# qq456cvb/VoteNet

Hardware: AMD Instinct MI355X
Metric: SUN RGB-D 20k-pt scenes/sec (fwd+bwd) (higher is better)
Workload: dtype f32

## Files before the change

### votenet_amd/_lib.py

```python
import ctypes
import os
import re
import subprocess

import torch

_HERE = os.path.dirname(os.path.abspath(__file__))
_LIB_PATH = os.path.join(_HERE, "lib", "libvotenet_hip.so")
_lib = None
SIDE_LIBS = {
    "monitors": "votenet_monitors.h",
    "guard": "votenet_step_guard.h",
    "features": "votenet_point_features.h",
    "detect": "votenet_detections.h",
    "boxpts": "votenet_box_points.h",
    "aabb": "votenet_aabb_nms.h",
    "depth": "votenet_depth_scan.h",
    "votesup": "votenet_vote_supervision.h",
    "propsup": "votenet_proposal_supervision.h",
    "votesamp": "votenet_vote_sampling.h",
    "instbox": "votenet_instance_boxes.h",
    "instvote": "votenet_instance_votes.h",
    "unitvote": "votenet_unit_votes.h",
}
_side = {}


class VotenetError(RuntimeError):
    """A HIP runtime / launch / workspace error reported by libvotenet_hip.so."""


class InvalidArgumentError(ValueError):
    """Mirror of tf.errors.InvalidArgumentError raised by the reference's OP_REQUIRES checks."""


def lib_path():
    return _LIB_PATH


def build(force=False):
    if force:
        import glob
        objs = [o for d in ["obj"] + [os.path.join(name, "obj") for name in SIDE_LIBS] for o in glob.glob(os.path.join(_HERE, "csrc", d, "*.o"))]
        for f in [_LIB_PATH] + [side_path(name) for name in SIDE_LIBS] + objs:
            if os.path.exists(f):
                os.remove(f)
    out = subprocess.run(["bash", os.path.join(_HERE, "csrc", "build.sh")], capture_output=True, text=True)
    if out.returncode != 0:
        raise VotenetError("libvotenet_hip.so build failed:\n" + out.stdout + out.stderr)
    return _LIB_PATH


_SCALARS = {"int": ctypes.c_int, "long": ctypes.c_long, "float": ctypes.c_float, "double": ctypes.c_double, "unsigned": ctypes.c_uint,
            "unsigned long long": ctypes.c_ulonglong, "size_t": ctypes.c_size_t}
_POINTEES = set(_SCALARS) | {"void", "char", "unsigned char", "unsigned short", "long long"}


def _declarator(text, where):
    words = text.replace("*", " * ").split()
    if not words or not words[-1].isidentifier():
        raise ValueError("%s: cannot read the declaration '%s'" % (where, " ".join(text.split())))
    return " ".join(w for w in words[:-1] if w != "const" and w != "*"), words.count("*"), words[-1]


def _ctype(base, stars, structs, where, ret=False):
    if stars == 0 and base in _SCALARS:
        return _SCALARS[base]
    if stars == 0 and ret and base == "void":
        return None
    if stars == 1 and base in structs:
        return ctypes.POINTER(structs[base])
    if stars == 1 and ret and base == "char":
        return ctypes.c_char_p
    if stars == 1 and base in _POINTEES:
        return ctypes.c_void_p
    raise ValueError("%s: no ctypes type for the C type '%s'" % (where, base + " *" * stars))


def parse_header(text, structs):
    text = re.sub(r"/\*.*?\*/|//[^\n]*", " ", text, flags=re.S)
    text = re.sub(r"#ifdef __cplusplus.*?#endif", "", text, flags=re.S)
    text = re.sub(r"^[ \t]*#.*$", "", text, flags=re.M)

    def struct(m):
        name, fields = m.group(2), []
        for line in filter(str.strip, m.group(1).split(";")):
            decls = [_declarator(d, name) for d in line.split(",")]
            fields += [(n, _ctype(decls[0][0], stars, structs, name + "." + n)) for _, stars, n in decls]
        structs[name] = type("".join(w.capitalize() for w in name.split("_")[1:]), (ctypes.Structure,),
                             {"_fields_": fields, "__doc__": "struct %s of the C ABI." % name})
        return ""
    text = re.sub(r"typedef\s+struct\s+\w+\s*\{(.*?)\}\s*(\w+)\s*;", struct, text, flags=re.S)
    funcs = {}
    for stmt in text.split(";"):
        if not stmt.strip():
            continue
        m = re.fullmatch(r"(.*?)\((.*)\)\s*", stmt, flags=re.S)
        if not m:
            raise ValueError("not a function declaration: '%s'" % " ".join(stmt.split()))
        base, stars, name = _declarator(m.group(1), "function")
        params = [] if m.group(2).strip() == "void" else m.group(2).split(",")
        funcs[name] = (_ctype(base, stars, structs, name, ret=True),
                       [_ctype(*_declarator(p, name)[:2], structs, name) for p in params])
    return funcs


_STRUCTS = ("BnRaw", "CoefTail", "MlpInput", "RowSegment", "CopySegment")
_abi_read = None


def _abi():
    global _abi_read
    if _abi_read is None:
        structs, protos = {}, []
        for h in ("votenet_hip.h", "votenet_hip_debug.h"):
            with open(os.path.join(_HERE, os.pardir, "include", h)) as f:
                protos.append(parse_header(f.read(), structs))
        globals().update({cls.__name__: cls for cls in structs.values()})
        _abi_read = tuple(protos)
    return _abi_read


def __getattr__(name):
    if name in _STRUCTS:
        _abi()
        return globals()[name]
    raise AttributeError("module %r has no attribute %r" % (__name__, name))


class _Library(ctypes.CDLL):

    def __getattr__(self, name):
        fn = super().__getattr__(name)
        for protos in _abi():
            if name in protos:
                fn.restype, fn.argtypes = protos[name]
        if "debug" in name and name not in ("votenet_debug_enable", "votenet_debug_enabled", "votenet_debug_fps_split_timeouts"):
            self.votenet_debug_enable(1)
        return fn


def lib():
    global _lib
    if _lib is None:
        if not os.path.exists(_LIB_PATH):
            raise VotenetError(
                "libvotenet_hip.so not found at %s -- run `python -c 'import __graft_entry__ as g; g.build()'` "
                "(there is no CPU fallback)" % _LIB_PATH)
        L = _Library(_LIB_PATH)
        for name in _abi()[0]:
            getattr(L, name)
        _lib = L
    return _lib


def side_path(name):
    return os.path.join(os.path.dirname(_LIB_PATH), "libvotenet_%s.so" % name)


def side_loaded(name):
    return name in _side


def side_lib(name):
    if name not in _side:
        path = side_path(name)
        if not os.path.exists(path):
            raise VotenetError("libvotenet_%s.so not found at %s -- run `python -c 'import __graft_entry__ as g; g.build()'` "
                               "(there is no CPU fallback)" % (name, path))
        with open(os.path.join(_HERE, os.pardir, "include", SIDE_LIBS[name])) as f:
            protos = parse_header(f.read(), {})
        S = ctypes.CDLL(path)
        for fname, (restype, argtypes) in protos.items():
            fn = getattr(S, fname)
            fn.restype, fn.argtypes = restype, argtypes
        last_error, = [getattr(S, fname) for fname in protos if fname.endswith("_last_error")]
        _side[name] = (S, last_error)
    return _side[name][0]


def check(rc, side=None):
    if rc == 0:
        return
    if side is None:
        msg, who = lib().votenet_last_error().decode(), "hip"
    else:
        side_lib(side)
        msg, who = _side[side][1]().decode(), side
    if rc == 1:
        raise InvalidArgumentError(msg)
    raise VotenetError("libvotenet_%s error %d: %s" % (who, rc, msg))


_raw_stream = getattr(torch._C, "_cuda_getCurrentRawStream", None)
_cur_device = getattr(torch._C, "_cuda_getDevice", None)


def stream_ptr():
    if _raw_stream is not None and _cur_device is not None:
        return _raw_stream(_cur_device())
    return torch.cuda.current_stream().cuda_stream


class _NoGuard:
    def __enter__(self):
        return None

    def __exit__(self, *a):
        return False


_NOGUARD = _NoGuard()


def device_guard(device):
    idx = device.index
    if _cur_device is not None and (idx is None or idx == _cur_device()):
        return _NOGUARD
    return torch.cuda.device(device)


def ptr(t):
    return t.data_ptr() if t is not None else None


def dev_f32(t, name, rank=None, last=None):
    if not isinstance(t, torch.Tensor):
        raise InvalidArgumentError("%s must be a torch.Tensor" % name)
    if not t.is_cuda:
        raise VotenetError("%s must live on the GPU (no CPU fallback in votenet_amd)" % name)
    if t.dtype != torch.float32:
        raise InvalidArgumentError("%s must be float32" % name)
    if rank is not None and t.dim() != rank:
        raise InvalidArgumentError("%s expects rank %d, got shape %s" % (name, rank, tuple(t.shape)))
    if last is not None and t.shape[-1] != last:
        raise InvalidArgumentError("%s expects last dimension %d, got shape %s" % (name, last, tuple(t.shape)))
    return t.contiguous()


def pitched_rows(t):
    return t.dim() == 3 and t.stride(2) == 1 and t.stride(1) >= t.shape[2] and t.stride(0) == t.shape[1] * t.stride(1)


def dev_f32_rows(t, name):
    if isinstance(t, torch.Tensor) and t.is_cuda and t.dtype == torch.float32 and pitched_rows(t):
        return t
    return dev_f32(t, name, 3)


def dev_i32(t, name, rank=None):
    if not isinstance(t, torch.Tensor):
        raise InvalidArgumentError("%s must be a torch.Tensor" % name)
    if not t.is_cuda:
        raise VotenetError("%s must live on the GPU (no CPU fallback in votenet_amd)" % name)
    if t.dtype != torch.int32:
        raise InvalidArgumentError("%s must be int32" % name)
    if rank is not None and t.dim() != rank:
        raise InvalidArgumentError("%s expects rank %d, got shape %s" % (name, rank, tuple(t.shape)))
    return t.contiguous()
```

### votenet_amd/csrc/half.hip

```cpp
#include "mlp_types.h"

namespace votenet {

constexpr int PS = kPiece, NP = kBallPieces, TP = kTilePieces;

__device__ __forceinline__ int kept_pieces(int cnt)
{
    const int c = cnt < 1 ? 1 : cnt;
    const int k = (c + PS - 1) / PS;
    return k > NP ? NP : k;
}

__global__ __launch_bounds__(1024) void half_groups_kernel(int G, const int *__restrict__ pts_cnt, int *__restrict__ pos, int *__restrict__ hc,
                                                           float *__restrict__ wh, int *__restrict__ nh_out, int *nh_host)
{
    __shared__ int s_wave[16];
    __shared__ int s_carry;
    const int tid = threadIdx.x, lane = tid & 63, wv = tid >> 6;
    if (tid == 0) s_carry = 0;
    __syncthreads();
    for (int c0 = 0; c0 < G; c0 += 1024) {
        const int c = c0 + tid;
        const int kc = c < G ? kept_pieces(pts_cnt[c]) : 1;
        const int mine = kc - 1;
        int x = mine;
#pragma unroll
        for (int off = 1; off < 64; off <<= 1) {
            const int t = __shfl_up(x, off);
            if (lane >= off) x += t;
        }
        if (lane == 63) s_wave[wv] = x;
        __syncthreads();
        int base = s_carry;
        for (int w = 0; w < wv; w++) base += s_wave[w];
        int p = base + x - mine;
        if (c < G) {
            hc[c] = c * NP;
            for (int j = 1; j < NP; j++) {
                if (j < kc) {
                    hc[G + p] = c * NP + j;
                    pos[c * (NP - 1) + j - 1] = p++;
                } else {
                    pos[c * (NP - 1) + j - 1] = -1;
                }
            }
        }
        __syncthreads();
        if (tid == 1023) s_carry = base + x;
        __syncthreads();
    }
    if (tid == 0) {
        int n2 = s_carry;
        for (int c = 0; c < G && ((G + n2) % TP) != 0; c++)
            for (int j = 1; j < NP && ((G + n2) % TP) != 0; j++)
                if (pos[c * (NP - 1) + j - 1] < 0) {
                    pos[c * (NP - 1) + j - 1] = n2;
                    hc[G + n2] = c * NP + j;
                    n2++;
                }
        s_carry = n2;
        nh_out[0] = G + n2;
        if (nh_host != nullptr) {
            nh_host[0] = G + n2;
            __threadfence_system();
        }
    }
    __syncthreads();
    const int nh = G + s_carry;
    for (int q = tid; q < nh; q += 1024) {
        float w = 1.0f;
        if (q < G) {
            int kc = 1;
            for (int j = 1; j < NP; j++) kc += pos[q * (NP - 1) + j - 1] >= 0 ? 1 : 0;
            w = 1.0f + (float)(PS * (NP - kc));
        }
        wh[q] = w;
    }
}

__device__ __forceinline__ double half_shfl_xor_f64(double v, int m)
{
    int lo = __double2loint(v), hi = __double2hiint(v);
    lo = __shfl_xor(lo, m);
    hi = __shfl_xor(hi, m);
    return __hiloint2double(hi, lo);
}
__device__ __forceinline__ long long half_fixed(float v) { return (long long)((double)v * 4294967296.0); }

__device__ __forceinline__ void half_sort_runs(unsigned prow, bool live, int lane, int &run_start, int &run_len)
{
    const unsigned prev = __shfl_up(prow, 1);
    const bool prev_live = __shfl_up((int)live, 1) != 0;
    const bool starts = live && (lane == 0 || !prev_live || prev != prow);
    const unsigned long long sm = __ballot(starts), lm = __ballot(live);
    const unsigned long long below = sm & ((lane == 63) ? ~0ull : ((1ull << (lane + 1)) - 1ull));
    run_start = below ? 63 - __builtin_clzll(below) : 0;
    const unsigned long long after = (sm | ~lm) & ~((run_start == 63) ? ~0ull : ((1ull << (run_start + 1)) - 1ull));
    const int end = after ? __builtin_ctzll(after) : 64;
    run_len = end - run_start;
}
__global__ __launch_bounds__(256) void assemble_rows_half_kernel(const int *__restrict__ nh_dev, long max_rows, int n, int groups_per_scene, const float *__restrict__ xyz,
                                                                 const float *__restrict__ new_xyz, const int *__restrict__ idx,
                                                                 const int *__restrict__ pts_cnt, const int *__restrict__ hc,
                                                                 float4 *__restrict__ geo, long long *__restrict__ cntv,
                                                                 double *__restrict__ moments, int *__restrict__ count)
{
    __shared__ double red[4][9];
    double acc[9];
#pragma unroll
    for (int i = 0; i < 9; i++) acc[i] = 0.0;
    const long rows = (long)nh_dev[0] * PS;
    for (long r0 = (long)blockIdx.x * 256; r0 < max_rows; r0 += (long)gridDim.x * 256) {
        const long r = r0 + threadIdx.x;
        const bool live = r < rows;
        unsigned my_prow = 0;
        if (!live && r < max_rows) geo[r] = make_float4(0.f, 0.f, 0.f, __uint_as_float(0u));
        if (live) {
        const int q = (int)(r / PS), s = (int)(r % PS);
        const int code = hc[q];
        const int c = code / NP;
        const int k = (code % NP) * PS + s;
        const int id = idx[(size_t)c * 64 + k];
        const unsigned prow = ((unsigned)c / (unsigned)groups_per_scene) * (unsigned)n + (unsigned)id;
        const float dx = xyz[(size_t)prow * 3 + 0] - new_xyz[(size_t)c * 3 + 0];
        const float dy = xyz[(size_t)prow * 3 + 1] - new_xyz[(size_t)c * 3 + 1];
        const float dz = xyz[(size_t)prow * 3 + 2] - new_xyz[(size_t)c * 3 + 2];
        geo[r] = make_float4(dx, dy, dz, __uint_as_float(prow));
        my_prow = prow;
        int cnt = pts_cnt[c];
        if (cnt < 1) cnt = 1;
        if (k < cnt) {
            const long long mult = (k == 0) ? (long long)(64 - cnt + 1) : 1LL;
            if (cntv) {
                unsigned long long *cv = reinterpret_cast<unsigned long long *>(cntv + (size_t)prow * 4);
                atomicAdd(cv + 0, (unsigned long long)mult);
                atomicAdd(cv + 1, (unsigned long long)(mult * half_fixed(dx)));
                atomicAdd(cv + 2, (unsigned long long)(mult * half_fixed(dy)));
                atomicAdd(cv + 3, (unsigned long long)(mult * half_fixed(dz)));
            }
            const double m = (double)mult, x = dx, y = dy, z = dz;
            acc[0] += m * x; acc[1] += m * y; acc[2] += m * z;
            acc[3] += m * x * x; acc[4] += m * x * y; acc[5] += m * x * z; acc[6] += m * y * y; acc[7] += m * y * z; acc[8] += m * z * z;
        }
        }
        if (count) {
            int rs, rl;
            half_sort_runs(my_prow, live, threadIdx.x & 63, rs, rl);
            if (live && rs == (int)(threadIdx.x & 63)) atomicAdd(&count[my_prow], rl);
        }
    }
    if (!moments) return;
#pragma unroll
    for (int i = 0; i < 9; i++) {
        double v = acc[i];
#pragma unroll
        for (int m = 32; m >= 1; m >>= 1) v += half_shfl_xor_f64(v, m);
        if ((threadIdx.x & 63) == 0) red[threadIdx.x >> 6][i] = v;
    }
    __syncthreads();
    if (threadIdx.x < 9)
        unsafeAtomicAdd(&moments[threadIdx.x], (red[0][threadIdx.x] + red[1][threadIdx.x]) + (red[2][threadIdx.x] + red[3][threadIdx.x]));
}

__global__ __launch_bounds__(256) void narrow_rows_half_kernel(const int *__restrict__ nh_dev, int n, int groups_per_scene, int c,
                                                               const float *__restrict__ xyz, const float *__restrict__ new_xyz,
                                                               const float *__restrict__ feat, const int *__restrict__ idx,
                                                               const int *__restrict__ pts_cnt, const int *__restrict__ hc,
                                                               float *__restrict__ u8, double *__restrict__ moments)
{
    __shared__ double red[4][44];
    double acc[44];
#pragma unroll
    for (int i = 0; i < 44; i++) acc[i] = 0.0;
    const long rows = (long)nh_dev[0] * PS;
    for (long r = (long)blockIdx.x * 256 + threadIdx.x; r < rows; r += (long)gridDim.x * 256) {
        const int q = (int)(r / PS), s = (int)(r % PS);
        const int code = hc[q];
        const int ctr = code / NP;
        const int k = (code % NP) * PS + s;
        const int id = idx[(size_t)ctr * 64 + k];
        const size_t prow = (size_t)((unsigned)ctr / (unsigned)groups_per_scene) * n + id;
        float u[8];
        u[0] = xyz[prow * 3 + 0] - new_xyz[(size_t)ctr * 3 + 0];
        u[1] = xyz[prow * 3 + 1] - new_xyz[(size_t)ctr * 3 + 1];
        u[2] = xyz[prow * 3 + 2] - new_xyz[(size_t)ctr * 3 + 2];
#pragma unroll
        for (int d = 0; d < 5; d++) u[3 + d] = d < c ? feat[prow * c + d] : 0.0f;
        *reinterpret_cast<float4 *>(u8 + (size_t)r * 8) = make_float4(u[0], u[1], u[2], u[3]);
        *reinterpret_cast<float4 *>(u8 + (size_t)r * 8 + 4) = make_float4(u[4], u[5], u[6], u[7]);
        int cnt = pts_cnt[ctr];
        if (cnt < 1) cnt = 1;
        if (k < cnt) {
            const double mult = (k == 0) ? (double)(64 - cnt + 1) : 1.0;
            int t = 8;
#pragma unroll
            for (int d = 0; d < 8; d++) {
                acc[d] += mult * (double)u[d];
#pragma unroll
                for (int e = d; e < 8; e++) acc[t++] += mult * ((double)u[d] * (double)u[e]);
            }
        }
    }
    if (!moments) return;
#pragma unroll
    for (int i = 0; i < 44; i++) {
        double v = acc[i];
#pragma unroll
        for (int m = 32; m >= 1; m >>= 1) v += half_shfl_xor_f64(v, m);
        if ((threadIdx.x & 63) == 0) red[threadIdx.x >> 6][i] = v;
    }
    __syncthreads();
    if (threadIdx.x < 44) {
        const double v = (red[0][threadIdx.x] + red[1][threadIdx.x]) + (red[2][threadIdx.x] + red[3][threadIdx.x]);
        const int i = threadIdx.x;
        if (i < 8) {
            unsafeAtomicAdd(&moments[i], v);
        } else {
            int d = 0, t = 8;
            while (i >= t + (8 - d)) {
                t += 8 - d;
                d++;
            }
            const int e = d + (i - t);
            unsafeAtomicAdd(&moments[8 + d * 8 + e], v);
            if (e != d) unsafeAtomicAdd(&moments[8 + e * 8 + d], v);
        }
    }
}

__global__ void bn_pool_finalize_half_kernel(long total, int G, int c, const float *__restrict__ zbest, const int *__restrict__ abest,
                                             const int *__restrict__ pos, const float *__restrict__ scale, const float *__restrict__ shift,
                                             BnRaw raw, int relu, float *__restrict__ out, int *__restrict__ argmax, float *__restrict__ zsel)
{
    const long e0 = (long)blockIdx.x * blockDim.x + threadIdx.x;
    const int ch = (int)(e0 % c);
    float s = 0.0f, h = 0.0f;
    if (e0 < total) {
        if (raw.stats) bn_raw_channel(raw, c, ch, e0 < c, s, h);
        else {
            s = scale[ch];
            h = shift[ch];
        }
    }
    for (long e = e0; e < total; e += (long)gridDim.x * blockDim.x) {
        const long g = e / c;
        const float sg = s >= 0.0f ? 1.0f : -1.0f;
        int pj[NP - 1];
#pragma unroll
        for (int j = 1; j < NP; j++) pj[j - 1] = pos[g * (NP - 1) + j - 1];
        float zb[NP];
        int ab[NP];
        zb[0] = zbest[e];
        ab[0] = abest[e];
#pragma unroll
        for (int j = 1; j < NP; j++) {
            const size_t e2 = pj[j - 1] >= 0 ? (size_t)(G + pj[j - 1]) * c + ch : (size_t)e;
            zb[j] = zbest[e2];
            ab[j] = abest[e2];
        }
        float best = sg * zb[0];
        int ibest = ab[0];
#pragma unroll
        for (int j = 1; j < NP; j++) {
            const float b = sg * zb[j];
            if (pj[j - 1] >= 0 && b > best) {
                best = b;
                ibest = j * PS + ab[j];
            }
        }
        const float zr = sg * best;
        float v = zr * s + h;
        if (relu && !(v > 0.0f)) v = 0.0f;
        out[e] = v;
        if (argmax) argmax[e] = ibest;
        if (zsel) zsel[e] = zr;
    }
}

__global__ __launch_bounds__(256) void half_sort_count_kernel(const int *__restrict__ nh_dev, const float4 *__restrict__ geo,
                                                              int *__restrict__ count)
{
    const long rows = (long)nh_dev[0] * PS;
    const int lane = threadIdx.x & 63;
    for (long r0 = (long)blockIdx.x * 256; r0 < rows; r0 += (long)gridDim.x * 256) {
        const long r = r0 + threadIdx.x;
        const bool live = r < rows;
        const unsigned prow = live ? __float_as_uint(geo[r].w) : 0u;
        int rs, rl;
        half_sort_runs(prow, live, lane, rs, rl);
        if (live && rs == lane) atomicAdd(&count[prow], rl);
    }
}
__global__ __launch_bounds__(1024) void half_sort_scan_kernel(int npts, int *__restrict__ count)
{
    __shared__ int s_wave[16];
    const int tid = threadIdx.x, lane = tid & 63, wv = tid >> 6;
    const int per = (npts + 1023) / 1024;
    const int b0 = tid * per < npts ? tid * per : npts, e0 = b0 + per < npts ? b0 + per : npts;
    constexpr int KEEP = 16;
    int v[KEEP];
    int tot = 0;
    if (per <= KEEP) {
#pragma unroll
        for (int i = 0; i < KEEP; i++) v[i] = b0 + i < e0 ? count[b0 + i] : 0;
#pragma unroll
        for (int i = 0; i < KEEP; i++) tot += v[i];
    } else {
        for (int p = b0; p < e0; p++) tot += count[p];
    }
    int x = tot;
#pragma unroll
    for (int off = 1; off < 64; off <<= 1) {
        const int t = __shfl_up(x, off);
        if (lane >= off) x += t;
    }
    if (lane == 63) s_wave[wv] = x;
    __syncthreads();
    int run = x - tot;
    for (int w = 0; w < wv; w++) run += s_wave[w];
    if (per <= KEEP) {
#pragma unroll
        for (int i = 0; i < KEEP; i++) {
            if (b0 + i < e0) count[b0 + i] = run;
            run += v[i];
        }
        return;
    }
    for (int p = b0; p < e0; p++) {
        const int c = count[p];
        count[p] = run;
        run += c;
    }
}
__global__ __launch_bounds__(256) void half_sort_fill_kernel(const int *__restrict__ nh_dev, const float4 *__restrict__ geo,
                                                             int *__restrict__ cursor, int *__restrict__ order)
{
    const long rows = (long)nh_dev[0] * PS;
    const int lane = threadIdx.x & 63;
    for (long r0 = (long)blockIdx.x * 256; r0 < rows; r0 += (long)gridDim.x * 256) {
        const long r = r0 + threadIdx.x;
        const bool live = r < rows;
        const unsigned prow = live ? __float_as_uint(geo[r].w) : 0u;
        int rs, rl;
        half_sort_runs(prow, live, lane, rs, rl);
        int base = 0;
        if (live && rs == lane) base = atomicAdd(&cursor[prow], rl);
        base = __shfl(base, rs);
        if (live) order[base + (lane - rs)] = (int)r;
    }
}

template <int COUT>
__global__ __launch_bounds__(256) void group_linear_bwd_sorted_kernel(long rows, const int *__restrict__ order, const float4 *__restrict__ geo,
                                                                      const float *__restrict__ wh, const float *__restrict__ ptab,
                                                                      const float *__restrict__ wx, const float *__restrict__ da,
                                                                      const float *__restrict__ coef, int relu, float *__restrict__ spt,
                                                                      float *__restrict__ dw_xyz, const int *__restrict__ nh_dev)
{
    if (nh_dev != nullptr) {
        const long lim = (long)nh_dev[0] * PS;
        rows = lim < rows ? lim : rows;
    }
    constexpr int CPB = 256 / COUT;
    constexpr int CH = 64;
    __shared__ int s_row[CPB][CH];
    __shared__ float4 s_geo[CPB][CH];
    __shared__ float s_w[CPB][CH];
    __shared__ float red[256][3];
    const int tid = threadIdx.x;
    const int ch = tid % COUT, cl = tid / COUT;
    const float kA = coef[ch], kB = coef[COUT + ch], kC = coef[2 * COUT + ch], kS = coef[3 * COUT + ch], kH = coef[4 * COUT + ch];
    const float wx0 = wx[ch], wx1 = wx[COUT + ch], wx2 = wx[2 * COUT + ch];
    float a0 = 0.f, a1 = 0.f, a2 = 0.f;
    const long nchunk = (rows + CH - 1) / CH;
    for (long c0 = (long)blockIdx.x * CPB; c0 < nchunk; c0 += (long)gridDim.x * CPB) {
        lds_barrier();
        if (tid < CPB * CH) {
            const long e = c0 * CH + tid;
            int r = -1;
            float4 g4 = make_float4(0.f, 0.f, 0.f, 0.f);
            float w = 1.0f;
            if (e < rows) {
                r = order[e];
                g4 = geo[r];
                if (r % PS == 0) w = wh[r / PS];
            }
            s_row[tid / CH][tid % CH] = r;
            s_geo[tid / CH][tid % CH] = g4;
            s_w[tid / CH][tid % CH] = w;
        }
        lds_barrier();
        if (c0 + cl >= nchunk) continue;
        unsigned cur = 0xffffffffu;
        float acc = 0.0f;
        bool first = true;
#pragma unroll 1
        for (int e0 = 0; e0 < CH; e0 += 8) {
            float gg[8], zz[8];
#pragma unroll
            for (int u = 0; u < 8; u++) {
                const int r = s_row[cl][e0 + u];
                const int rr = r < 0 ? 0 : r;
                gg[u] = da[(size_t)rr * COUT + ch];
                zz[u] = ptab[(size_t)__float_as_uint(s_geo[cl][e0 + u].w) * COUT + ch];
            }
#pragma unroll
            for (int u = 0; u < 8; u++) {
                if (s_row[cl][e0 + u] < 0) continue;
                const float4 g4 = s_geo[cl][e0 + u];
                const unsigned prow = __float_as_uint(g4.w);
                if (prow != cur) {
                    if (cur != 0xffffffffu) {
                        if (first) unsafeAtomicAdd(&spt[(size_t)cur * COUT + ch], acc);
                        else spt[(size_t)cur * COUT + ch] = acc;
                        first = false;
                    }
                    cur = prow;
                    acc = 0.0f;
                }
                const float z = assembled_z(zz[u], g4, wx0, wx1, wx2);
                float gq = gg[u];
                if (relu && !(z * kS + kH > 0.0f)) gq = 0.0f;
                const float d = kA * gq + s_w[cl][e0 + u] * (kB + kC * z);
                a0 += g4.x * d;
                a1 += g4.y * d;
                a2 += g4.z * d;
                acc += d;
            }
        }
        if (cur != 0xffffffffu) unsafeAtomicAdd(&spt[(size_t)cur * COUT + ch], acc);
    }
    red[tid][0] = a0;
    red[tid][1] = a1;
    red[tid][2] = a2;
    __syncthreads();
    if (tid < COUT) {
#pragma unroll
        for (int d = 0; d < 3; d++) {
            float t = 0.0f;
            for (int q = 0; q < CPB; q++) t += red[q * COUT + tid][d];
            unsafeAtomicAdd(&dw_xyz[(size_t)d * COUT + tid], t);
        }
    }
}

constexpr int kMaskedSlots = 32;
template <int COUT>
__global__ __launch_bounds__(256) void group_linear_bwd_masked_kernel(long rows, const int *__restrict__ order, const float4 *__restrict__ geo,
                                                                      const float *__restrict__ ptab, const float *__restrict__ wx,
                                                                      const float *__restrict__ da, const float *__restrict__ scale,
                                                                      const float *__restrict__ shift, const float *__restrict__ mean,
                                                                      const float *__restrict__ var, float eps, int relu,
                                                                      float *__restrict__ sg, float *__restrict__ ug, double *__restrict__ sums,
                                                                      double *__restrict__ part ,
                                                                      const int *__restrict__ nh_dev, CoefTail tail)
{
    if (nh_dev != nullptr) {
        const long lim = (long)nh_dev[0] * PS;
        rows = lim < rows ? lim : rows;
    }
    constexpr int CPB = 256 / COUT;
    constexpr int CH = 64;
    constexpr int GB = 8;
    __shared__ int s_row[CPB][CH];
    __shared__ float4 s_geo[CPB][CH];
    __shared__ float red[256][5];
    const int tid = threadIdx.x;
    const int ch = tid % COUT, cl = tid / COUT;
    const float kS = scale[ch], kH = shift[ch], kM = mean[ch], kR = 1.0f / sqrtf(var[ch] + eps);
    const float wx0 = wx[ch], wx1 = wx[COUT + ch], wx2 = wx[2 * COUT + ch];
    float a0 = 0.f, a1 = 0.f, a2 = 0.f, s1 = 0.f, s2 = 0.f;
    const long nchunk = (rows + CH - 1) / CH;
    for (long c0 = (long)blockIdx.x * CPB; c0 < nchunk; c0 += (long)gridDim.x * CPB) {
        lds_barrier();
        if (tid < CPB * CH) {
            const long e = c0 * CH + tid;
            int r = -1;
            float4 g4 = make_float4(0.f, 0.f, 0.f, 0.f);
            if (e < rows) {
                r = order[e];
                g4 = geo[r];
            }
            s_row[tid / CH][tid % CH] = r;
            s_geo[tid / CH][tid % CH] = g4;
        }
        lds_barrier();
        if (c0 + cl >= nchunk) continue;
        unsigned cur = 0xffffffffu;
        float acc = 0.0f;
        bool first = true;
#pragma unroll 1
        for (int e0 = 0; e0 < CH; e0 += GB) {
            float gg[GB], zz[GB];
#pragma unroll
            for (int u = 0; u < GB; u++) {
                const int r = s_row[cl][e0 + u];
                const int rr = r < 0 ? 0 : r;
                gg[u] = da[(size_t)rr * COUT + ch];
                zz[u] = ptab[(size_t)__float_as_uint(s_geo[cl][e0 + u].w) * COUT + ch];
            }
#pragma unroll
            for (int u = 0; u < GB; u++) {
                if (s_row[cl][e0 + u] < 0) continue;
                const float4 g4 = s_geo[cl][e0 + u];
                const unsigned prow = __float_as_uint(g4.w);
                if (prow != cur) {
                    if (cur != 0xffffffffu) {
                        if (first) unsafeAtomicAdd(&sg[(size_t)cur * COUT + ch], acc);
                        else sg[(size_t)cur * COUT + ch] = acc;
                        first = false;
                    }
                    cur = prow;
                    acc = 0.0f;
                }
                const float z = assembled_z(zz[u], g4, wx0, wx1, wx2);
                float gq = gg[u];
                if (relu && !(z * kS + kH > 0.0f)) gq = 0.0f;
                a0 += g4.x * gq;
                a1 += g4.y * gq;
                a2 += g4.z * gq;
                s1 += gq;
                s2 += gq * ((z - kM) * kR);
                acc += gq;
            }
        }
        if (cur != 0xffffffffu) unsafeAtomicAdd(&sg[(size_t)cur * COUT + ch], acc);
    }
    red[tid][0] = a0;
    red[tid][1] = a1;
    red[tid][2] = a2;
    red[tid][3] = s1;
    red[tid][4] = s2;
    __syncthreads();
    if (tid < COUT) {
        float t[5];
#pragma unroll
        for (int d = 0; d < 5; d++) {
            t[d] = 0.0f;
            for (int q = 0; q < CPB; q++) t[d] += red[q * COUT + tid][d];
        }
        double *ps = part + (size_t)(blockIdx.x % kMaskedSlots) * 5 * COUT;
#pragma unroll
        for (int d = 0; d < 5; d++) unsafeAtomicAdd(&ps[(size_t)d * COUT + tid], (double)t[d]);
    }
    __shared__ unsigned s_last;
    asm volatile("s_waitcnt vmcnt(0)" ::: "memory");
    __syncthreads();
    if (threadIdx.x == 0) s_last = (__hip_atomic_fetch_add(tail.ticket, 1u, __ATOMIC_RELAXED, __HIP_MEMORY_SCOPE_AGENT) == gridDim.x - 1) ? 1u : 0u;
    __syncthreads();
    if (!s_last) return;
    const double invn = 1.0 / (double)tail.rows;
    for (int col = threadIdx.x; col < COUT; col += blockDim.x) {
        double q[5] = {0.0, 0.0, 0.0, 0.0, 0.0};
        for (int sl = 0; sl < kMaskedSlots; sl++)
#pragma unroll
            for (int d = 0; d < 5; d++)
                q[d] += __hip_atomic_load(&part[((size_t)sl * 5 + d) * COUT + col], __ATOMIC_RELAXED, __HIP_MEMORY_SCOPE_AGENT);
#pragma unroll
        for (int d = 0; d < 3; d++) ug[(size_t)d * COUT + col] = (float)q[d];
        sums[col] = q[3];
        sums[COUT + col] = q[4];
        const float inv = 1.0f / sqrtf(var[col] + eps);
        const float m1 = (float)(q[3] * invn), m2 = (float)(q[4] * invn);
        const float cA = tail.gamma[col] * inv;
        const float cC = -cA * inv * m2;
        tail.coef[col] = cA;
        tail.coef[COUT + col] = -cA * m1 - cC * mean[col];
        tail.coef[2 * COUT + col] = cC;
        tail.coef[3 * COUT + col] = scale[col];
        tail.coef[4 * COUT + col] = shift[col];
        if (tail.dgamma) tail.dgamma[col] += (float)q[4];
        if (tail.dbeta) tail.dbeta[col] += (float)q[3];
    }
    if (threadIdx.x == 0) *tail.ticket = 0u;
}

template <int COUT>
__global__ __launch_bounds__(256) void assembled_point_grad_kernel(long npts, const float *__restrict__ ptab, const long long *__restrict__ cntv,
                                                                   const float *__restrict__ wx, const float *__restrict__ coef,
                                                                   float *__restrict__ s, float *__restrict__ vp )
{
    constexpr int PPB = 256 / COUT;
    constexpr int U = 4;
    __shared__ float red[256][3];
    const int tid = threadIdx.x, ch = tid % COUT, pl = tid / COUT;
    const float kA = coef[ch], kB = coef[COUT + ch], kC = coef[2 * COUT + ch];
    const float wx0 = wx[ch], wx1 = wx[COUT + ch], wx2 = wx[2 * COUT + ch];
    float v0 = 0.f, v1 = 0.f, v2 = 0.f;
    const long stride = (long)gridDim.x * PPB;
    for (long p0 = (long)blockIdx.x * PPB + pl; p0 < npts; p0 += U * stride) {
        long long c4[U][4];
        float pv[U], sv[U];
#pragma unroll
        for (int u = 0; u < U; u++) {
            const long p = p0 + u * stride < npts ? p0 + u * stride : p0;
            const long long *cv = cntv + (size_t)p * 4;
            c4[u][0] = cv[0];
            c4[u][1] = cv[1];
            c4[u][2] = cv[2];
            c4[u][3] = cv[3];
            pv[u] = ptab[(size_t)p * COUT + ch];
            sv[u] = s[(size_t)p * COUT + ch];
        }
#pragma unroll
        for (int u = 0; u < U; u++) {
            const long p = p0 + u * stride;
            if (p >= npts || c4[u][0] == 0) continue;
            const float fx = (float)((double)c4[u][1] * (1.0 / 4294967296.0)), fy = (float)((double)c4[u][2] * (1.0 / 4294967296.0)),
                        fz = (float)((double)c4[u][3] * (1.0 / 4294967296.0));
            const float fc = (float)c4[u][0];
            const float zsum = fc * pv[u] + (fx * wx0 + fy * wx1 + fz * wx2);
            s[(size_t)p * COUT + ch] = kA * sv[u] + fc * kB + kC * zsum;
            v0 += fx * pv[u];
            v1 += fy * pv[u];
            v2 += fz * pv[u];
        }
    }
    red[tid][0] = v0;
    red[tid][1] = v1;
    red[tid][2] = v2;
    __syncthreads();
    if (tid < COUT) {
#pragma unroll
        for (int d = 0; d < 3; d++) {
            float t = 0.0f;
            for (int q = 0; q < PPB; q++) t += red[q * COUT + tid][d];
            unsafeAtomicAdd(&vp[((size_t)(blockIdx.x % kMaskedSlots) * 3 + d) * COUT + tid], t);
        }
    }
}

__global__ __launch_bounds__(256) void assembled_wx_finish_kernel(int cout, const float *__restrict__ coef, const float *__restrict__ ug,
                                                                  const float *__restrict__ vp, int nparts, const double *__restrict__ mom,
                                                                  const float *__restrict__ wx, float *__restrict__ dw_xyz)
{
// ... 241 lines not shown
```

### votenet_amd/csrc/loss.hip

```cpp
#include "common.h"
#include "nearest_box.h"

namespace votenet {

#ifndef LOSS_ABL
#define LOSS_ABL 0
#endif
constexpr int LOSS_T = 1024;
constexpr int LOSS_MAXC = 32;
constexpr int LOSS_NACC = 12;

struct LossArgs {
    int b, n, p, bb, nh, ns, nc;
    const float *seeds, *votes, *pxyz, *pout;
    const float *gxyz, *glwh, *groty;
    const int *sem, *hlab, *slab;
    const float *hres, *sres;
    float pos_thr, neg_thr;
    float *losses, *d_votes, *d_pxyz, *d_pout;
    long pout_pitch;
};

__device__ __forceinline__ float huber(float e, float &grad)
{
    const float a = fabsf(e);
    grad = a <= 1.0f ? e : (e > 0.0f ? 1.0f : -1.0f);
    return a <= 1.0f ? 0.5f * e * e : a - 0.5f;
}

__device__ __forceinline__ float softmax_ce(const float *lg, int c, int label, float *probs)
{
    float m = lg[0];
    for (int i = 1; i < c; i++) m = fmaxf(m, lg[i]);
    float s = 0.0f;
    for (int i = 0; i < c; i++) {
        probs[i] = expf(lg[i] - m);
        s += probs[i];
    }
    if ((unsigned)label >= (unsigned)c) {
        const float nan = __uint_as_float(0x7FC00000u);
        for (int i = 0; i < c; i++) probs[i] = nan;
        return nan;
    }
    const float inv = 1.0f / s;
    for (int i = 0; i < c; i++) probs[i] = probs[i] * inv - (i == label ? 1.0f : 0.0f);
    return logf(s) + m - lg[label];
}


__global__ __launch_bounds__(256) void votenet_loss_count_kernel(LossArgs A, int *counts)
{
    __shared__ float s_box[LOSS_MAXBOX][8];
    const int b = blockIdx.x, tid = threadIdx.x, BB = A.bb, P = A.p;
    for (int j = tid; j < BB; j += 256)
        for (int k = 0; k < 3; k++) s_box[j][k] = A.gxyz[(b * BB + j) * 3 + k];
    __syncthreads();
    int np_local = 0, nn_local = 0;
    for (int pq = tid; pq < P; pq += 256) {
        const int q = b * P + pq;
        int g;
        const float best = nearest_box(s_box, BB, A.pxyz[q * 3 + 0], A.pxyz[q * 3 + 1], A.pxyz[q * 3 + 2], g);
        np_local += best < A.pos_thr;
        nn_local += best > A.neg_thr;
    }
    for (int off = 32; off > 0; off >>= 1) {
        np_local += __shfl_down(np_local, off);
        nn_local += __shfl_down(nn_local, off);
    }
    if ((tid & 63) == 0) {
        if (np_local) atomicAdd(&counts[0], np_local);
        if (nn_local) atomicAdd(&counts[1], nn_local);
    }
}

__global__ __launch_bounds__(LOSS_T) void votenet_loss_kernel(LossArgs A, int *counts, float *partial )
{
    __shared__ float s_box[LOSS_MAXBOX][8];
    __shared__ float s_red[LOSS_T / 64][LOSS_NACC];
    __shared__ float s_dual[LOSS_MAXBOX][3];
    __shared__ int s_dualp[LOSS_MAXBOX];
    __shared__ int s_last;
    const int tid = threadIdx.x, b = blockIdx.x;
    const int B = A.b, N = A.n, P = A.p, BB = A.bb, NH = A.nh, NS = A.ns, NC = A.nc;
    const int W = 5 + 2 * NH + 4 * NS + NC;
    for (int j = tid; j < BB; j += LOSS_T) {
        const int e = b * BB + j;
        s_box[j][0] = A.gxyz[e * 3 + 0];
        s_box[j][1] = A.gxyz[e * 3 + 1];
        s_box[j][2] = A.gxyz[e * 3 + 2];
        s_box[j][3] = A.glwh[e * 3 + 0] * 0.5f;
        s_box[j][4] = A.glwh[e * 3 + 1] * 0.5f;
        s_box[j][5] = A.glwh[e * 3 + 2] * 0.5f;
        s_box[j][6] = cosf(-A.groty[e]);
        s_box[j][7] = sinf(-A.groty[e]);
    }
    __syncthreads();
    const int n_pos = counts[0], n_neg = counts[1];
    const float inv_np = 1.0f / (float)n_pos, inv_nn = 1.0f / (float)n_neg;
    float acc[LOSS_NACC];
#pragma unroll
    for (int i = 0; i < LOSS_NACC; i++) acc[i] = 0.0f;
    const int wave = tid >> 6, nwave = LOSS_T / 64;
    const int nbusy = (P + 63) / 64 < nwave ? (P + 63) / 64 : nwave, nfree = nwave - nbusy;
    const bool early = nfree > 0;
    const float inv_bn = 1.0f / (float)(B * N);
    auto seed_terms = [&](int first, int step) {
        for (int i = first; i < ((LOSS_ABL & 2) ? 0 : N); i += step) {
            const int e = b * N + i;
            const float sx = A.seeds[e * 3 + 0], sy = A.seeds[e * 3 + 1], sz = A.seeds[e * 3 + 2];
            float best = 0.0f;
            int g = 0;
            bool surface = false;
            for (int j = 0; j < BB; j++) {
                const float dx = fabsf(sx - s_box[j][0]), dy = fabsf(sy - s_box[j][1]), dz = fabsf(sz - s_box[j][2]);
                const float c = s_box[j][6], s = s_box[j][7];
                const float rx = c * dx + s * dz, ry = dy, rz = -s * dx + c * dz;
                surface = surface || (rx < s_box[j][3] && ry < s_box[j][4] && rz < s_box[j][5]);
                const float d = sqrtf(rx * rx + ry * ry + rz * rz);
                if (j == 0 || d < best) {
                    best = d;
                    g = j;
                }
            }
            if (surface) {
                for (int k = 0; k < 3; k++) {
                    const float df = A.votes[e * 3 + k] - s_box[g][k];
                    acc[0] += fabsf(df);
                    A.d_votes[e * 3 + k] = (df > 0.0f ? 1.0f : (df < 0.0f ? -1.0f : 0.0f)) * inv_bn;
                }
            }
        }
    };
    float pr[LOSS_MAXC];
    for (int pq = tid; pq < ((LOSS_ABL & 1) ? 0 : P); pq += LOSS_T) {
        const int q = b * P + pq;
        const float px = A.pxyz[q * 3 + 0], py = A.pxyz[q * 3 + 1], pz = A.pxyz[q * 3 + 2];
        int g;
        const float best = nearest_box(s_box, BB, px, py, pz, g);
        const float *o = A.pout + (size_t)q * A.pout_pitch;
        float *go = A.d_pout + (size_t)q * W;
        const bool pos = best < A.pos_thr, neg = best > A.neg_thr;
        if (pos || neg) {
            const float l = softmax_ce(o, 2, pos ? 1 : 0, pr);
            const float w = 0.5f * (pos ? inv_np : inv_nn);
            acc[pos ? 1 : 2] += l;
            go[0] = pr[0] * w;
            go[1] = pr[1] * w;
        }
        if (pos) {
            const int gi = b * BB + g;
            const float cg[3] = {s_box[g][0] - px, s_box[g][1] - py, s_box[g][2] - pz};
            for (int k = 0; k < 3; k++) {
                float gr;
                acc[3] += huber(o[2 + k] - cg[k], gr);
                go[2 + k] += gr * inv_np;
                A.d_pxyz[q * 3 + k] += gr * inv_np;
            }
            const int hl = A.hlab[gi];
            const bool hok = (unsigned)hl < (unsigned)NH;
            acc[5] += softmax_ce(o + 5, NH, hl, pr);
            for (int i = 0; i < NH; i++) go[5 + i] = pr[i] * (0.1f * inv_np);
            {
                float gr;
                acc[6] += huber((hok ? o[5 + NH + hl] : 0.0f) - A.hres[gi], gr);
                if (hok) go[5 + NH + hl] = gr * inv_np;
            }
            const int sl = A.slab[gi], so = 5 + 2 * NH;
            const bool sok = (unsigned)sl < (unsigned)NS;
            acc[7] += softmax_ce(o + so, NS, sl, pr);
            for (int i = 0; i < NS; i++) go[so + i] = pr[i] * (0.1f * inv_np);
            for (int k = 0; k < 3; k++) {
                float gr;
                acc[8] += huber((sok ? o[so + NS + sl * 3 + k] : 0.0f) - A.sres[gi * 3 + k], gr);
                if (sok) go[so + NS + sl * 3 + k] = gr * inv_np;
            }
            const int co = W - NC;
            acc[9] += softmax_ce(o + co, NC, A.sem[gi], pr);
            for (int i = 0; i < NC; i++) go[co + i] = pr[i] * (0.1f * inv_np);
        }
    }
    const float inv_bbb = 1.0f / (float)(B * BB);
    const int dw = early ? wave - nbusy : wave, dstep = early ? nfree : nwave;
    for (int j = dw < 0 ? BB : dw; j < ((LOSS_ABL & 4) ? 0 : BB); j += dstep) {
        const int lane = tid & 63;
        const float gx = s_box[j][0], gy = s_box[j][1], gz = s_box[j][2];
        float best = INFINITY;
        int bp = 0x7FFFFFFF;
        for (int p = lane; p < P; p += 64) {
            const float dx = A.pxyz[(b * P + p) * 3 + 0] - gx, dy = A.pxyz[(b * P + p) * 3 + 1] - gy,
                        dz = A.pxyz[(b * P + p) * 3 + 2] - gz;
            const float d = sqrtf(dx * dx + dy * dy + dz * dz);
            if (d < best) {
                best = d;
                bp = p;
            }
        }
        for (int off = 32; off > 0; off >>= 1) {
            const float ob = __shfl_xor(best, off);
            const int op = __shfl_xor(bp, off);
            if (ob < best || (ob == best && op < bp)) {
                best = ob;
                bp = op;
            }
        }
        if ((unsigned)bp >= (unsigned)P) bp = 0;
        if (lane < 3) {
            const int k = lane, q = b * P + bp;
            const float cgk = (k == 0 ? gx : (k == 1 ? gy : gz)) - A.pxyz[q * 3 + k];
            float gr;
            acc[4] += huber(A.pout[(size_t)q * A.pout_pitch + 2 + k] - cgk, gr);
            s_dual[j][k] = gr * inv_bbb;
            if (k == 0) s_dualp[j] = bp;
        }
    }
    if (early && wave >= nbusy) seed_terms(tid - nbusy * 64, nfree * 64);
    __syncthreads();
    for (int pq = tid; pq < P; pq += LOSS_T) {
        const int q = b * P + pq;
        for (int j = 0; j < BB; j++)
            if (s_dualp[j] == pq) {
#pragma unroll
                for (int k = 0; k < 3; k++) {
                    A.d_pout[(size_t)q * W + 2 + k] += s_dual[j][k];
                    A.d_pxyz[q * 3 + k] += s_dual[j][k];
                }
            }
    }
    if (!early) seed_terms(tid, LOSS_T);
#pragma unroll
    for (int i = 0; i < LOSS_NACC; i++) {
        float v = acc[i];
        for (int off = 32; off > 0; off >>= 1) v += __shfl_down(v, off);
        if ((tid & 63) == 0) s_red[tid >> 6][i] = v;
    }
    __syncthreads();
    if (tid < LOSS_NACC) {
        float v = 0.0f;
        for (int w = 0; w < LOSS_T / 64; w++) v += s_red[w][tid];
        partial[b * LOSS_NACC + tid] = v;
    }
    __threadfence();
    __syncthreads();
    if (tid == 0) s_last = (atomicAdd(&counts[2], 1) == B - 1);
    __syncthreads();
    if (!s_last) return;
    __threadfence();
    if (tid < LOSS_NACC) {
        float v = 0.0f;
        for (int sc = 0; sc < B; sc++) v += __builtin_nontemporal_load(&partial[sc * LOSS_NACC + tid]);
        s_red[0][tid] = v;
    }
    __syncthreads();
    if (tid == 0) {
        float t[LOSS_NACC];
        for (int i = 0; i < LOSS_NACC; i++) t[i] = s_red[0][i];
        const float vote = t[0] * inv_bn;
        const float obj = t[1] * inv_np + t[2] * inv_nn;
        const float center = t[3] * inv_np + t[4] * inv_bbb;
        const float hcls = t[5] * inv_np, hres = t[6] * inv_np, scls = t[7] * inv_np, sres = t[8] * inv_np, sem = t[9] * inv_np;
        const float box = center + 0.1f * hcls + hres + 0.1f * scls + sres;
        float *L = A.losses;
        L[0] = vote + 0.5f * obj + box + 0.1f * sem;
        L[1] = vote;
        L[2] = obj;
        L[3] = center;
        L[4] = hcls;
        L[5] = hres;
        L[6] = scls;
        L[7] = sres;
        L[8] = sem;
        L[9] = box;
        L[10] = (float)n_pos;
        L[11] = (float)n_neg;
    }
}

}

using namespace votenet;

extern "C" size_t votenet_loss_workspace_floats(int b) { return 4 + (size_t)(b > 0 ? b : 0) * LOSS_NACC; }

extern "C" int votenet_loss_pitched(int b, int n_seeds, int n_prop, int n_box, int nh, int ns, int nc, const float *seeds_xyz,
                            const float *votes_xyz, const float *proposals_xyz, const float *proposals_output, long output_pitch,
                            const float *bboxes_xyz,
                            const float *bboxes_lwh, const float *bboxes_roty, const int *semantic_labels, const int *heading_labels,
                            const float *heading_residuals, const int *size_labels, const float *size_residuals, float pos_thr,
                            float neg_thr, float *losses, float *d_votes_xyz, float *d_proposals_xyz, float *d_proposals_output,
                            float *workspace, void *stream)
{
    VN_REQUIRE(b > 0 && n_seeds > 0 && n_prop > 0 && n_box > 0, "votenet_loss expects b, n_seeds, n_prop, n_box > 0");
    VN_REQUIRE(n_box <= LOSS_MAXBOX, "votenet_loss expects at most 256 boxes per scene");
    VN_REQUIRE(nh > 0 && ns > 0 && nc > 0 && nh <= LOSS_MAXC && ns <= LOSS_MAXC && nc <= LOSS_MAXC, "votenet_loss expects 0 < nh, ns, nc <= 32");
    VN_REQUIRE(pos_thr < neg_thr, "votenet_loss expects pos_thr < neg_thr (config.py)");
    VN_REQUIRE(seeds_xyz && votes_xyz && proposals_xyz && proposals_output && bboxes_xyz && bboxes_lwh && bboxes_roty &&
                   semantic_labels && heading_labels && heading_residuals && size_labels && size_residuals && losses &&
                   d_votes_xyz && d_proposals_xyz && d_proposals_output && workspace,
               "votenet_loss: null buffer");
    VN_REQUIRE(output_pitch >= 5 + 2 * nh + 4 * ns + nc, "votenet_loss: the pitch of proposals_output is smaller than its width");
    LossArgs a = {b, n_seeds, n_prop, n_box, nh, ns, nc, seeds_xyz, votes_xyz, proposals_xyz, proposals_output, bboxes_xyz, bboxes_lwh,
                  bboxes_roty, semantic_labels, heading_labels, size_labels, heading_residuals, size_residuals, pos_thr, neg_thr, losses,
                  d_votes_xyz, d_proposals_xyz, d_proposals_output, output_pitch};
    int *counts = reinterpret_cast<int *>(workspace);
    hipStream_t st = as_stream(stream);
    hipLaunchKernelGGL(votenet_loss_count_kernel, dim3(b), dim3(256), 0, st, a, counts);
    hipLaunchKernelGGL(votenet_loss_kernel, dim3(b), dim3(LOSS_T), 0, st, a, counts, workspace + 4);
    return check_launch("votenet_loss");
}

extern "C" int votenet_loss(int b, int n_seeds, int n_prop, int n_box, int nh, int ns, int nc, const float *seeds_xyz,
                            const float *votes_xyz, const float *proposals_xyz, const float *proposals_output, const float *bboxes_xyz,
                            const float *bboxes_lwh, const float *bboxes_roty, const int *semantic_labels, const int *heading_labels,
                            const float *heading_residuals, const int *size_labels, const float *size_residuals, float pos_thr,
                            float neg_thr, float *losses, float *d_votes_xyz, float *d_proposals_xyz, float *d_proposals_output,
                            float *workspace, void *stream)
{
    return votenet_loss_pitched(b, n_seeds, n_prop, n_box, nh, ns, nc, seeds_xyz, votes_xyz, proposals_xyz, proposals_output,
                                5 + 2 * nh + 4 * ns + nc, bboxes_xyz, bboxes_lwh, bboxes_roty, semantic_labels, heading_labels,
                                heading_residuals, size_labels, size_residuals, pos_thr, neg_thr, losses, d_votes_xyz, d_proposals_xyz,
                                d_proposals_output, workspace, stream);
}

namespace votenet {

__global__ void decode_boxes_kernel(int total, int nh, int ns, int nc, const float *__restrict__ pxyz, const float *__restrict__ pout,
                                    const float *__restrict__ mean_size, float *__restrict__ boxes, float *__restrict__ scores)
{
    const int q = blockIdx.x * blockDim.x + threadIdx.x;
    if (q >= total) return;
    const int W = 5 + 2 * nh + 4 * ns + nc;
    const float *o = pout + (size_t)q * W;
    int sc = 0;
    for (int i = 1; i < ns; i++)
        if (o[5 + 2 * nh + i] > o[5 + 2 * nh + sc]) sc = i;
    int hc = 0;
    for (int i = 1; i < nh; i++)
        if (o[5 + i] > o[5 + hc]) hc = i;
    float size[3];
    for (int k = 0; k < 3; k++) size[k] = mean_size[sc * 3 + k] * fmaxf(1.0f + o[5 + 2 * nh + ns + sc * 3 + k], 1e-6f);
    const float cx = pxyz[q * 3 + 0] + o[2], cy = pxyz[q * 3 + 1] + o[3], cz = pxyz[q * 3 + 2] + o[4];
    const float PI_F = 3.14159265358979323846f;
    const float t = ((float)hc * 2.0f + o[5 + nh + hc]) * (PI_F / (float)nh);
    float ang = fmodf(t, 2.0f * PI_F);
    if (ang < 0.0f) ang += 2.0f * PI_F;
    const float c = cosf(ang), s = sinf(ang);
    const float l = size[0], w = size[1], h = size[2];
    const float sx[8] = {1, 1, -1, -1, 1, 1, -1, -1}, sy[8] = {1, 1, 1, 1, -1, -1, -1, -1}, sz[8] = {1, -1, -1, 1, 1, -1, -1, 1};
    float *bx = boxes + (size_t)q * 24;
    for (int m = 0; m < 8; m++) {
        const float x0 = sx[m] * l * 0.5f, y0 = sy[m] * h * 0.5f, z0 = sz[m] * w * 0.5f;
        bx[m * 3 + 0] = c * x0 + s * z0 + cx;
        bx[m * 3 + 1] = y0 + cy;
        bx[m * 3 + 2] = -s * x0 + c * z0 + cz;
    }
    float best = o[W - nc];
    for (int i = 1; i < nc; i++) best = fmaxf(best, o[W - nc + i]);
    scores[q] = best;
}

}

extern "C" int votenet_decode_boxes(int b, int n_prop, int nh, int ns, int nc, const float *proposals_xyz, const float *proposals_output,
                                    const float *class_mean_size, float *bboxes, float *scores, void *stream)
{
    VN_REQUIRE(b >= 0 && n_prop >= 0 && nh > 0 && ns > 0 && nc > 0, "decode_boxes: bad shape");
    const int total = b * n_prop;
    if (total == 0) return VOTENET_OK;
    VN_REQUIRE(proposals_xyz && proposals_output && class_mean_size && bboxes && scores, "decode_boxes: null buffer");
    hipLaunchKernelGGL(votenet::decode_boxes_kernel, dim3((total + 255) / 256), dim3(256), 0, as_stream(stream), total, nh, ns, nc,
                       proposals_xyz, proposals_output, class_mean_size, bboxes, scores);
    return check_launch("decode_boxes");
}
```

### votenet_amd/loss.py

```python
import torch

from . import _lib as L
from .synth import NC, NH, NS

POSITIVE_THRES, NEGATIVE_THRES = 0.3, 0.6
NAMES = ("total_cost", "vote_reg_loss", "obj_cls_loss", "center_loss", "heading_cls_loss", "heading_residual_loss",
         "size_cls_loss", "size_residual_loss", "sem_cls_loss", "box_loss", "n_pos", "n_neg")
GT_KEYS = ("bboxes_xyz", "bboxes_lwh", "bboxes_roty", "semantic_labels", "heading_labels", "heading_residuals", "size_labels",
           "size_residuals")


def gt_to_device(gt, device):
    return {k: torch.from_numpy(gt[k]).contiguous().to(device) for k in GT_KEYS}


def loss_buffers(out, losses=None):
    from . import mlp as M
    votes, pxyz, pout = out["votes_xyz"], out["proposals_xyz"], out["proposals_output"]
    nws = int(L.lib().votenet_loss_workspace_floats(votes.shape[0]))
    if losses is None:
        losses = torch.empty(12, dtype=torch.float32, device=votes.device)
    return losses, M._zeros_f32((votes.numel() + pxyz.numel() + pout.numel() + nws,), votes.device)


def cotangent_views(votes, pxyz, pout, flat):
    nv, npx, npo = votes.numel(), pxyz.numel(), pout.numel()
    cot = dict(votes_xyz=flat[:nv].view_as(votes), proposals_xyz=flat[nv:nv + npx].view_as(pxyz),
               proposals_output=flat[nv + npx:nv + npx + npo].view_as(pout))
    return cot, flat[nv + npx + npo:]


def check_losses(losses, dev, who):
    if not (isinstance(losses, torch.Tensor) and losses.is_cuda and losses.dtype == torch.float32 and losses.numel() == 12
            and losses.is_contiguous() and losses.device == dev):
        raise L.InvalidArgumentError("%s: losses must be the 12 floats of votenet_loss on the device" % who)


def votenet_loss(out, gt, nh=NH, ns=NS, nc=NC, buffers=None):
    seeds = L.dev_f32(out["seeds_xyz"], "loss seeds_xyz", 3, 3)
    votes = L.dev_f32(out["votes_xyz"], "loss votes_xyz", 3, 3)
    pxyz = L.dev_f32(out["proposals_xyz"], "loss proposals_xyz", 3, 3)
    pout = L.dev_f32_rows(out["proposals_output"], "loss proposals_output")
    b, n = seeds.shape[:2]
    p = pxyz.shape[1]
    bb = gt["bboxes_xyz"].shape[1]
    if pout.shape[2] != 5 + 2 * nh + 4 * ns + nc:
        raise L.InvalidArgumentError("loss: proposals_output has %d channels, expected %d" % (pout.shape[2], 5 + 2 * nh + 4 * ns + nc))
    dev = seeds.device
    total = votes.numel() + pxyz.numel() + pout.numel() + int(L.lib().votenet_loss_workspace_floats(b))
    from . import mlp as M
    if buffers is not None:
        losses, flat = buffers
        if flat.numel() != total or losses.numel() != 12:
            raise L.InvalidArgumentError("loss: the buffers were made for other shapes (loss_buffers(out))")
    else:
        losses = torch.empty(12, dtype=torch.float32, device=dev)
        flat = M._zeros_f32((total,), dev)
    cot, ws = cotangent_views(votes, pxyz, pout, flat)
    with L.device_guard(dev):
        L.check(L.lib().votenet_loss_pitched(b, n, p, bb, nh, ns, nc, L.ptr(seeds), L.ptr(votes), L.ptr(pxyz), L.ptr(pout), pout.stride(1),
                                     L.ptr(gt["bboxes_xyz"]), L.ptr(gt["bboxes_lwh"]), L.ptr(gt["bboxes_roty"]),
                                     L.ptr(gt["semantic_labels"]), L.ptr(gt["heading_labels"]), L.ptr(gt["heading_residuals"]),
                                     L.ptr(gt["size_labels"]), L.ptr(gt["size_residuals"]), POSITIVE_THRES, NEGATIVE_THRES,
                                     L.ptr(losses), L.ptr(cot["votes_xyz"]), L.ptr(cot["proposals_xyz"]), L.ptr(cot["proposals_output"]),
                                     L.ptr(ws), L.stream_ptr()))
    return losses, cot


ACCURACY_COUNTS = ("n_obj_correct", "n_sem_correct", "n_pos", "n_neg")
RING_COLS = 5


def votenet_accuracies(out, gt, nh=NH, ns=NS, nc=NC, losses=None, ring=None, ring_row=0, buffers=None):
    pxyz = L.dev_f32(out["proposals_xyz"], "accuracies proposals_xyz", 3, 3)
    pout = L.dev_f32_rows(out["proposals_output"], "accuracies proposals_output")
    b, p = pxyz.shape[:2]
    if pout.shape[2] != 5 + 2 * nh + 4 * ns + nc or tuple(pout.shape[:2]) != (b, p):
        raise L.InvalidArgumentError("accuracies: proposals_output has shape %s, expected (%d, %d, %d)"
                                     % (tuple(pout.shape), b, p, 5 + 2 * nh + 4 * ns + nc))
    gxyz, sem = L.dev_f32(gt["bboxes_xyz"], "accuracies bboxes_xyz", 3, 3), L.dev_i32(gt["semantic_labels"], "accuracies semantic_labels", 2)
    if gxyz.shape[0] != b or tuple(sem.shape) != tuple(gxyz.shape[:2]):
        raise L.InvalidArgumentError("accuracies: ground truth of %s boxes / %s labels for %d scenes" % (tuple(gxyz.shape), tuple(sem.shape), b))
    dev = pxyz.device
    if buffers is not None:
        acc, counts, work = buffers
    else:
        acc = torch.empty(2, dtype=torch.float32, device=dev)
        counts = torch.empty(4, dtype=torch.int32, device=dev)
        work = torch.zeros(8, dtype=torch.int32, device=dev)
    if acc.numel() != 2 or counts.numel() != 4 or work.numel() < 8:
        raise L.InvalidArgumentError("accuracies: buffers of the wrong size")
    rows = 0
    if ring is not None:
        ring = L.dev_f32(ring, "accuracies ring", 2, RING_COLS)
        rows = ring.shape[0]
        if not 0 <= ring_row < rows:
            raise L.InvalidArgumentError("accuracies: row %d outside a ring of %d rows" % (ring_row, rows))
    if losses is not None and (losses.numel() != 12 or losses.dtype != torch.float32 or not losses.is_cuda):
        raise L.InvalidArgumentError("accuracies: losses must be the 12 floats of votenet_loss on the device")
    with L.device_guard(dev):
        L.check(L.side_lib("monitors").votenet_accuracies(b, p, gxyz.shape[1], nh, ns, nc, L.ptr(pxyz), L.ptr(pout), pout.stride(1), L.ptr(gxyz), L.ptr(sem),
                                           POSITIVE_THRES, NEGATIVE_THRES, L.ptr(losses), L.ptr(ring), rows, ring_row, L.ptr(acc),
                                           L.ptr(counts), L.ptr(work), L.stream_ptr()), side="monitors")
    return acc, counts


def decode_boxes(proposals_xyz, proposals_output, nh=NH, ns=NS, nc=NC):
    from .synth import MEAN_SIZES
    pxyz = L.dev_f32(proposals_xyz, "decode_boxes proposals_xyz", 3, 3)
    pout = L.dev_f32(proposals_output, "decode_boxes proposals_output", 3)
    b, p = pxyz.shape[:2]
    if pout.shape[2] != 5 + 2 * nh + 4 * ns + nc:
        raise L.InvalidArgumentError("decode_boxes: proposals_output has %d channels" % pout.shape[2])
    mean = torch.tensor(MEAN_SIZES, dtype=torch.float32, device=pxyz.device).contiguous()
    boxes = torch.empty((b, p, 8, 3), dtype=torch.float32, device=pxyz.device)
    scores = torch.empty((b, p), dtype=torch.float32, device=pxyz.device)
    with L.device_guard(pxyz.device):
        L.check(L.lib().votenet_decode_boxes(b, p, nh, ns, nc, L.ptr(pxyz), L.ptr(pout), L.ptr(mean), L.ptr(boxes), L.ptr(scores),
                                             L.stream_ptr()))
    return boxes, scores
```

### votenet_amd/model.py

```python

import math
from typing import NamedTuple

import torch

from . import checkpoint
from . import dp
from . import mlp as M
from . import pointnet2 as P

NH, NS, NC = 12, 10, 10
PREFETCH_AFTER = 2
SIDE_PRIORITY = 0
WGRAD_PRIORITY = 0
PROPOSAL_NUM = 256
PROPOSAL_OUT = 5 + 2 * NH + 4 * NS + NC
LEARNING_RATE = 1e-3


GEOMETRY_GRAPHS = True
GEOMETRY_MAX_EVICTIONS = 8
GEOMETRY_RING = 3


# ... 442 lines not shown
            tape.append(dict(op="vote", recs=recs, b=b, n=n))
        return v_xyz, v_p

    def propose(self, votes_xyz, votes_points, seeds_xyz, tape=None, prop_fps=None):
        geom = None
        if self.proposal_sampling == "vote_fps":
            from . import vote_sampling as VSAMP
            pr = self.proposal
            geom = pr.geometry(votes_xyz, grouped=VSAMP.cluster_votes(votes_xyz, pr.npoint, pr.radius, pr.nsample))
        elif prop_fps is not None:
            geom = self.proposal.geometry(votes_xyz, fps_idx=prop_fps, ahead=False)
        p_xyz, p_out, _ = self.proposal.forward(votes_xyz, votes_points, sample_xyz=seeds_xyz, tape=tape, geom=geom)
        return p_xyz, p_out

    def forward(self, x, tape=None, next_x=None, feats=None, next_feats=None):
        self._sa1_points(x, feats)
        self.store.refresh_split()
        M.arena_begin(self.device)
        try:
            lv, g = self.backbone_levels(x, tape, next_x=next_x, feats=feats, next_feats=next_feats)
            self._stamp_tape(tape)
            out = self._head_forward(lv, g.get("fp1"), g.get("fp2"), g.get("prop_fps"), tape,
                                     copy_seeds=self._geometry.current is not None)
        finally:
            M.arena_end()
        return out

    def _stamp_tape(self, tape):
        gg = self._geometry.current
        if gg is not None and tape:
            tape[0]["geometry_stamp"] = (gg, gg.generation)

    def _head_forward(self, lv, fp1_geom, fp2_geom, prop_fps, tape, copy_seeds=False):
        l3_p2 = self.fp1.forward(lv["l3_xyz"], lv["l4_xyz"], lv["l3_p"], lv["l4_p"], tape=tape, geom=fp1_geom)
        seeds_p = self.fp2.forward(lv["l2_xyz"], lv["l3_xyz"], lv["l2_p"], l3_p2, tape=tape, geom=fp2_geom)
        seeds_xyz = lv["l2_xyz"]
        seeds_out = torch.empty_like(seeds_xyz) if copy_seeds else None
        v_xyz, v_p = self.vote(seeds_xyz, seeds_p, tape, seeds_copy=seeds_out)
        p_xyz, p_out = self.propose(v_xyz, v_p, seeds_xyz, tape, prop_fps)
        return dict(seeds_xyz=seeds_out if seeds_out is not None else seeds_xyz, seeds_points=seeds_p, votes_xyz=v_xyz, votes_points=v_p,
                    proposals_xyz=p_xyz, proposals_output=p_out)

    def decode_boxes(self, proposals_xyz, proposals_output):
        from . import loss as VL
        return VL.decode_boxes(proposals_xyz, proposals_output)

    BN_MOMENTUM = 0.9

    def _bn_layers(self):
        mods = [self.sa1, self.sa2, self.sa3, self.sa4, self.fp1, self.fp2, self.proposal]
        layers = [L for m in mods for L in m.mlp + (getattr(m, "mlp2", None) or [])] + list(self.voting)
        return [L for L in layers if L.bn]

    def _ema_state(self):
        if getattr(self, "_ema", None) is None:
            self._ema = {}
            st = self.store
            self._ema_flat = torch.zeros_like(st.bn_flat) if st.bn_flat is not None else None
            base = st.bn_flat.data_ptr() if st.bn_flat is not None else 0
            for L in self._bn_layers():
                blk = st._bn_views.get(L.name)
                if blk is not None and self._ema_flat is not None:
                    o = (blk.data_ptr() - base) // 4
                    t = self._ema_flat[o:o + 4 * L.cout].view(4, L.cout)
                else:
                    t = torch.zeros((4, L.cout), dtype=torch.float32, device=self.device)
                t[3].fill_(1.0)
                self._ema[L.name] = t
            self._ema_fac = {}
            self._ema_fac_flat = None
            self._ema_fac_by_rows = {}
            self._ema_version = 0
        return self._ema

    @staticmethod
    def _bn_records(tape):
        for t in tape:
            for r in t.get("recs", []) + t.get("recs2", []):
                if r.get("bn_out") is not None:
                    yield r

    def update_moving_averages(self, tape):
        ema = self._ema_state()
        recs = list(self._bn_records(tape))
        for r in recs:
            P.check_bn_block(r)
        st = self.store
        blocks = st._bn_views
        if self._ema_flat is not None and self._ema_flat.is_cuda and len(recs) == len(blocks) and \
                all(r["bn_out"] is blocks.get(r["layer"].name) for r in recs):
            key = tuple(r["rows"] for r in recs)
            if self._ema_fac_flat is None or self._ema_fac_flat[0] != key:
                f = self._ema_fac_by_rows.get(key)
                if f is None:
                    f = torch.full_like(st.bn_flat, 1.0 - self.BN_MOMENTUM)
                    base = st.bn_flat.data_ptr()
                    for r in recs:
                        c, rows = r["layer"].cout, r["rows"]
                        o = (blocks[r["layer"].name].data_ptr() - base) // 4
                        f[o + 3 * c:o + 4 * c] *= rows / max(rows - 1.0, 1.0)
                    self._ema_fac_by_rows[key] = f
                self._ema_fac_flat = (key, f)
            from . import _lib as L_
            with L_.device_guard(self.device):
                L_.check(L_.lib().votenet_ema_update(st.bn_flat.numel(), self.BN_MOMENTUM, L_.ptr(self._ema_flat), L_.ptr(st.bn_flat),
                                                     L_.ptr(self._ema_fac_flat[1]), L_.stream_ptr()))
            self._ema_version += 1
            return
        dst, src, fac = [], [], []
        for r in recs:
            name, rows = r["layer"].name, r["rows"]
            key = (name, rows)
            if key not in self._ema_fac:
                f = torch.full((4, r["layer"].cout), 1.0 - self.BN_MOMENTUM, dtype=torch.float32, device=self.device)
                f[3].mul_(rows / max(rows - 1.0, 1.0))
                self._ema_fac[key] = f
            dst.append(ema[name])
            src.append(r["bn_out"])
            fac.append(self._ema_fac[key])
        if dst:
            torch._foreach_mul_(dst, self.BN_MOMENTUM)
            torch._foreach_addcmul_(dst, src, fac)
            self._ema_version += 1

    def inference_bn(self):
        ema = self._ema_state()
        key = (self._ema_version, self.store.generation, self.store.flat._version)
        if getattr(self, "_frozen_key", None) != key:
            self._frozen = {}
            for L in self._bn_layers():
                e = ema[L.name]
                sc = L.p("gamma") * torch.rsqrt(e[3] + M.BN_EPS)
                self._frozen[L.name] = M.FrozenBN(torch.stack([sc, L.p("beta") - e[2] * sc]).contiguous())
            self._frozen_key = key
        return self._frozen

    def predict(self, x, iou_threshold=0.25, next_x=None, sync=True, batch_statistics=False, feats=None, next_feats=None,
                protocol="reference", min_points=0, nms_overlap="rotated", nms_measure="iou"):
        from . import aabb_nms, detections, tf_nms3d
        params = detections.protocol_params(protocol, iou_threshold)
        aabb_nms.check_overlap(protocol, nms_overlap, nms_measure, "predict")
        if isinstance(min_points, bool) or not isinstance(min_points, int) or min_points < 0:
            raise M.L.InvalidArgumentError("predict: min_points must be an int >= 0, got %r" % (min_points,))
        self._sa1_points(x, feats, "predict")
        if not batch_statistics and self._ema_state() is not None and self._ema_version == 0 and not getattr(self, "_warned_ema", False):
            import warnings
            warnings.warn("VoteNetHotPath.predict: no training step has updated the BatchNorm moving averages yet (mean 0, variance 1): "
                          "pass batch_statistics=True for a freshly initialised model", stacklevel=2)
            self._warned_ema = True
        with P.frozen_bn(None if batch_statistics else self.inference_bn()):
            out = self.forward(x, next_x=next_x, **self._feats_kw(feats, next_feats))
        boxes, score = self.decode_boxes(out["proposals_xyz"], out["proposals_output"])
        objectness = lambda: out["proposals_output"][..., :2].contiguous()
        gate = {}
        if min_points > 0:
            from . import box_points
            gate = dict(point_counts=box_points.box_point_counts(boxes, x))
            gated = box_points.gate_objectness(objectness(), gate["point_counts"], min_points)
            objectness = lambda: gated
        if params is not None:
            cls = out["proposals_output"][..., -NC:].contiguous()
            if nms_overlap == "rotated":
                det = detections.class_nms3d(boxes, objectness(), cls, **params)
            else:
                det = aabb_nms.class_nms_aabb(boxes, objectness(), cls, overlap=nms_overlap, measure=nms_measure, **params)
            return dict(bboxes=boxes, scores=score, class_scores=cls, **gate, **det, **out)
        keep = tf_nms3d.NMS3D(boxes, score, objectness(), iou_threshold, padded=not sync)
        extra = dict(gate) if sync else dict(nms_count=keep[1], **gate)
        return dict(bboxes=boxes, scores=score, nms_idx=keep if sync else keep[0], class_scores=out["proposals_output"][..., -NC:].contiguous(),
                    **extra, **out)

    def make_cotangents(self, b, seed=0):
        g = torch.Generator(device="cpu").manual_seed(1234 + seed)
        n_seed = self.sa2.npoint
        return dict(proposals_output=(torch.randn(b, PROPOSAL_NUM, PROPOSAL_OUT, generator=g) / (b * PROPOSAL_NUM)).to(self.device),
                    votes_xyz=(torch.randn(b, n_seed, 3, generator=g) / (b * n_seed)).to(self.device))

    def backward(self, tape, cot):
        self.check_tape(tape)
        M.arena_begin(self.device)
        try:
            with P.WGRAD.on(self._wgrad_side()):
                self._backward(tape, cot)
                P.wgrad_join()
        finally:
            M.arena_end()

    @staticmethod
    def check_tape(tape):
        stamp = tape[0].get("geometry_stamp") if tape else None
        if stamp is not None and stamp[0].generation != stamp[1]:
            raise M.L.VotenetError("backward(): the geometry buffers this tape was recorded on have been overwritten by %d later prefetch(es) "
                                   "(model.GeometryGraph; a tape on prefetched geometry is valid until GEOMETRY_RING - 1 = %d further "
                                   "batches have been prefetched)" % (stamp[0].generation - stamp[1], GEOMETRY_RING - 1))

    def _backward(self, tape, cot):
        d_l2p, d_l3p, d_l4p = self._head_backward(tape[4:8], cot)
        self._levels_backward(tape[:4], d_l2p, d_l3p, d_l4p)

    def _head_backward(self, tail, cot, cut=None):
        fp1, fp2, vote, prop = tail
        cut = cut if cut is not None else (lambda: None)
        d_vp, d_vx = self.proposal.backward(prop, cot["proposals_output"], need_feat_grad=True, need_xyz_grad=True)
        P.wgrad_flush()
        cut()
        if cot.get("proposals_xyz") is not None:
            d_vx = P.tf_sampling.gather_point_grad_raw(d_vx.shape[1], prop["fps_idx"], cot["proposals_xyz"], into=d_vx.contiguous())
        b, n = vote["b"], vote["n"]
        rows = b * n
        last = self.voting[-1]
        padw = last.cout_pad if last.cout_pad else 259
        d_votes_p = torch.empty((rows, padw), dtype=torch.float32, device=d_vp.device)
        cv = cot.get("votes_xyz")
        segs = [(d_votes_p[:, :3], d_vx.reshape(rows, 3), cv.reshape(rows, 3) if cv is not None else None),
                (d_votes_p[:, 3:259], d_vp.reshape(rows, 256), None)]
        if padw > 259:
            segs.append((d_votes_p[:, 259:], None, None))
        if vote.get("unit") is not None:
            from . import unit_votes as UV
            UV.unit_votes_backward(d_vx, cv, d_vp, vote["unit"]["y"], vote["unit"]["norm"], d_votes_p)
        else:
            M.row_segments(rows, segs)
        d_votes = d_votes_p[:, :259]
        d_in = P.mlp_chain_backward(vote["recs"], d_votes, "plain", need_input_grad=True, g_padded=d_votes_p if padw > 259 else None)
        P.wgrad_flush()
        cut()
        d_seeds_p = torch.empty((b, n, 256), dtype=torch.float32, device=d_vp.device)
        M.row_segments(rows, [(d_seeds_p.view(rows, 256), d_votes[:, 3:], d_in[:, 3:259])])
        d_l2p, d_l3p2 = self.fp2.backward(fp2, d_seeds_p)
        P.wgrad_flush()
        cut()
        d_l3p, d_l4p = self.fp1.backward(fp1, d_l3p2)
        P.wgrad_flush()
        return d_l2p, d_l3p, d_l4p

    def _levels_backward(self, levels, d_l2p, d_l3p, d_l4p):
        sa1, sa2, sa3, sa4 = levels
        self._grams_early(dict(sa1=sa1, sa2=sa2, sa3=sa3, sa4=sa4))
        g3, _ = self.sa4.backward(sa4, d_l4p)
        P.wgrad_flush()
        d_l3p = P.add_rows(d_l3p, g3)
        g2, _ = self.sa3.backward(sa3, d_l3p)
        P.wgrad_flush()
        d_l2p = P.add_rows(d_l2p, g2)
        if getattr(self, "_gsync", None) is not None:
            self._gsync.start_tail([P.WGRAD.stream])
        with P.WGRAD.on(None if getattr(self, "inline_wgrad_tail", INLINE_WGRAD_TAIL) else P.WGRAD.stream):
            g1, _ = self.sa2.backward(sa2, d_l2p)
            P.wgrad_flush()
            with P.WGRAD.fine():
                self.sa1.backward(sa1, g1, need_feat_grad=False)

    def _stretch_eligible(self, x, cot, gt):
        return bool(STRETCH_GRAPH and gt is not None and cot is None and x.is_cuda and not M.DETERMINISTIC and PREFETCH_AFTER < 5
                    and M.PROFILE_EVENTS is None and P._FROZEN.table is None and not getattr(self, "_stretch_off", False)
                    and not torch.cuda.is_current_stream_capturing())

    @staticmethod
    def _stretch_inputs(lv, g):
        ins = dict(lv)
        for name in ("fp1", "fp2"):
            idx = g[name].idx
            ins[name + "_idx"], ins[name + "_w"] = idx, g[name].weight
            inv = getattr(idx, "_inv", None)
            if inv is not None:
                ins[name + "_inv0"], ins[name + "_inv1"] = inv
        ins["prop_fps"] = g["prop_fps"]
        return ins

    def _stretch_body(self, I, tape_levels, wgrad_stream, gt=None, cut=None, loss_hook=None, copy_seeds=False):
        from . import loss as VL

        def geom(name):
            idx = I[name + "_idx"]
            if name + "_inv0" in I:
                idx._inv = (I[name + "_inv0"], I[name + "_inv1"])
            return P.FPGeometry(idx, I[name + "_w"])
        tail = []
        lv = {k: I[k] for k in ("l2_xyz", "l2_p", "l3_xyz", "l3_p", "l4_xyz", "l4_p")}
        out = self._head_forward(lv, geom("fp1"), geom("fp2"), I["prop_fps"], tail, copy_seeds=copy_seeds)
        self.update_moving_averages(list(tape_levels) + tail)
        losses, cot = loss_hook(out) if loss_hook is not None else VL.votenet_loss(out, gt)
        if loss_hook is None:
            self._after_loss(out, gt, losses, cot)
        with P.WGRAD.on(wgrad_stream):
            grads = self._head_backward(tail, cot, cut=cut)
            if cut is None:
                P.wgrad_join()
        self._stretch_tail = tail
        return out, losses, grads

    def _train_step_stretch(self, x, gt, tape, next_x, feats=None, next_feats=None):
        self.store.refresh_split()
        lv, g = self.backbone_levels(x, tape, next_x=next_x, feats=feats, next_feats=next_feats)
        self._stamp_tape(tape)
        self._keep_seed_levels(tape)
        self._grams_ahead(tape)
        if not all(k in g for k in ("fp1", "fp2", "prop_fps")):
            g = dict(g)
            g.setdefault("fp1", P.FPModule.geometry(lv["l3_xyz"], lv["l4_xyz"]))
            g.setdefault("fp2", P.FPModule.geometry(lv["l2_xyz"], lv["l3_xyz"]))
            g.setdefault("prop_fps", P.tf_sampling.farthest_point_sample(self.proposal.npoint, lv["l2_xyz"]))
        ins = self._stretch_inputs(lv, g)
        key = tuple((k, tuple(v.shape), v.dtype) for k, v in ins.items()) + (P.HALF_GROUPS, P.ASSEMBLE_FIRST, P.ASSEMBLE_INLINE, P.POOL_GRAM_BACKWARD, P.ASSEMBLED_DECOMPOSED,
                                                                             self.overlap_wgrad, STRETCH_SEGMENTS, M.SPLIT_K, M.COEF_TAIL, P.WGRAD_BATCH, P.POOL_IN_EPILOGUE,
                                                                             self.store.split, bool(getattr(self, "inline_wgrad_tail", INLINE_WGRAD_TAIL)), M.FORWARD_H2, M.ADHOC_H2,
                                                                             self.proposal_sampling or "seed_fps", self.vote_features or "sum", M.CONFIG_EPOCH)
        graphs = self.__dict__.setdefault("_stretch_graphs", {})
        sg = graphs.get(key)
        self._gsync.begin()
        if sg is None:
            dkey = key[:-1]
            demand = self.__dict__.setdefault("_stretch_demand", {}).get(dkey)
            geometry_events = P.tf_sampling.PROFILE_EVENTS is not None or P.tf_grouping.PROFILE_EVENTS is not None
            if demand is None or geometry_events:
                a = M._StatsArena
                off0, want0 = a.off, a.want32
                self.check_tape(tape)
                out, self.last_losses, grads = self._stretch_body(ins, tape, self._wgrad_side(), gt=gt,
                                                                  copy_seeds=self._geometry.current is not None)
                self._stretch_demand[dkey] = (a.off - off0, a.want32 - want0)
                self._backward_levels_pass(tape, grads)
                return out
            while len(graphs) >= STRETCH_MAX_GRAPHS:
                graphs.pop(min(graphs, key=lambda k: graphs[k].last_used))
            sg = graphs[key] = StretchGraph(self, ins, tape, demand)
        self._stretch_clock = getattr(self, "_stretch_clock", 0) + 1
        sg.last_used = self._stretch_clock
        self.store._fresh_wait()
        out, self.last_losses, grads = sg.replay(ins, gt, self._wgrad_side(),
                                                 after_loss=self._after_loss)
        self._ema_version += 1
        self._backward_levels_pass(tape, grads)
        return out

    def _grams_early(self, levels):
        if not GRAM_EARLY or M.DETERMINISTIC or P.WGRAD.stream is None:
            return
        todo = [levels[n]["recs"][-1] for n in GRAM_EARLY if n in levels]
        todo = [r for r in todo if r.get("gram_form") and r.get("in_affine") is not None and "gram_ahead" not in r]
        if not todo:
            return

        def run():
            for r in todo:
                r["gram_ahead"] = M.gram(r["x"], r["in_affine"][:2], r["in_relu"], half=r.get("half"))
        P.on_wgrad_stream(run, *[r["x"] for r in todo])
        P.wgrad_flush()

    def _grams_ahead(self, tape):
        if not GRAMS_AHEAD or M.DETERMINISTIC or not self.overlap_wgrad or not torch.cuda.is_available():
            return
        todo = [t["recs"][-1] for t in tape[:4] if t.get("op") == "sa" and t["recs"][-1].get("gram_form") and t["recs"][-1].get("in_affine") is not None]
        if not todo:
            return

        def run():
            for r in todo:
                r["gram_ahead"] = M.gram(r["x"], r["in_affine"][:2], r["in_relu"], half=r.get("half"))
        with P.WGRAD.on(self._wgrad_side()):
            P.on_wgrad_stream(run, *[r["x"] for r in todo])

    def _backward_levels_pass(self, tape, grads):
        self.check_tape(tape)
        M.arena_begin(self.device)
        try:
            with P.WGRAD.on(self._wgrad_side()):
                self._levels_backward(tape[:4], *grads)
                P.wgrad_join()
        finally:
            M.arena_end()

    def drop_graphs(self):
        self.__dict__.pop("_stretch_graphs", None)
        self.__dict__.pop("_stretch_demand", None)
        self._geometry.drop()

    monitors = None
    last_accuracies = None

    def enable_monitors(self, window=100, tensors_every=0):
        from . import monitors
        self.monitors = monitors.Monitors(self, window, tensors_every)
        self.last_accuracies = None
        return self.monitors

    def disable_monitors(self):
        self.monitors = None
        self.last_accuracies = None

    vote_supervision = None

    def enable_vote_supervision(self, mode="paper"):
        from . import vote_supervision as VS
        if mode not in VS.MODES:
            raise M.L.InvalidArgumentError("enable_vote_supervision: mode must be one of %s, got %r" % (", ".join(VS.MODES), mode))
        if mode == "paper" and self.instance_votes == "instance":
            raise M.L.InvalidArgumentError("enable_vote_supervision: \"paper\" and enable_instance_votes() both write the vote term: "
                                           "disable_instance_votes() first")
        self.vote_supervision = mode

    def disable_vote_supervision(self):
        self.vote_supervision = None

    instance_votes = None

    def enable_instance_votes(self, mode="instance"):
        from . import instance_votes as IV
        if mode not in IV.MODES:
            raise M.L.InvalidArgumentError("enable_instance_votes: mode must be one of %s, got %r" % (", ".join(IV.MODES), mode))
        if mode == "instance" and self.vote_supervision == "paper":
            raise M.L.InvalidArgumentError("enable_instance_votes: enable_vote_supervision(\"paper\") is in force and both write the vote "
                                           "term: disable_vote_supervision() first")
        self.instance_votes = mode

    def disable_instance_votes(self):
        self.instance_votes = None
        self.__dict__.pop("_seed_levels", None)

    def _check_point_box(self, x, gt):
        pb = gt.get("point_box") if hasattr(gt, "get") else None
        want = tuple(x.shape[:2])
        if not (torch.is_tensor(pb) and pb.dtype == torch.int32 and pb.device == x.device and tuple(pb.shape) == want and pb.is_contiguous()):
            raise M.L.InvalidArgumentError(
                "train_step: enable_instance_votes() is in force: gt[\"point_box\"] must be a contiguous int32 tensor of shape %s on %s "
                "(input_pipeline.build_batch_from_labels(..., point_box=True)), got %s"
                % (want, x.device, (tuple(pb.shape), pb.dtype, pb.device) if torch.is_tensor(pb) else type(pb).__name__))

    def _keep_seed_levels(self, tape):
        if self.instance_votes != "instance":
            return
        sa = [t for t in tape[:2] if t.get("op") == "sa" and t.get("fps_idx") is not None]
        if len(sa) != 2:
            raise M.L.VotenetError("enable_instance_votes: the tape does not start with sa1's and sa2's records")
        gg = self._geometry.current
        self._seed_levels = (sa[0]["fps_idx"], sa[1]["fps_idx"], gg, gg.generation if gg is not None else 0)

    proposal_supervision = None

    def enable_proposal_supervision(self, mode="paper"):
        from . import proposal_supervision as PS
        if mode not in PS.MODES:
            raise M.L.InvalidArgumentError("enable_proposal_supervision: mode must be one of %s, got %r" % (", ".join(PS.MODES), mode))
        self.proposal_supervision = mode

    def disable_proposal_supervision(self):
        self.proposal_supervision = None

    def _after_loss(self, out, gt, losses, cot):
        if self.vote_supervision == "paper":
            from . import vote_supervision as VS
            work, supervised = self._loss_tail_buffers(VS, out["votes_xyz"].shape[0], 1)
            VS.paper_vote_loss(out, gt, losses, d_votes=cot["votes_xyz"], supervised=supervised, work=work)
        if self.instance_votes == "instance":
            from . import instance_votes as IV
            idx1, idx2, gg, generation = self._seed_levels
            if gg is not None and gg.generation != generation:
                raise M.L.VotenetError("instance votes: the geometry buffers that hold this step's fps_idx have been overwritten by a later prefetch")
            work, counts = self._loss_tail_buffers(IV, out["votes_xyz"].shape[0], 2)
            IV.instance_vote_loss(out, gt, losses, (idx1, idx2), d_votes=cot["votes_xyz"], counts=counts, work=work)
        if self.proposal_supervision == "paper":
            from . import proposal_supervision as PS
            work, counts = self._loss_tail_buffers(PS, out["proposals_xyz"].shape[0], 3)
            PS.paper_proposal_loss(out, gt, losses, d_xyz=cot["proposals_xyz"], d_out=cot["proposals_output"], counts=counts, work=work)
        if self.monitors is not None:
            self.last_accuracies = self.monitors.after_loss(out, gt, losses)

    def _loss_tail_buffers(self, mod, b, ncounts):
        work = self.__dict__.setdefault("_loss_tail_work", {})
        if (mod, b) not in work:
            work[mod, b] = (mod.workspace(b, self.device), torch.empty(ncounts, dtype=torch.int32, device=self.device))
        return work[mod, b]

    proposal_sampling = None

    def enable_proposal_sampling(self, mode="vote_fps"):
        from . import vote_sampling as VSAMP
        if mode not in VSAMP.MODES:
            raise M.L.InvalidArgumentError("enable_proposal_sampling: mode must be one of %s, got %r" % (", ".join(VSAMP.MODES), mode))
        if mode == "vote_fps":
            n, pr = self.sa2.npoint, self.proposal
            if pr.knn or pr.group_all or not VSAMP.supported(n, pr.npoint, pr.nsample):
                raise M.L.InvalidArgumentError(
                    "enable_proposal_sampling: vote_fps takes 1 to %d votes, 1 to %d clusters and 1 to %d votes per ball-query cluster; "
                    "this network has %d seeds and a proposal module of npoint %r, nsample %r, knn %r, group_all %r"
                    % (VSAMP.MAX_N, VSAMP.MAX_M, VSAMP.MAX_NSAMPLE, n, pr.npoint, pr.nsample, pr.knn, pr.group_all))
        self.proposal_sampling = mode

    def disable_proposal_sampling(self):
        self.proposal_sampling = None

    vote_features = None

    def enable_vote_features(self, mode="unit"):
        from . import unit_votes as UV
        if mode not in UV.MODES:
            raise M.L.InvalidArgumentError("enable_vote_features: mode must be one of %s, got %r" % (", ".join(UV.MODES), mode))
        self.vote_features = mode

    def disable_vote_features(self):
        self.vote_features = None

    step_guard = None

    def enable_step_guard(self):
        from . import step_guard
        self.step_guard = step_guard.StepGuard(self)
        return self.step_guard

    def disable_step_guard(self):
        self.step_guard = None

    def init_optimizer(self, lr=LEARNING_RATE):
        s = self.store
        base = s.flat.data_ptr()
        seg = []
        for name, shape, _ in s._specs:
            a = (s.views[name].data_ptr() - base) // 4
            seg += [a, a + math.prod(shape)]
        self._seg = torch.tensor(seg, dtype=torch.int64, device=self.device)
        self._sumsq = torch.zeros(M.SUMSQ_SLICES * (len(seg) // 2), dtype=torch.float32, device=self.device)
        self._m = torch.zeros_like(s.flat)
        self._v = torch.zeros_like(s.flat)
        self._step = 0
        self._lr = lr

    def set_lr(self, lr):
        lr = float(lr)
        if not (math.isfinite(lr) and lr >= 0.0):
            raise ValueError("set_lr: the learning rate must be finite and >= 0, got %r" % lr)
        if not hasattr(self, "_seg"):
            self.init_optimizer(lr)
        self._lr = lr

    def state_dict(self, optimizer=True):
        return checkpoint.state_dict(self, optimizer)

    def load_state_dict(self, sd, strict=True):
        checkpoint.load_state_dict(self, sd, strict)

    def save(self, path, optimizer=True):
        checkpoint.save(self, path, optimizer)

    def load(self, path, strict=True):
        checkpoint.load(self, path, strict)

    def train_step(self, x, cot=None, world=1, gt=None, next_x=None, feats=None, next_feats=None):
        self._sa1_points(x, feats, "train_step")
        if self.instance_votes == "instance" and gt is not None:
            self._check_point_box(x, gt)
        if not hasattr(self, "_seg"):
            self.init_optimizer()
        self.store.grad.zero_()
        self.store.refresh_transposes(self._side_stream())
        tape = []
        M.arena_begin(self.device, whole_step=True)
        try:
            if getattr(self, "_gsync", None) is None:
                self._gsync = dp.GradSync(self.store, self.store.offset_of("sa3/"))
            if self._stretch_eligible(x, cot, gt):
                out = self._train_step_stretch(x, gt, tape, next_x, **self._feats_kw(feats, next_feats))
            else:
                out = self.forward(x, tape, next_x=next_x, **self._feats_kw(feats, next_feats))
                self._grams_ahead(tape)
                self.update_moving_averages(tape)
                if gt is not None:
                    from . import loss as VL
                    self._keep_seed_levels(tape)
                    self.last_losses, cot = VL.votenet_loss(out, gt)
                    self._after_loss(out, gt, self.last_losses, cot)
                self._gsync.begin()
                if PREFETCH_AFTER >= 5:
                    for nx, nf in self._pair_next(next_x, next_feats):
                        self.prefetch_geometry(nx, nf)
                self.backward(tape, cot)
        finally:
            M.arena_end()
        self.store.invalidate_transposes()
        gscale = self._gsync.finish()
        self._step += 1
        if self.step_guard is not None:
            self.step_guard.apply(self, gscale)
        else:
            M.clip_adam(self._seg, self._sumsq, self.store.flat, self.store.grad, self._m, self._v, self._lr, self._step,
                        grad_scale=gscale)
        if self.monitors is not None:
            self.monitors.after_optimizer(self, gscale, 0.5)
        return out
```

### votenet_amd/pointnet2.py

```python
import math
import threading
from typing import NamedTuple

import torch

from . import mlp as M
from . import tf_grouping, tf_interpolate, tf_sampling


PAD_RAGGED = True
NARROW_FIRST = True
PAD_RAGGED_IN = True
ASSEMBLE_FIRST = True
ASSEMBLE_INLINE = True
HALF_GROUPS = True
FUSE_BN_REDUCE = True


class ParamStore:

    def __init__(self, device):
        self.device = device
        self._specs = []
        self.flat = None
        self.grad = None
        self.views = {}
        self.gviews = {}
        self._tspecs = []
        self._tviews = {}
        self._tflat = self._ttable = None
        self.t_event = None
        self.split = False
        self._split_flat = self._split_t = None
        self.generation = 0
        self._split_gen = -1
        self._split_rows = []
        self._bn_specs = []
        self.bn_flat = None
        self._bn_views = {}
        self._bn_pass = {}
        self._bn_passes = 0

    def want_transpose(self, name, lo=0, hi=None):
        self._tspecs.append((name, lo, hi, "T", 0))

    def want_padded(self, name, pad_to):
        self._tspecs.append((name, 0, None, "P", pad_to))
        self._tspecs.append((name, 0, None, "PT", pad_to))

    def want_padded_rows(self, name, pad_to):
        self._tspecs.append((name, 0, None, "R", pad_to))
        self._tspecs.append((name, 0, None, "RT", pad_to))

    def enable_split(self, on=True):
        self.split = bool(on)
        if not on:
            for im in (self._split_flat, self._split_t, getattr(self, "_split_tf", None)):
                if im is not None:
                    im.close()
            self._split_flat = self._split_t = self._split_tf = None

    def refresh_split(self):
        if not self.split or self.flat is None or not self.flat.is_cuda:
            return
        if self._split_flat is None:
            mats = [v for v in self.views.values() if v.dim() == 2]
            mats += [self.views[name][lo:hi] for name, lo, hi in self._split_rows]
            self._split_flat = M.SplitImages(mats, pieces=2 if (M.FORWARD_H2 and not M.SPLIT_K) else 3)
        self._split_flat.refresh()
        self._split_gen = self.generation

    def rebuild_split(self):
        for name in ("_split_flat", "_split_t", "_split_tf"):
            im = getattr(self, name, None)
            if im is not None:
                im.close()
            setattr(self, name, None)
        self._split_gen = -1
        self.t_event = None
        M.CONFIG_EPOCH += 1

    def ensure_split(self):
        if self.split and self._split_gen != self.generation:
            self.refresh_split()

    def refresh_transposes(self, stream=None):
        if not self._tspecs:
            return
        if self._tflat is None:
            base = self.flat.data_ptr()
            table, total, shapes = [], 0, {}
            for name, lo, hi, kind, pad in self._tspecs:
                v = self.views[name]
                v2 = v if v.dim() == 2 else v.view(1, -1)
                if kind == "PT" and v.dim() != 2:
                    continue
                hi_ = v2.shape[0] if hi is None else hi
                rows, cols = hi_ - lo, v2.shape[1]
                src = (v.data_ptr() - base) // 4 + lo * cols
                if kind == "T":
                    table += [src, total, rows, cols, rows, 1]
                    shp = (cols, rows)
                elif kind == "R":
                    table += [src, total, rows, cols, cols, 0]
                    shp = (pad, cols)
                elif kind == "RT":
                    table += [src, total, rows, cols, pad, 1]
                    shp = (cols, pad)
                elif kind == "P":
                    table += [src, total, rows, cols, pad, 0]
                    shp = (rows, pad) if v.dim() == 2 else (pad,)
                else:
                    table += [src, total, rows, cols, rows, 1]
                    shp = (pad, rows)
                shapes[(name, lo, hi, kind)] = (total, shp)
                n_el = 1
                for d in shp:
                    n_el *= d
                total += (n_el + 3) // 4 * 4
            self._tflat = torch.zeros(total, dtype=torch.float32, device=self.device)
            self._ttable = torch.tensor(table, dtype=torch.int64, device=self.device)
            self._nseg = len(table) // 6
            for key, (off, shp) in shapes.items():
                n_el = 1
                for d in shp:
                    n_el *= d
                self._tviews[key] = self._tflat[off:off + n_el].view(shp)
        from . import _lib as L_
        cur = torch.cuda.current_stream()
        st = stream if stream is not None else cur
        if st is not cur:
            st.wait_stream(cur)
        with M.L.device_guard(self.device), torch.cuda.stream(st):
            L_.check(L_.lib().votenet_transpose_segments(self._nseg, L_.ptr(self._ttable), L_.ptr(self.flat),
                                                         L_.ptr(self._tflat), L_.stream_ptr()))
            if self.split:
                if self._split_t is None:
                    fwd = [v for k, v in self._tviews.items() if v.dim() == 2 and k[3] in ("R", "P")]
                    bwd = [v for k, v in self._tviews.items() if v.dim() == 2 and k[3] not in ("R", "P")]
                    h2 = M.FORWARD_H2 and not M.SPLIT_K
                    self._split_t = M.SplitImages(bwd + ([] if h2 else fwd))
                    self._split_tf = M.SplitImages(fwd, pieces=2) if h2 else None
                self._split_t.refresh()
                if self._split_tf is not None:
                    self._split_tf.refresh()
            self.t_event = torch.cuda.Event()
            self.t_event.record(st)
        self._t_waited = False

    def params_changed(self):
        self.generation += 1
        self.t_event = None

    def invalidate_transposes(self):
        self.params_changed()

    def _fresh(self, key):
        if self.t_event is None and self._tspecs and self.flat is not None and self.flat.is_cuda:
            self.refresh_transposes()
        v = self._tviews.get(key) if self.t_event is not None else None
        if v is None:
            return None
        if not self._t_waited:
            torch.cuda.current_stream().wait_event(self.t_event)
            self._t_waited = True
        return v

    def _fresh_wait(self):
        if self.t_event is None and self._tspecs and self.flat is not None and self.flat.is_cuda:
            self.refresh_transposes()
        if self.t_event is not None and not self._t_waited:
            torch.cuda.current_stream().wait_event(self.t_event)
            self._t_waited = True

    def transposed(self, name, lo=0, hi=None):
        v = self._fresh((name, lo, hi, "T"))
        return v if v is not None else self.views[name][lo:hi].t().contiguous()

    def padded(self, name, pad_to, transpose=False):
        v = self._fresh((name, 0, None, "PT" if transpose else "P"))
        if v is not None:
            return v
        w = self.views[name]
        p = torch.nn.functional.pad(w, (0, pad_to - w.shape[-1]))
        return p.t().contiguous() if transpose else p

    def padded_rows(self, name, pad_to, transpose=False):
        v = self._fresh((name, 0, None, "RT" if transpose else "R"))
        if v is not None:
            return v
        w = self.views[name]
        p = torch.nn.functional.pad(w, (0, 0, 0, pad_to - w.shape[0]))
        return p.t().contiguous() if transpose else p

    def declare(self, name, shape, init):
        self._specs.append((name, tuple(shape), init))

    def bn_block_written(self, name):
        self._bn_passes += 1
        self._bn_pass[name] = self._bn_passes
        return self._bn_passes

    def materialize(self, seed=0):
        offs, total = [], 0
        for _, shape, _ in self._specs:
            offs.append(total)
            total += (math.prod(shape) + 3) // 4 * 4
        self.flat = torch.zeros(total, dtype=torch.float32, device=self.device)
        self.grad = torch.zeros(total, dtype=torch.float32, device=self.device)
        nbn = sum(4 * c for _, c in self._bn_specs)
        self.bn_flat = torch.zeros(max(nbn, 1), dtype=torch.float32, device=self.device)
        o = 0
        for name, c in self._bn_specs:
            self._bn_views[name] = self.bn_flat[o:o + 4 * c].view(4, c)
            o += 4 * c
        gen = torch.Generator(device="cpu").manual_seed(seed)
        for (name, shape, init), off in zip(self._specs, offs):
            n = math.prod(shape)
            v = self.flat[off:off + n].view(shape)
            if init == "he":
                v.copy_((torch.randn(shape, generator=gen) * math.sqrt(2.0 / shape[0])).to(self.device))
            elif init == "ones":
                v.fill_(1.0)
            self.views[name] = v
            self.gviews[name] = self.grad[off:off + n].view(shape)
        return self

    def offset_of(self, prefix):
        for name, _, _ in self._specs:
            if name.startswith(prefix):
                return self.views[name].storage_offset()
        raise KeyError(prefix)

    def __getitem__(self, name):
        return self.views[name]

    def g(self, name):
        return self.gviews[name]

    def numel(self):
        return sum(math.prod(s) for _, s, _ in self._specs)


class Layer:

    def __init__(self, store, name, cin, cout, bn=True, relu=True):
        self.store, self.name, self.cin, self.cout, self.bn, self.relu = store, name, cin, cout, bn, relu
        store.declare(name + "/W", (cin, cout), "he")
        store.want_transpose(name + "/W")
        store.declare(name + "/b", (cout,), "zeros")
        if bn:
            store.declare(name + "/gamma", (cout,), "ones")
            store.declare(name + "/beta", (cout,), "zeros")
            store._bn_specs.append((name, cout))
        self.cout_pad = 0
        if PAD_RAGGED and not bn and cout % 64 != 0 and cin % 32 == 0:
            self.cout_pad = (cout + 63) // 64 * 64
            store.want_padded(name + "/W", self.cout_pad)
            store.want_padded(name + "/b", self.cout_pad)
        self.cin_pad = 0
        if PAD_RAGGED and bn and cin % 32 != 0 and cin > 64 and cout % 64 == 0:
            self.cin_pad = (cin + 63) // 64 * 64
            store.want_padded_rows(name + "/W", self.cin_pad)

    def p(self, k):
        st = self.store
        if st.split and st._split_gen != st.generation:
            st.refresh_split()
        return st[self.name + "/" + k]

    def wT(self, lo=0, hi=None):
        return self.store.transposed(self.name + "/W", lo, hi)

    def gp(self, k):
        return self.store.g(self.name + "/" + k)


def make_mlp(store, scope, cin, widths, prefix="conv", last_plain=False):
    layers = []
    for i, co in enumerate(widths):
        plain = last_plain and i == len(widths) - 1
        layers.append(Layer(store, "%s/%s%d" % (scope, prefix, i), cin, co, bn=not plain, relu=not plain))
        cin = co
    return layers


PRE_LINEAR = True
POOL_IN_EPILOGUE = True
POOL_GRAM_BACKWARD = True
ASSEMBLED_DECOMPOSED = True
class _FrozenBN(threading.local):
    table = None


_FROZEN = _FrozenBN()


class frozen_bn:
    def __init__(self, table):
        self.table = table

    def __enter__(self):
        self.prev, _FROZEN.table = _FROZEN.table, self.table
        return self.table

    def __exit__(self, *a):
        _FROZEN.table = self.prev
        return False


def _with_inverse(idx):
    yield idx
    yield from getattr(idx, "_inv", None) or ()


class NarrowRows(NamedTuple):
    u8: torch.Tensor
    mom: torch.Tensor
    half: object = None
# ... 250 lines not shown
            self._keep.append(thunks)
        else:
            for t in tensors:
                t.record_stream(self.stream)
        torch.cuda.set_stream(self.stream)
        try:
            for f in thunks:
                f()
        finally:
            torch.cuda.set_stream(main)
        self._pending = True

    def run(self, fn, *tensors):
        tensors = [t for t in tensors if isinstance(t, torch.Tensor)]
        if self._defer is not None:
            self._defer.append((fn, tensors))
        elif self.stream is None:
            fn()
        elif WGRAD_BATCH and not self._fine:
            self._deferred.append((fn, tensors))
        else:
            self.hand_over([fn], tensors)

    def flush(self):
        if self._deferred:
            if self.stream is None:
                for f, _ in self._deferred:
                    f()
            else:
                self.hand_over([f for f, _ in self._deferred], [t for _, ts in self._deferred for t in ts])
            self._deferred.clear()

    def join(self):
        self.flush()
        if self.stream is not None and self._pending:
            ev = self._event()
            ev.record(self.stream)
            torch.cuda.current_stream().wait_event(ev)
            self._pending = False


WGRAD = WgradLane()
on_wgrad_stream, wgrad_flush, wgrad_join = WGRAD.run, WGRAD.flush, WGRAD.join


def check_bn_block(rec):
    n = rec.get("bn_pass")
    if n is not None and rec["layer"].store._bn_pass.get(rec["layer"].name) != n:
        raise M.L.VotenetError("BatchNorm statistics of layer %s: the record belongs to forward pass %d, the layer's persistent block was "
                               "rewritten by a later training-mode pass (run backward / update_moving_averages before the next forward of "
                               "the same net)" % (rec["layer"].name, n))


def bn_of(rec):
    return rec["scale"], rec["shift"], rec["mean"], rec["var"]


def below_of(rec, with_z=False):
    if with_z:
        return rec["z"], rec["scale"], rec["shift"], rec["mean"], rec["var"], rec["layer"].relu
    return rec["scale"], rec["shift"], rec["mean"], rec["var"], rec["layer"].relu


def tail_of(rec):
    Lr = rec["layer"]
    return (rec["rows"], Lr.p("gamma"), Lr.gp("gamma"), Lr.gp("beta"))


def _bwd_pooled_gram(r, below, gout, argmax, zsel, k, want_da):
    L = r["layer"]
    x, aff, W, b, half = r["x"], r["in_affine"], L.p("W"), L.p("b"), r.get("half")
    coef = M.bn_backward_reduce_pool(gout, zsel, *bn_of(r), L.relu, tail=tail_of(r))
    mm = M.pool_dgrad_prepare(W, b, coef, x.shape[0]) if want_da else None

    def wgrad():
        G = r.pop("gram_ahead", None)
        if G is None:
            G = M.gram(x, aff[:2], r["in_relu"], half=half)
        M.pool_wgrad(x, r["in_scale"], r["in_shift"], r["in_relu"], G, W, b, coef, L.relu, gout, argmax, zsel, k, L.gp("W"), half=half)
    on_wgrad_stream(wgrad, x, aff, coef, gout, argmax, zsel)
    if not want_da:
        return None, None, False
    if below is not None and below["layer"].bn and below["z"] is x:
        da_below, coef_below = M.pool_dgrad(x, r["in_scale"], r["in_shift"], r["in_relu"], W, b, L.wT(), coef, L.relu, gout, argmax, zsel, k,
                                            below=below_of(below), mm=mm, below_tail=tail_of(below), half=half)
        return da_below, coef_below, False
    return M.pool_dgrad(x, r["in_scale"], r["in_shift"], r["in_relu"], W, b, L.wT(), coef, L.relu, gout, argmax, zsel, k, mm=mm,
                        half=half), None, False


def _bwd_above_assembled(r, r0, da, coef, pool, want_da):
    L, z = r["layer"], r["z"]
    geo, Pt, wx, half = r0["geo"], r0["P"], r0["wx"], r0["half"]
    on_wgrad_stream(lambda: M.assembled_wgrad_bn(geo, Pt, wx, r["in_scale"], r["in_shift"], r["in_relu"], z, coef, L.relu, da, L.gp("W"),
                                                 half=half), geo, Pt, z, coef, da)
    if ASSEMBLED_DECOMPOSED and half is not None and r0["layer"].bn and r0.get("cntv") is not None:
        da0 = M.dgrad_bn_half(z, coef, L.relu, L.wT(), da, half)
        return FirstLayerGrad(da=da0, relu=r0["layer"].relu, bn=bn_of(r0), tail=tail_of(r0)), None, True
    da0, coef0 = M.assembled_dgrad_bn_reduce(z, coef, L.relu, L.wT(), da, geo, Pt, wx, below_of(r0), below_tail=tail_of(r0), half=half)
    return da0, coef0, False


def _bwd_above_narrow(r, r0, da, coef, pool, want_da):
    L, z = r["layer"], r["z"]
    L0, u8, mom, half = r0["layer"], r0["u8"], r0["mom"], r0["half"]
    w0, b0 = L0.p("W"), L0.p("b")
    on_wgrad_stream(lambda: M.narrow_wgrad_bn(u8, w0, b0, r["in_scale"], r["in_shift"], r["in_relu"], z, coef, L.relu, da, L.gp("W"),
                                              half=half), u8, z, coef, da)
    coef0, ug = M.narrow_dgrad_bn_reduce(z, coef, L.relu, L.wT(), da, u8, w0, b0, below_of(r0), tail=tail_of(r0), half=half,
                                         mask=r.get("mask0") if M.NARROW_MASK else None)
    M.narrow_wgrad_first(mom, ug, coef0, w0, b0, L0.gp("W"))
    return None, None, True


def _bwd_padded_input(r, below, da, coef, pool, want_da):
    L, z = r["layer"], r["z"]

    def wgrad():
        G = M._zeros_f32((L.cin_pad, L.cout), z.device)
        M.wgrad_dense_bn(r["x"], z, coef, L.relu, G, da=da)
        gw = L.gp("W")
        M.row_segments(L.cin, [(gw, gw, G[:L.cin])])
    on_wgrad_stream(wgrad, r["x"], z, coef, da)
    if not want_da:
        return None, None, False
    return M.dgrad_bn(z, coef, L.relu, L.store.padded_rows(L.name + "/W", L.cin_pad, transpose=True), da=da)[:, :L.cin], None, False


def _bwd_fused_dense(r, below, da, coef, pool, want_da):
    L, z = r["layer"], r["z"]
    src = dict(gout=da, argmax=pool[0], k=pool[1]) if pool else dict(da=da)
    on_wgrad_stream(lambda: M.wgrad_dense_bn(r["x"], z, coef, L.relu, L.gp("W"), in_scale=r["in_scale"], in_shift=r["in_shift"],
                                             in_relu=r["in_relu"], **src), r["x"], z, coef, da, pool[0] if pool else None)
    if not want_da:
        return None, None, False
    if FUSE_BN_REDUCE and not pool and below is not None and below["layer"].bn and below["z"] is r["x"]:
        da_below, coef_below = M.dgrad_bn(z, coef, L.relu, L.wT(), da=da, below=below_of(below, with_z=True), below_tail=tail_of(below))
        return da_below, coef_below, False
    return M.dgrad_bn(z, coef, L.relu, L.wT(), **src), None, False


def _bwd_first_fused(r, below, da, coef, pool, want_da):
    return FirstLayerGrad(da=da, coef=coef, relu=r["layer"].relu), None, True


def _bwd_unfused(r, below, da, coef, pool, want_da):
    dz = M.bn_backward_apply(r["z"], coef, r["layer"].relu, da, argmax=pool[0] if pool else None, k=pool[1] if pool else 0)
    return _bwd_written_out(r, below, dz, want_da)


def _bwd_written_out(r, below, dz, want_da):
    L = r["layer"]
    if below is None and r["kind"] == "gather":
        return FirstLayerGrad(dz=dz), None, True
    on_wgrad_stream(lambda: M.wgrad_dense(r["x"], dz, L.gp("W"), r["in_scale"], r["in_shift"], r["in_relu"]), dz, r.get("x"))
    return (M.linear_dense(dz, L.wT(), want_stats=False)[0] if want_da else None), None, False


def _bwd_plain(r, below, dz, want_da, g_padded):
    L = r["layer"]
    on_wgrad_stream(lambda: M.bias_grad(dz, L.gp("b")), dz)
    if not r.get("padded"):
        return _bwd_written_out(r, below, dz, want_da)
    if g_padded is not None and g_padded.shape[1] == L.cout_pad:
        dzp = g_padded
    else:
        dzp = torch.empty((dz.shape[0], L.cout_pad), dtype=torch.float32, device=dz.device)
        M.row_segments(dz.shape[0], [(dzp[:, :L.cout], dz, None), (dzp[:, L.cout:], None, None)])

    def wgrad():
        G = M._zeros_f32((L.cin, L.cout_pad), dzp.device)
        M.wgrad_dense(r["x"], dzp, G, r["in_scale"], r["in_shift"], r["in_relu"])
        gw = L.gp("W")
        M.row_segments(L.cin, [(gw, gw, G[:, :L.cout])])
    on_wgrad_stream(wgrad, dzp, r.get("x"))
    if not want_da:
        return None, None, False
    return M.linear_dense(dzp, L.store.padded(L.name + "/W", L.cout_pad, transpose=True), want_stats=False)[0], None, False


def mlp_chain_backward(recs, g, mode, argmax=None, k=0, need_input_grad=True, zsel=None, g_padded=None):
    for r in recs:
        check_bn_block(r)
    last = len(recs) - 1
    da = g
    coef_from_above = None
    for i in range(last, -1, -1):
        r, below = recs[i], recs[i - 1] if i > 0 else None
        L = r["layer"]
        pooled = mode == "pool" and i == last
        want_da = i > 0 or need_input_grad
        if pooled and r.get("gram_form") and zsel is not None:
            step = _bwd_pooled_gram(r, below, da, argmax, zsel, k, want_da)
        elif not L.bn:
            step = _bwd_plain(r, below, da, want_da, g_padded if i == last else None)
        else:
            coef = coef_from_above
            if coef is None:
                coef = M.bn_backward_reduce(r["z"], *bn_of(r), L.relu, da, argmax=argmax if pooled else None, k=k if pooled else 0,
                                            tail=tail_of(r))
            if r.get("assembled"):
                arm = _bwd_above_assembled
            elif r.get("narrow"):
                arm = _bwd_above_narrow
            elif r.get("cin_padded") and not pooled and M.dgrad_bn_supported(r["rows"], L.cout, L.cin_pad):
                arm = _bwd_padded_input
            elif r["kind"] == "dense" and (not want_da or M.dgrad_bn_supported(r["rows"], L.cout, r["x"].shape[1])):
                arm = _bwd_fused_dense
            elif i == 0 and r["kind"] == "assembled":
                arm = _bwd_first_fused
            elif i == 0 and r["kind"] == "gather" and PRE_LINEAR and not pooled and r["feat"] is not None and \
                    M.group_linear_backward_supported(L.cout, r["idx"].shape[2]):
                arm = _bwd_first_fused
            else:
                arm = _bwd_unfused
            step = arm(r, below, da, coef, (argmax, k) if pooled else None, want_da)
        da, coef_from_above, done = step
        if done:
            break
    return da


def add_rows(a, b):
    c = a.shape[-1]
    rows = a.numel() // c
    out = torch.empty(a.shape, dtype=torch.float32, device=a.device)

    def two_d(t):
        if t.is_contiguous():
            return t.view(rows, c)
        if M.L.pitched_rows(t):
            return t.as_strided((rows, c), (t.stride(1), 1), t.storage_offset())
        return t.contiguous().view(rows, c)
    M.row_segments(rows, [(out.view(rows, c), two_d(a), two_d(b))])
    return out


def _group_indices(radius, nsample, xyz, new_xyz, knn):
    if knn:
        _, idx = tf_grouping.knn_point(nsample, xyz, new_xyz)
        return M.attach_inverse(idx, xyz.shape[1]), torch.full(idx.shape[:2], nsample, dtype=torch.int32, device=idx.device)
    idx, cnt = tf_grouping.query_ball_point(radius, nsample, xyz, new_xyz)
    return M.attach_inverse(idx, xyz.shape[1]), cnt


def sample_and_group(npoint, radius, nsample, xyz, sample_xyz=None, knn=False):
    fps_idx = tf_sampling.farthest_point_sample(npoint, sample_xyz if sample_xyz is not None else xyz)
    new_xyz = tf_sampling.gather_point(xyz, fps_idx)
    idx, pts_cnt = _group_indices(radius, nsample, xyz, new_xyz, knn)
    return fps_idx, new_xyz, idx, pts_cnt


POOLINGS = ("max", "avg", "weighted_avg", "max_and_avg")


class SAModule:

    def __init__(self, store, scope, npoint, radius, nsample, cin, mlp, mlp2=None, knn=False, prefix="conv", leaf=False, pooling="max",
                 group_all=False):
        if pooling not in POOLINGS:
            raise ValueError("SAModule: pooling must be one of %s, got %r" % (", ".join(POOLINGS), pooling))
        self.pooling, self.group_all = pooling, bool(group_all)
        self.plain_pool = self.group_all or pooling != "max"
        if self.group_all:
            npoint, radius, nsample, knn = 1, None, None, False
        self.npoint, self.radius, self.nsample, self.knn = npoint, radius, nsample, knn
        self.leaf, self.cin = leaf, cin
        self.mlp = make_mlp(store, scope, 3 + cin, mlp, prefix)
        store.want_transpose(self.mlp[0].name + "/W", 3, None)
        store._split_rows.append((self.mlp[0].name + "/W", 3, None))
        store.want_transpose(self.mlp[0].name + "/W", 0, 3)
        pooled = 2 * mlp[-1] if pooling == "max_and_avg" else mlp[-1]
        self.mlp2 = make_mlp(store, scope, pooled, mlp2, "conv_post_", last_plain=True) if mlp2 else None

    def narrow(self, rows):
        m = self.mlp
        return bool(NARROW_FIRST and not self.plain_pool and self.leaf and len(m) >= 3 and m[0].bn and m[1].bn and m[0].relu and
                    M.narrow_supported(rows, 3 + self.cin, m[0].cout, m[1].cout))

    def assembled(self, b, n):
        m = self.mlp
        if self.plain_pool:
            return False
        rows = b * self.npoint * self.nsample
        return bool(ASSEMBLE_FIRST and PRE_LINEAR and not M.DETERMINISTIC and self.cin > 0 and not self.narrow(rows) and len(m) >= 3
                    and m[0].bn and m[1].bn and m[0].relu and M.assembled_supported(rows, m[0].cout, m[1].cout)
                    and M.group_linear_backward_supported(m[0].cout, self.nsample) and b * n * m[0].cout * 4 < 2 ** 32)

    def half_groups(self, b, n):
        m = self.mlp
        if not (HALF_GROUPS and not self.plain_pool and not M.DETERMINISTIC and not self.knn and self.nsample == 64 and len(m) == 3 and m[2].bn and POOL_IN_EPILOGUE
                and POOL_GRAM_BACKWARD and (b * self.npoint) % 8 == 0 and M.pool_backward_supported(m[1].cout, m[2].cout, 64)):
            return False
        return bool(self.narrow(b * self.npoint * 64) or (m[1].cout == 128 and self.assembled(b, n)))

    def geometry(self, xyz, sample_xyz=None, fps_idx=None, points=None, ahead=True, grouped=None):
        if grouped is not None:
            fps_idx, new_xyz, idx, pts_cnt = grouped
            idx = M.attach_inverse(idx, xyz.shape[1])
            ahead = False
        elif fps_idx is None:
            fps_idx, new_xyz, idx, pts_cnt = sample_and_group(self.npoint, self.radius, self.nsample, xyz, sample_xyz, self.knn)
        else:
            new_xyz = tf_sampling.gather_point(xyz, fps_idx)
            idx, pts_cnt = _group_indices(self.radius, self.nsample, xyz, new_xyz, self.knn)
        first = None
        if (points is not None or self.cin == 0) and self.narrow(xyz.shape[0] * self.npoint * self.nsample):
            if ahead and self.half_groups(xyz.shape[0], xyz.shape[1]):
                half = M.half_groups(pts_cnt)
                first = NarrowRows(*M.narrow_rows_half(xyz, new_xyz, points, idx, pts_cnt, half), half)
            else:
                first = NarrowRows(*M.narrow_rows(xyz, new_xyz, points, idx))
        elif (ahead or ASSEMBLE_INLINE) and self.half_groups(xyz.shape[0], xyz.shape[1]):
            half = M.half_groups(pts_cnt, device_count=not ahead)
            first = AssembledRows(*M.assemble_rows_half(xyz, new_xyz, idx, pts_cnt, half), half)
            M.half_sort_rows(half, xyz.shape[0] * xyz.shape[1])
        elif self.assembled(xyz.shape[0], xyz.shape[1]) and (ahead or ASSEMBLE_INLINE):
            first = AssembledRows(*M.assemble_rows(xyz, new_xyz, idx, pts_cnt=pts_cnt, in_pass=not ahead))
        return SAGeometry(fps_idx, new_xyz, idx, pts_cnt, first)

    def forward(self, xyz, points, sample_xyz=None, tape=None, geom=None):
        if self.plain_pool:
            return self._forward_plain_pool(xyz, points, sample_xyz, tape, geom)
        b = xyz.shape[0]
        geom = geom if geom is not None else self.geometry(xyz, sample_xyz, points=points)
        fps_idx, new_xyz, idx, pts_cnt, ahead = geom.fps_idx, geom.new_xyz, geom.idx, geom.pts_cnt, geom.first
        recs = []
        rows = b * self.npoint * self.nsample
        if self.narrow(rows):
            r = ahead if isinstance(ahead, NarrowRows) else NarrowRows(*M.narrow_rows(xyz, new_xyz, points, idx))
            half = r.half.resolve() if r.half is not None else None
            first = NarrowInput(half.u8 if half is not None else r.u8, r.mom, half)
        elif points is not None and self.assembled(b, xyz.shape[1]) and (isinstance(ahead, AssembledRows) or ASSEMBLE_INLINE):
            r = ahead if isinstance(ahead, AssembledRows) else AssembledRows(*M.assemble_rows(xyz, new_xyz, idx, pts_cnt=pts_cnt, in_pass=True))
            half = r.half.resolve() if r.half is not None else None
            first = AssembledInput(xyz, new_xyz, points, idx, half.geo if half is not None else r.geo, r.cntv, r.mom, half)
        else:
            first = GatherInput(xyz, new_xyz, points, idx)
        z, pend = mlp_chain_forward(self.mlp, rows, first, recs, pool_k=self.nsample, keep_z=tape is not None)
        if recs[-1]["pool"] is not None:
            res = M.bn_pool_finalize(recs[-1]["pool"], None, None, True, want_argmax=tape is not None, bn=pend,
                                     want_zsel=tape is not None and bool(recs[-1].get("gram_form")), half=recs[-1].get("half"))
            pooled, argmax, zsel = res if len(res) == 3 else (res[0], res[1], None)
        else:
            zsel = None
            sc, sh = pend.finalize()
            pooled, argmax = M.bn_relu_max(z, self.nsample, sc, sh, True, want_argmax=tape is not None)
        recs2 = []
        out = pooled
        if self.mlp2:
            z2, _ = mlp_chain_forward(self.mlp2, b * self.npoint, DenseInput(pooled), recs2)
            out = z2
        if tape is not None:
            tape.append(dict(op="sa", module=self, recs=recs, recs2=recs2, argmax=argmax, zsel=zsel, fps_idx=fps_idx, idx=idx, pts_cnt=pts_cnt,
                             xyz=xyz, points=points, new_xyz=new_xyz, b=b))
        return new_xyz, out.reshape(b, self.npoint, -1), idx


    def backward(self, rec, g_out, need_feat_grad=True, need_xyz_grad=False):
        if self.plain_pool:
            return self._backward_plain_pool(rec, g_out, need_feat_grad, need_xyz_grad)
        b = rec["b"]
        g = g_out.reshape(b * self.npoint, -1).contiguous()
        if self.mlp2:
            g = mlp_chain_backward(rec["recs2"], g, "plain", need_input_grad=True)
        need_feat = need_feat_grad and rec["points"] is not None
        h = mlp_chain_backward(rec["recs"], g, "pool", argmax=rec["argmax"], k=self.nsample, need_input_grad=need_feat,
                               zsel=rec.get("zsel"))
        if rec["recs"][0]["kind"] == "narrow":
            if need_feat or need_xyz_grad:
                raise ValueError("SAModule(leaf=True): the narrow first layer keeps no per-row gradient; build the module with leaf=False")
            return None, None
        return self._first_layer_backward(rec, h, need_feat, need_xyz_grad)

    def _forward_plain_pool(self, xyz, points, sample_xyz, tape, geom):
        b, n = xyz.shape[:2]
        if self.group_all:
            fps_idx = pts_cnt = None
            new_xyz = torch.zeros((b, 1, 3), dtype=torch.float32, device=xyz.device)
            idx = torch.arange(n, dtype=torch.int32, device=xyz.device).view(1, 1, n).expand(b, 1, n).contiguous()
            m, k = 1, n
            x = xyz.reshape(b * n, 3)
            if points is not None:
                c = points.shape[2]
                x = torch.empty((b * n, 3 + c), dtype=torch.float32, device=xyz.device)
                M.row_segments(b * n, [(x[:, :3], xyz.reshape(b * n, 3), None), (x[:, 3:], points.reshape(b * n, c), None)])
            first = DenseInput(x)
        else:
            geom = geom if geom is not None else self.geometry(xyz, sample_xyz)
            fps_idx, new_xyz, idx, pts_cnt = geom.fps_idx, geom.new_xyz, geom.idx, geom.pts_cnt
            m, k = self.npoint, self.nsample
            first = GatherInput(xyz, new_xyz, points, idx)
        rows = b * m * k
        recs = []
        z, pend = mlp_chain_forward(self.mlp, rows, first, recs)
        sc, sh = pend.finalize()
        w = None
        if self.pooling == "weighted_avg":
            w = M.sa_pool_weights(xyz, None, None) if self.group_all else M.sa_pool_weights(xyz, new_xyz, idx)
        pooled, argmax = M.bn_relu_pool(z, k, sc, sh, self.mlp[-1].relu, self.pooling, w=w, want_argmax=tape is not None)
        recs2 = []
        out = pooled
        if self.mlp2:
            out, _ = mlp_chain_forward(self.mlp2, b * m, DenseInput(pooled), recs2)
        if tape is not None:
            tape.append(dict(op="sa", module=self, recs=recs, recs2=recs2, argmax=argmax, zsel=None, fps_idx=fps_idx, idx=idx,
                             pts_cnt=pts_cnt, xyz=xyz, points=points, new_xyz=new_xyz, b=b, m=m, k=k, weights=w))
        return new_xyz, out.reshape(b, m, -1), idx

    def _backward_plain_pool(self, rec, g_out, need_feat_grad, need_xyz_grad):
        b, m, k = rec["b"], rec["m"], rec["k"]
        g = g_out.reshape(b * m, -1).contiguous()
        if self.mlp2:
            g = mlp_chain_backward(rec["recs2"], g, "plain", need_input_grad=True)
        last = rec["recs"][-1]
        c = last["layer"].cout
        need_feat = need_feat_grad and rec["points"] is not None
        dy = M.sa_pool_grad(g, k, c, self.pooling, w=rec["weights"], argmax=rec["argmax"])
        dv = None
        if need_xyz_grad and self.pooling == "weighted_avg":
            new_xyz, idx = (None, None) if self.group_all else (rec["new_xyz"], rec["idx"])
            dv = M.sa_pool_weights_grad(rec["xyz"], new_xyz, idx, last["z"], last["scale"], last["shift"], last["layer"].relu, g,
                                        rec["weights"])
        xyz = rec["xyz"]
        n = xyz.shape[1]
        if not self.group_all:
            h = mlp_chain_backward(rec["recs"], dy, "act", need_input_grad=need_feat)
            return self._first_layer_backward(rec, h, need_feat, need_xyz_grad, d_rows_xyz_extra=dv)
        dx = mlp_chain_backward(rec["recs"], dy, "act", need_input_grad=need_feat or need_xyz_grad)
        d_feat = d_xyz = None
        if need_feat:
            c_in = rec["points"].shape[2]
            d_feat = torch.empty((b * n, c_in), dtype=torch.float32, device=xyz.device)
            M.row_segments(b * n, [(d_feat, dx[:, 3:3 + c_in], None)])
            d_feat = d_feat.view(b, n, c_in)
        if need_xyz_grad:
            d_xyz = torch.empty((b * n, 3), dtype=torch.float32, device=xyz.device)
            M.row_segments(b * n, [(d_xyz, dx[:, :3], dv)])
            d_xyz = d_xyz.view(b, n, 3)
        return d_feat, d_xyz

    def _first_layer_backward(self, rec, h, need_feat, need_xyz_grad, d_rows_xyz_extra=None):
        r0 = rec["recs"][0]
        L0 = r0["layer"]
        W, gW = L0.p("W"), L0.gp("W")
        xyz, new_xyz, feat, idx, pts_cnt = r0["xyz"], r0["new_xyz"], r0["feat"], r0["idx"], rec["pts_cnt"]
        b, n = xyz.shape[:2]
        cout = W.shape[1]
        d_feat = d_xyz = None
        if h.dz is not None:
            S, dz = _first_written_out(rec, h.dz, gW), h.dz
        elif r0["kind"] == "assembled" and r0.get("half") is not None:
            S, dz, d_xyz = _first_piece_layout(rec, h, W, gW, need_xyz_grad)
        elif r0["kind"] == "assembled":
            S, dz = M.group_linear_backward_assembled(xyz, new_xyz, idx, pts_cnt, r0["P"], r0["wx"], h.da, h.coef, h.relu, gW[:3],
                                                      want_dz=need_xyz_grad)
        else:
            S, dz = M.group_linear_backward(xyz, new_xyz, idx, pts_cnt, r0["z"], h.da, h.coef, h.relu, gW[:3], want_dz=need_xyz_grad)
        if feat is not None:
            c = feat.shape[2]
            if PRE_LINEAR:
                S2, feat2 = S.view(b * n, cout), feat.reshape(b * n, c)
                on_wgrad_stream(lambda: M.wgrad_dense(feat2, S2, gW[3:]), S2, feat2)
                if need_feat:
                    d2, _ = M.linear_dense(S2, L0.wT(3, None), want_stats=False)
                    d_feat = d2.view(b, n, c)
            else:
                on_wgrad_stream(lambda: M.wgrad_gather(xyz, new_xyz, feat, idx, dz, gW), dz, feat)
                if need_feat:
                    d_rows_feat, _ = M.linear_dense(dz, L0.wT(3, None), want_stats=False)
                    d_feat, _, _ = M.group_concat_grad(d_rows_feat, None, idx, pts_cnt, n, c)
        if need_xyz_grad and d_xyz is None:
            d_rows_xyz = M.rows_dot3(dz, W[:3])
            if d_rows_xyz_extra is not None:
                d_rows_xyz = add_rows(d_rows_xyz, d_rows_xyz_extra)
            _, d_xyz, d_new = M.group_concat_grad(None, d_rows_xyz, idx, pts_cnt, n, 0)
            d_xyz = tf_sampling.gather_point_grad_raw(n, rec["fps_idx"], d_new, into=d_xyz)
        return d_feat, d_xyz


def _first_written_out(rec, dz, gW):
    r0 = rec["recs"][0]
    xyz, new_xyz, feat, idx = r0["xyz"], r0["new_xyz"], r0["feat"], r0["idx"]
    if feat is None or PRE_LINEAR:
        on_wgrad_stream(lambda: M.wgrad_gather(xyz, new_xyz, None, idx, dz, gW), dz)
    if feat is not None and PRE_LINEAR:
        return M.group_concat_grad(dz, None, idx, rec["pts_cnt"], xyz.shape[1], gW.shape[1])[0]
    return None


def _first_piece_layout(rec, h, W, gW, need_xyz_grad):
    r0 = rec["recs"][0]
    half = r0["half"]
    b, n = r0["xyz"].shape[:2]
    if h.coef is None:
        S, coef = M.group_linear_backward_decomposed(half, b, n, r0["P"], r0["wx"], h.da, h.bn, h.relu, h.tail, r0["cntv"], r0["mom"],
                                                     gW[:3], defer=on_wgrad_stream)
    else:
        S, coef = M.group_linear_backward_half(half, b, n, r0["P"], r0["wx"], h.da, h.coef, h.relu, gW[:3]), h.coef
    if not need_xyz_grad:
        return S, None, None
    d_xyz = M.rows_dot3(S.view(b * n, W.shape[1]), W[:3]).view(b, n, 3)
    d_new = M.rows_dot3(M.half_centre_sums(half, r0["P"], r0["wx"], h.da, coef, h.relu), W[:3]).view(b, -1, 3)
    return S, None, tf_sampling.gather_point_grad_raw(n, rec["fps_idx"], d_new, into=d_xyz)


class SAModuleMSG:

    def __init__(self, store, scope, npoint, radius_list, nsample_list, cin, mlp_list):
        self.npoint, self.cin = npoint, cin
        self.scales = [SAModule(store, scope, npoint, r, k, cin, mlp, prefix="conv%d_" % i)
                       for i, (r, k, mlp) in enumerate(zip(radius_list, nsample_list, mlp_list))]
        self.widths = [mlp[-1] for mlp in mlp_list]

    @staticmethod
    def reference_rows(w):
        return torch.cat([w[3:], w[:3]], 0)

    @staticmethod
    def from_reference_rows(w):
        return torch.cat([w[-3:], w[:-3]], 0)

    def forward(self, xyz, points, tape=None):
        fps_idx = tf_sampling.farthest_point_sample(self.npoint, xyz)
        subs, outs, new_xyz = [], [], None
        for sc in self.scales:
            sub = [] if tape is not None else None
            new_xyz, o, _ = sc.forward(xyz, points, tape=sub, geom=sc.geometry(xyz, fps_idx=fps_idx))
            outs.append(o)
            subs.append(sub[0] if sub else None)
        if tape is not None:
            tape.append(dict(op="sa_msg", module=self, subs=subs))
        return new_xyz, torch.cat(outs, -1)

    def backward(self, rec, g_out, need_feat_grad=True):
        d_feat, o = None, 0
        for sc, sub, w in zip(self.scales, rec["subs"], self.widths):
            d, _ = sc.backward(sub, g_out[..., o:o + w].contiguous(), need_feat_grad=need_feat_grad)
            o += w
            if d is not None:
                d_feat = d if d_feat is None else d_feat + d
        return d_feat


class FPModule:

    def __init__(self, store, scope, cin1, cin2, mlp):
        self.mlp = make_mlp(store, scope, cin1 + cin2, mlp, "conv_")

    @staticmethod
    def geometry(xyz1, xyz2):
        dist, idx = tf_interpolate.three_nn(xyz1, xyz2)
        return FPGeometry(M.attach_inverse(idx, xyz2.shape[1], always=tf_interpolate.GATHER_GRAD), tf_interpolate.three_nn_weights(dist))

    def forward(self, xyz1, xyz2, points1, points2, tape=None, geom=None):
        b, n1 = xyz1.shape[:2]
        geom = geom if geom is not None else self.geometry(xyz1, xyz2)
        idx, weight = geom.idx, geom.weight
        if points1 is not None:
            x = tf_interpolate.three_interpolate_concat(points2, idx, weight, points1)
        else:
            x = tf_interpolate.three_interpolate(points2, idx, weight)
        rows = b * n1
        recs = []
        z, pend = mlp_chain_forward(self.mlp, rows, DenseInput(x.view(rows, -1)), recs)
        y = M.bn_relu(z, None, None, True, bn=pend)
        if tape is not None:
            tape.append(dict(op="fp", module=self, recs=recs, idx=idx, weight=weight, m=xyz2.shape[1],
                             c2=points2.shape[2], c1=0 if points1 is None else points1.shape[2], b=b, n1=n1))
        return y.view(b, n1, -1)

    def backward(self, rec, dy):
        b, n1, c1, c2 = rec["b"], rec["n1"], rec["c1"], rec["c2"]
        d_x = mlp_chain_backward(rec["recs"], dy.reshape(b * n1, -1).contiguous(), "act", need_input_grad=True)
        d_x3 = d_x.view(b, n1, c2 + c1)
        d_p1 = d_x3[:, :, c2:] if c1 else None
        d_p2 = tf_interpolate.three_interpolate_grad_raw(rec["m"], rec["idx"], rec["weight"], d_x3[:, :, :c2])
        return d_p1, d_p2
```

Measured before the change: 2297.

## Fuse vote gather, ball query, half-groups and row assembly; add fused loss kernel

Adds a side library that runs, for the vote-grouping SA layer, the gather of sampled centers, the ball query, the half-group layout, row assembly and sort counting as one launch sequence. This replaces separate gather_point, group_indices, half_groups, assemble and sort kernels. It also adds a fused loss kernel that replaces the pitched loss launch. Shared device bodies move into a header so both paths reuse them. The cost targeted is launch overhead and intermediate global-memory round trips, at the price of more code and extra zeroed workspace.

```diff
diff --git a/include/votenet_vote_group.h b/include/votenet_vote_group.h
--- /dev/null
+++ b/include/votenet_vote_group.h
@@ -0,0 +1,30 @@
+#ifndef VOTENET_VOTE_GROUP_H
+#define VOTENET_VOTE_GROUP_H
+
+#include <stddef.h>
+
+#ifdef __cplusplus
+extern "C" {
+#endif
+
+const char *votenet_votegroup_last_error(void);
+
+int votenet_vote_group_supported(int b, int n, int m);
+
+int votenet_vote_group(int b, int n, int m, float radius, const float *xyz, const int *fps_idx, float *new_xyz, int *idx, int *pts_cnt,
+                       int *pos, int *hc, float *wh, int *nh, float *geo, long long *cntv, double *moments, int *work, int *order,
+                       void *stream);
+
+int votenet_loss_fused(int b, int n_seeds, int n_prop, int n_box, int nh, int ns, int nc, const float *seeds_xyz,
+                       const float *votes_xyz, const float *proposals_xyz, const float *proposals_output, long output_pitch,
+                       const float *bboxes_xyz, const float *bboxes_lwh, const float *bboxes_roty,
+                       const int *semantic_labels, const int *heading_labels, const float *heading_residuals,
+                       const int *size_labels, const float *size_residuals, float pos_thr, float neg_thr, float *losses,
+                       float *d_votes_xyz, float *d_proposals_xyz, float *d_proposals_output, float *workspace, void *stream);
+size_t votenet_loss_fused_workspace_floats(int b);
+
+#ifdef __cplusplus
+}
+#endif
+
+#endif
diff --git a/votenet_amd/_lib.py b/votenet_amd/_lib.py
--- a/votenet_amd/_lib.py
+++ b/votenet_amd/_lib.py
@@ -22,6 +22,7 @@
     "instbox": "votenet_instance_boxes.h",
     "instvote": "votenet_instance_votes.h",
     "unitvote": "votenet_unit_votes.h",
+    "votegroup": "votenet_vote_group.h",
 }
 _side = {}
 
diff --git a/votenet_amd/csrc/half.hip b/votenet_amd/csrc/half.hip
--- a/votenet_amd/csrc/half.hip
+++ b/votenet_amd/csrc/half.hip
@@ -1,165 +1,20 @@
-#include "mlp_types.h"
+#include "half_pieces.h"
 
 namespace votenet {
-
-constexpr int PS = kPiece, NP = kBallPieces, TP = kTilePieces;
-
-__device__ __forceinline__ int kept_pieces(int cnt)
-{
-    const int c = cnt < 1 ? 1 : cnt;
-    const int k = (c + PS - 1) / PS;
-    return k > NP ? NP : k;
-}
 
 __global__ __launch_bounds__(1024) void half_groups_kernel(int G, const int *__restrict__ pts_cnt, int *__restrict__ pos, int *__restrict__ hc,
                                                            float *__restrict__ wh, int *__restrict__ nh_out, int *nh_host)
 {
-    __shared__ int s_wave[16];
-    __shared__ int s_carry;
-    const int tid = threadIdx.x, lane = tid & 63, wv = tid >> 6;
-    if (tid == 0) s_carry = 0;
-    __syncthreads();
-    for (int c0 = 0; c0 < G; c0 += 1024) {
-        const int c = c0 + tid;
-        const int kc = c < G ? kept_pieces(pts_cnt[c]) : 1;
-        const int mine = kc - 1;
-        int x = mine;
-#pragma unroll
-        for (int off = 1; off < 64; off <<= 1) {
-            const int t = __shfl_up(x, off);
-            if (lane >= off) x += t;
-        }
-        if (lane == 63) s_wave[wv] = x;
-        __syncthreads();
-        int base = s_carry;
-        for (int w = 0; w < wv; w++) base += s_wave[w];
-        int p = base + x - mine;
-        if (c < G) {
-            hc[c] = c * NP;
-            for (int j = 1; j < NP; j++) {
-                if (j < kc) {
-                    hc[G + p] = c * NP + j;
-                    pos[c * (NP - 1) + j - 1] = p++;
-                } else {
-                    pos[c * (NP - 1) + j - 1] = -1;
-                }
-            }
-        }
-        __syncthreads();
-        if (tid == 1023) s_carry = base + x;
-        __syncthreads();
-    }
-    if (tid == 0) {
-        int n2 = s_carry;
-        for (int c = 0; c < G && ((G + n2) % TP) != 0; c++)
-            for (int j = 1; j < NP && ((G + n2) % TP) != 0; j++)
-                if (pos[c * (NP - 1) + j - 1] < 0) {
-                    pos[c * (NP - 1) + j - 1] = n2;
-                    hc[G + n2] = c * NP + j;
-                    n2++;
-                }
-        s_carry = n2;
-        nh_out[0] = G + n2;
-        if (nh_host != nullptr) {
-            nh_host[0] = G + n2;
-            __threadfence_system();
-        }
-    }
-    __syncthreads();
-    const int nh = G + s_carry;
-    for (int q = tid; q < nh; q += 1024) {
-        float w = 1.0f;
-        if (q < G) {
-            int kc = 1;
-            for (int j = 1; j < NP; j++) kc += pos[q * (NP - 1) + j - 1] >= 0 ? 1 : 0;
-            w = 1.0f + (float)(PS * (NP - kc));
-        }
-        wh[q] = w;
-    }
-}
-
-__device__ __forceinline__ double half_shfl_xor_f64(double v, int m)
-{
-    int lo = __double2loint(v), hi = __double2hiint(v);
-    lo = __shfl_xor(lo, m);
-    hi = __shfl_xor(hi, m);
-    return __hiloint2double(hi, lo);
-}
-__device__ __forceinline__ long long half_fixed(float v) { return (long long)((double)v * 4294967296.0); }
-
-__device__ __forceinline__ void half_sort_runs(unsigned prow, bool live, int lane, int &run_start, int &run_len)
-{
-    const unsigned prev = __shfl_up(prow, 1);
-    const bool prev_live = __shfl_up((int)live, 1) != 0;
-    const bool starts = live && (lane == 0 || !prev_live || prev != prow);
-    const unsigned long long sm = __ballot(starts), lm = __ballot(live);
-    const unsigned long long below = sm & ((lane == 63) ? ~0ull : ((1ull << (lane + 1)) - 1ull));
-    run_start = below ? 63 - __builtin_clzll(below) : 0;
-    const unsigned long long after = (sm | ~lm) & ~((run_start == 63) ? ~0ull : ((1ull << (run_start + 1)) - 1ull));
-    const int end = after ? __builtin_ctzll(after) : 64;
-    run_len = end - run_start;
-}
+    half_groups_body(G, pts_cnt, pos, hc, wh, nh_out, nh_host);
+}
+
 __global__ __launch_bounds__(256) void assemble_rows_half_kernel(const int *__restrict__ nh_dev, long max_rows, int n, int groups_per_scene, const float *__restrict__ xyz,
                                                                  const float *__restrict__ new_xyz, const int *__restrict__ idx,
                                                                  const int *__restrict__ pts_cnt, const int *__restrict__ hc,
                                                                  float4 *__restrict__ geo, long long *__restrict__ cntv,
                                                                  double *__restrict__ moments, int *__restrict__ count)
 {
-    __shared__ double red[4][9];
-    double acc[9];
-#pragma unroll
-    for (int i = 0; i < 9; i++) acc[i] = 0.0;
-    const long rows = (long)nh_dev[0] * PS;
-    for (long r0 = (long)blockIdx.x * 256; r0 < max_rows; r0 += (long)gridDim.x * 256) {
-        const long r = r0 + threadIdx.x;
-        const bool live = r < rows;
-        unsigned my_prow = 0;
-        if (!live && r < max_rows) geo[r] = make_float4(0.f, 0.f, 0.f, __uint_as_float(0u));
-        if (live) {
-        const int q = (int)(r / PS), s = (int)(r % PS);
-        const int code = hc[q];
-        const int c = code / NP;
-        const int k = (code % NP) * PS + s;
-        const int id = idx[(size_t)c * 64 + k];
-        const unsigned prow = ((unsigned)c / (unsigned)groups_per_scene) * (unsigned)n + (unsigned)id;
-        const float dx = xyz[(size_t)prow * 3 + 0] - new_xyz[(size_t)c * 3 + 0];
-        const float dy = xyz[(size_t)prow * 3 + 1] - new_xyz[(size_t)c * 3 + 1];
-        const float dz = xyz[(size_t)prow * 3 + 2] - new_xyz[(size_t)c * 3 + 2];
-        geo[r] = make_float4(dx, dy, dz, __uint_as_float(prow));
-        my_prow = prow;
-        int cnt = pts_cnt[c];
-        if (cnt < 1) cnt = 1;
-        if (k < cnt) {
-            const long long mult = (k == 0) ? (long long)(64 - cnt + 1) : 1LL;
-            if (cntv) {
-                unsigned long long *cv = reinterpret_cast<unsigned long long *>(cntv + (size_t)prow * 4);
-                atomicAdd(cv + 0, (unsigned long long)mult);
-                atomicAdd(cv + 1, (unsigned long long)(mult * half_fixed(dx)));
-                atomicAdd(cv + 2, (unsigned long long)(mult * half_fixed(dy)));
-                atomicAdd(cv + 3, (unsigned long long)(mult * half_fixed(dz)));
-            }
-            const double m = (double)mult, x = dx, y = dy, z = dz;
-            acc[0] += m * x; acc[1] += m * y; acc[2] += m * z;
-            acc[3] += m * x * x; acc[4] += m * x * y; acc[5] += m * x * z; acc[6] += m * y * y; acc[7] += m * y * z; acc[8] += m * z * z;
-        }
-        }
-        if (count) {
-            int rs, rl;
-            half_sort_runs(my_prow, live, threadIdx.x & 63, rs, rl);
-            if (live && rs == (int)(threadIdx.x & 63)) atomicAdd(&count[my_prow], rl);
-        }
-    }
-    if (!moments) return;
-#pragma unroll
-    for (int i = 0; i < 9; i++) {
-        double v = acc[i];
-#pragma unroll
-        for (int m = 32; m >= 1; m >>= 1) v += half_shfl_xor_f64(v, m);
-        if ((threadIdx.x & 63) == 0) red[threadIdx.x >> 6][i] = v;
-    }
-    __syncthreads();
-    if (threadIdx.x < 9)
-        unsafeAtomicAdd(&moments[threadIdx.x], (red[0][threadIdx.x] + red[1][threadIdx.x]) + (red[2][threadIdx.x] + red[3][threadIdx.x]));
+    assemble_rows_half_body<false>(nh_dev, max_rows, n, groups_per_scene, xyz, new_xyz, idx, pts_cnt, hc, geo, cntv, moments, count, nullptr);
 }
 
 __global__ __launch_bounds__(256) void narrow_rows_half_kernel(const int *__restrict__ nh_dev, int n, int groups_per_scene, int c,
@@ -293,44 +148,7 @@
 }
 __global__ __launch_bounds__(1024) void half_sort_scan_kernel(int npts, int *__restrict__ count)
 {
-    __shared__ int s_wave[16];
-    const int tid = threadIdx.x, lane = tid & 63, wv = tid >> 6;
-    const int per = (npts + 1023) / 1024;
-    const int b0 = tid * per < npts ? tid * per : npts, e0 = b0 + per < npts ? b0 + per : npts;
-    constexpr int KEEP = 16;
-    int v[KEEP];
-    int tot = 0;
-    if (per <= KEEP) {
-#pragma unroll
-        for (int i = 0; i < KEEP; i++) v[i] = b0 + i < e0 ? count[b0 + i] : 0;
-#pragma unroll
-        for (int i = 0; i < KEEP; i++) tot += v[i];
-    } else {
-        for (int p = b0; p < e0; p++) tot += count[p];
-    }
-    int x = tot;
-#pragma unroll
-    for (int off = 1; off < 64; off <<= 1) {
-        const int t = __shfl_up(x, off);
-        if (lane >= off) x += t;
-    }
-    if (lane == 63) s_wave[wv] = x;
-    __syncthreads();
-    int run = x - tot;
-    for (int w = 0; w < wv; w++) run += s_wave[w];
-    if (per <= KEEP) {
-#pragma unroll
-        for (int i = 0; i < KEEP; i++) {
-            if (b0 + i < e0) count[b0 + i] = run;
-            run += v[i];
-        }
-        return;
-    }
-    for (int p = b0; p < e0; p++) {
-        const int c = count[p];
-        count[p] = run;
-        run += c;
-    }
+    half_sort_scan_body(npts, count);
 }
 __global__ __launch_bounds__(256) void half_sort_fill_kernel(const int *__restrict__ nh_dev, const float4 *__restrict__ geo,
                                                              int *__restrict__ cursor, int *__restrict__ order)
diff --git a/votenet_amd/csrc/half_pieces.h b/votenet_amd/csrc/half_pieces.h
--- /dev/null
+++ b/votenet_amd/csrc/half_pieces.h
@@ -0,0 +1,219 @@
+#pragma once
+#include "mlp_types.h"
+
+namespace votenet {
+
+constexpr int PS = kPiece, NP = kBallPieces, TP = kTilePieces;
+
+__device__ __forceinline__ int kept_pieces(int cnt)
+{
+    const int c = cnt < 1 ? 1 : cnt;
+    const int k = (c + PS - 1) / PS;
+    return k > NP ? NP : k;
+}
+
+__device__ __forceinline__ void half_groups_body(int G, const int *__restrict__ pts_cnt, int *__restrict__ pos, int *__restrict__ hc,
+                                                 float *__restrict__ wh, int *__restrict__ nh_out, int *nh_host, int *count = nullptr,
+                                                 const int *__restrict__ idx = nullptr, int n = 0, int groups_per_scene = 1)
+{
+    __shared__ int s_wave[16];
+    __shared__ int s_carry;
+    const int tid = threadIdx.x, lane = tid & 63, wv = tid >> 6;
+    if (tid == 0) s_carry = 0;
+    __syncthreads();
+    for (int c0 = 0; c0 < G; c0 += 1024) {
+        const int c = c0 + tid;
+        const int kc = c < G ? kept_pieces(pts_cnt[c]) : 1;
+        const int mine = kc - 1;
+        int x = mine;
+#pragma unroll
+        for (int off = 1; off < 64; off <<= 1) {
+            const int t = __shfl_up(x, off);
+            if (lane >= off) x += t;
+        }
+        if (lane == 63) s_wave[wv] = x;
+        __syncthreads();
+        int base = s_carry;
+        for (int w = 0; w < wv; w++) base += s_wave[w];
+        int p = base + x - mine;
+        if (c < G) {
+            hc[c] = c * NP;
+            for (int j = 1; j < NP; j++) {
+                if (j < kc) {
+                    hc[G + p] = c * NP + j;
+                    pos[c * (NP - 1) + j - 1] = p++;
+                } else {
+                    pos[c * (NP - 1) + j - 1] = -1;
+                }
+            }
+        }
+        __syncthreads();
+        if (tid == 1023) s_carry = base + x;
+        __syncthreads();
+    }
+    if (tid == 0) {
+        int n2 = s_carry;
+        for (int c = 0; c < G && ((G + n2) % TP) != 0; c++)
+            for (int j = 1; j < NP && ((G + n2) % TP) != 0; j++)
+                if (pos[c * (NP - 1) + j - 1] < 0) {
+                    pos[c * (NP - 1) + j - 1] = n2;
+                    hc[G + n2] = c * NP + j;
+                    n2++;
+                    if (count) atomicAdd(&count[(size_t)(c / groups_per_scene) * n + idx[(size_t)c * 64]], PS);
+                }
+        s_carry = n2;
+        nh_out[0] = G + n2;
+        if (nh_host != nullptr) {
+            nh_host[0] = G + n2;
+            __threadfence_system();
+        }
+    }
+    __syncthreads();
+    const int nh = G + s_carry;
+    for (int q = tid; q < nh; q += 1024) {
+        float w = 1.0f;
+        if (q < G) {
+            int kc = 1;
+            for (int j = 1; j < NP; j++) kc += pos[q * (NP - 1) + j - 1] >= 0 ? 1 : 0;
+            w = 1.0f + (float)(PS * (NP - kc));
+        }
+        wh[q] = w;
+    }
+}
+
+__device__ __forceinline__ double half_shfl_xor_f64(double v, int m)
+{
+    int lo = __double2loint(v), hi = __double2hiint(v);
+    lo = __shfl_xor(lo, m);
+    hi = __shfl_xor(hi, m);
+    return __hiloint2double(hi, lo);
+}
+__device__ __forceinline__ long long half_fixed(float v) { return (long long)((double)v * 4294967296.0); }
+
+__device__ __forceinline__ void half_sort_runs(unsigned prow, bool live, int lane, int &run_start, int &run_len)
+{
+    const unsigned prev = __shfl_up(prow, 1);
+    const bool prev_live = __shfl_up((int)live, 1) != 0;
+    const bool starts = live && (lane == 0 || !prev_live || prev != prow);
+    const unsigned long long sm = __ballot(starts), lm = __ballot(live);
+    const unsigned long long below = sm & ((lane == 63) ? ~0ull : ((1ull << (lane + 1)) - 1ull));
+    run_start = below ? 63 - __builtin_clzll(below) : 0;
+    const unsigned long long after = (sm | ~lm) & ~((run_start == 63) ? ~0ull : ((1ull << (run_start + 1)) - 1ull));
+    const int end = after ? __builtin_ctzll(after) : 64;
+    run_len = end - run_start;
+}
+
+template <bool FILL>
+__device__ __forceinline__ void assemble_rows_half_body(const int *__restrict__ nh_dev, long max_rows, int n, int groups_per_scene,
+                                                        const float *__restrict__ xyz, const float *__restrict__ new_xyz,
+                                                        const int *__restrict__ idx, const int *__restrict__ pts_cnt,
+                                                        const int *__restrict__ hc, float4 *__restrict__ geo, long long *__restrict__ cntv,
+                                                        double *__restrict__ moments, int *__restrict__ count, int *__restrict__ order)
+{
+    __shared__ double red[4][9];
+    double acc[9];
+#pragma unroll
+    for (int i = 0; i < 9; i++) acc[i] = 0.0;
+    const long rows = (long)nh_dev[0] * PS;
+    for (long r0 = (long)blockIdx.x * 256; r0 < max_rows; r0 += (long)gridDim.x * 256) {
+        const long r = r0 + threadIdx.x;
+        const bool live = r < rows;
+        unsigned my_prow = 0;
+        if (!live && r < max_rows) geo[r] = make_float4(0.f, 0.f, 0.f, __uint_as_float(0u));
+        if (live) {
+        const int q = (int)(r / PS), s = (int)(r % PS);
+        const int code = hc[q];
+        const int c = code / NP;
+        const int k = (code % NP) * PS + s;
+        const int id = idx[(size_t)c * 64 + k];
+        const unsigned prow = ((unsigned)c / (unsigned)groups_per_scene) * (unsigned)n + (unsigned)id;
+        const float dx = xyz[(size_t)prow * 3 + 0] - new_xyz[(size_t)c * 3 + 0];
+        const float dy = xyz[(size_t)prow * 3 + 1] - new_xyz[(size_t)c * 3 + 1];
+        const float dz = xyz[(size_t)prow * 3 + 2] - new_xyz[(size_t)c * 3 + 2];
+        geo[r] = make_float4(dx, dy, dz, __uint_as_float(prow));
+        my_prow = prow;
+        int cnt = pts_cnt[c];
+        if (cnt < 1) cnt = 1;
+        if (k < cnt) {
+            const long long mult = (k == 0) ? (long long)(64 - cnt + 1) : 1LL;
+            if (cntv) {
+                unsigned long long *cv = reinterpret_cast<unsigned long long *>(cntv + (size_t)prow * 4);
+                atomicAdd(cv + 0, (unsigned long long)mult);
+                atomicAdd(cv + 1, (unsigned long long)(mult * half_fixed(dx)));
+                atomicAdd(cv + 2, (unsigned long long)(mult * half_fixed(dy)));
+                atomicAdd(cv + 3, (unsigned long long)(mult * half_fixed(dz)));
+            }
+            const double m = (double)mult, x = dx, y = dy, z = dz;
+            acc[0] += m * x; acc[1] += m * y; acc[2] += m * z;
+            acc[3] += m * x * x; acc[4] += m * x * y; acc[5] += m * x * z; acc[6] += m * y * y; acc[7] += m * y * z; acc[8] += m * z * z;
+        }
+        }
+        if (count) {
+            int rs, rl;
+            half_sort_runs(my_prow, live, threadIdx.x & 63, rs, rl);
+            if (FILL) {
+                int base = 0;
+                if (live && rs == (int)(threadIdx.x & 63)) base = atomicAdd(&count[my_prow], rl);
+                base = __shfl(base, rs);
+                if (live) order[base + ((int)(threadIdx.x & 63) - rs)] = (int)r;
+            } else {
+                if (live && rs == (int)(threadIdx.x & 63)) atomicAdd(&count[my_prow], rl);
+            }
+        }
+    }
+    if (!moments) return;
+#pragma unroll
+    for (int i = 0; i < 9; i++) {
+        double v = acc[i];
+#pragma unroll
+        for (int m = 32; m >= 1; m >>= 1) v += half_shfl_xor_f64(v, m);
+        if ((threadIdx.x & 63) == 0) red[threadIdx.x >> 6][i] = v;
+    }
+    __syncthreads();
+    if (threadIdx.x < 9)
+        unsafeAtomicAdd(&moments[threadIdx.x], (red[0][threadIdx.x] + red[1][threadIdx.x]) + (red[2][threadIdx.x] + red[3][threadIdx.x]));
+}
+
+__device__ __forceinline__ void half_sort_scan_body(int npts, int *__restrict__ count)
+{
+    __shared__ int s_wave[16];
+    const int tid = threadIdx.x, lane = tid & 63, wv = tid >> 6;
+    const int per = (npts + 1023) / 1024;
+    const int b0 = tid * per < npts ? tid * per : npts, e0 = b0 + per < npts ? b0 + per : npts;
+    constexpr int KEEP = 16;
+    int v[KEEP];
+    int tot = 0;
+    if (per <= KEEP) {
+#pragma unroll
+        for (int i = 0; i < KEEP; i++) v[i] = b0 + i < e0 ? count[b0 + i] : 0;
+#pragma unroll
+        for (int i = 0; i < KEEP; i++) tot += v[i];
+    } else {
+        for (int p = b0; p < e0; p++) tot += count[p];
+    }
+    int x = tot;
+#pragma unroll
+    for (int off = 1; off < 64; off <<= 1) {
+        const int t = __shfl_up(x, off);
+        if (lane >= off) x += t;
+    }
+    if (lane == 63) s_wave[wv] = x;
+    __syncthreads();
+    int run = x - tot;
+    for (int w = 0; w < wv; w++) run += s_wave[w];
+    if (per <= KEEP) {
+#pragma unroll
+        for (int i = 0; i < KEEP; i++) {
+            if (b0 + i < e0) count[b0 + i] = run;
+            run += v[i];
+        }
+        return;
+    }
+    for (int p = b0; p < e0; p++) {
+        const int c = count[p];
+        count[p] = run;
+        run += c;
+    }
+}
+
+}
diff --git a/votenet_amd/csrc/loss.hip b/votenet_amd/csrc/loss.hip
--- a/votenet_amd/csrc/loss.hip
+++ b/votenet_amd/csrc/loss.hip
@@ -1,5 +1,6 @@
 #include "common.h"
 #include "nearest_box.h"
+#include "loss_terms.h"
 
 namespace votenet {
 
@@ -7,45 +8,6 @@
 #define LOSS_ABL 0
 #endif
 constexpr int LOSS_T = 1024;
-constexpr int LOSS_MAXC = 32;
-constexpr int LOSS_NACC = 12;
-
-struct LossArgs {
-    int b, n, p, bb, nh, ns, nc;
-    const float *seeds, *votes, *pxyz, *pout;
-    const float *gxyz, *glwh, *groty;
-    const int *sem, *hlab, *slab;
-    const float *hres, *sres;
-    float pos_thr, neg_thr;
-    float *losses, *d_votes, *d_pxyz, *d_pout;
-    long pout_pitch;
-};
-
-__device__ __forceinline__ float huber(float e, float &grad)
-{
-    const float a = fabsf(e);
-    grad = a <= 1.0f ? e : (e > 0.0f ? 1.0f : -1.0f);
-    return a <= 1.0f ? 0.5f * e * e : a - 0.5f;
-}
-
-__device__ __forceinline__ float softmax_ce(const float *lg, int c, int label, float *probs)
-{
-    float m = lg[0];
-    for (int i = 1; i < c; i++) m = fmaxf(m, lg[i]);
-    float s = 0.0f;
-    for (int i = 0; i < c; i++) {
-        probs[i] = expf(lg[i] - m);
-        s += probs[i];
-    }
-    if ((unsigned)label >= (unsigned)c) {
-        const float nan = __uint_as_float(0x7FC00000u);
-        for (int i = 0; i < c; i++) probs[i] = nan;
-        return nan;
-    }
-    const float inv = 1.0f / s;
-    for (int i = 0; i < c; i++) probs[i] = probs[i] * inv - (i == label ? 1.0f : 0.0f);
-    return logf(s) + m - lg[label];
-}
 
 
 __global__ __launch_bounds__(256) void votenet_loss_count_kernel(LossArgs A, int *counts)
@@ -279,7 +241,7 @@
 
 using namespace votenet;
 
-extern "C" size_t votenet_loss_workspace_floats(int b) { return 4 + (size_t)(b > 0 ? b : 0) * LOSS_NACC; }
+extern "C" size_t votenet_loss_workspace_floats(int b) { return loss_workspace_floats(b); }
 
 extern "C" int votenet_loss_pitched(int b, int n_seeds, int n_prop, int n_box, int nh, int ns, int nc, const float *seeds_xyz,
                             const float *votes_xyz, const float *proposals_xyz, const float *proposals_output, long output_pitch,
diff --git a/votenet_amd/csrc/loss_terms.h b/votenet_amd/csrc/loss_terms.h
--- /dev/null
+++ b/votenet_amd/csrc/loss_terms.h
@@ -0,0 +1,54 @@
+#pragma once
+#include <hip/hip_runtime.h>
+
+namespace votenet {
+
+constexpr int LOSS_MAXC = 32;
+constexpr int LOSS_NACC = 12;
+constexpr int LOSS_FUSED_WGS = 32;
+
+__host__ __device__ inline size_t loss_ticket_ints(int b) { return ((size_t)(b > 0 ? b : 0) + 3) & ~(size_t)3; }
+inline size_t loss_workspace_floats(int b)
+{
+    const size_t nb = (size_t)(b > 0 ? b : 0);
+    return 4 + nb * LOSS_NACC + loss_ticket_ints(b) + nb * LOSS_FUSED_WGS * LOSS_NACC;
+}
+
+struct LossArgs {
+    int b, n, p, bb, nh, ns, nc;
+    const float *seeds, *votes, *pxyz, *pout;
+    const float *gxyz, *glwh, *groty;
+    const int *sem, *hlab, *slab;
+    const float *hres, *sres;
+    float pos_thr, neg_thr;
+    float *losses, *d_votes, *d_pxyz, *d_pout;
+    long pout_pitch;
+};
+
+__device__ __forceinline__ float huber(float e, float &grad)
+{
+    const float a = fabsf(e);
+    grad = a <= 1.0f ? e : (e > 0.0f ? 1.0f : -1.0f);
+    return a <= 1.0f ? 0.5f * e * e : a - 0.5f;
+}
+
+__device__ __forceinline__ float softmax_ce(const float *lg, int c, int label, float *probs)
+{
+    float m = lg[0];
+    for (int i = 1; i < c; i++) m = fmaxf(m, lg[i]);
+    float s = 0.0f;
+    for (int i = 0; i < c; i++) {
+        probs[i] = expf(lg[i] - m);
+        s += probs[i];
+    }
+    if ((unsigned)label >= (unsigned)c) {
+        const float nan = __uint_as_float(0x7FC00000u);
+        for (int i = 0; i < c; i++) probs[i] = nan;
+        return nan;
+    }
+    const float inv = 1.0f / s;
+    for (int i = 0; i < c; i++) probs[i] = probs[i] * inv - (i == label ? 1.0f : 0.0f);
+    return logf(s) + m - lg[label];
+}
+
+}
diff --git a/votenet_amd/csrc/votegroup/vote_group.hip b/votenet_amd/csrc/votegroup/vote_group.hip
--- /dev/null
+++ b/votenet_amd/csrc/votegroup/vote_group.hip
@@ -0,0 +1,424 @@
+#include "../common.h"
+#include "../error_text.h"
+#include "../ball_threshold.h"
+#include "../half_pieces.h"
+#include "../nearest_box.h"
+#include "../loss_terms.h"
+#include "../scene_fold.h"
+
+#pragma GCC visibility push(default)
+#include "../../../include/votenet_vote_group.h"
+#pragma GCC visibility pop
+
+namespace votenet {
+
+static thread_local ErrorText g_vg_err;
+#define VG_REQUIRE(cond, ...) VN_REQUIRE_IN(::votenet::g_vg_err, cond, __VA_ARGS__)
+
+constexpr int VG_MAX_N = 2048;
+constexpr int VG_WAVES = 8;
+constexpr int VG_K = 64;
+
+__global__ __launch_bounds__(VG_WAVES * 64) void vote_ball_kernel(int n, int m, float thr, const float *__restrict__ xyz,
+                                                                  const int *__restrict__ fps_idx, float *__restrict__ new_xyz,
+                                                                  int *__restrict__ idx, int *__restrict__ pts_cnt, int *__restrict__ count)
+{
+    __shared__ float s_pts[VG_MAX_N * 3];
+    __shared__ int s_row[VG_WAVES][VG_K];
+    const int tid = threadIdx.x, lane = lane_id(), w = wave_id_uniform(), sc = blockIdx.y;
+    const float *__restrict__ pts = xyz + (size_t)sc * n * 3;
+    for (int i = tid; i < n * 3; i += VG_WAVES * 64) s_pts[i] = pts[i];
+    __syncthreads();
+    const int q = blockIdx.x * VG_WAVES + w;
+    if (q >= m) return;
+    const size_t c = (size_t)sc * m + q;
+    const int pk = __builtin_amdgcn_readfirstlane(min(max(fps_idx[c], 0), n - 1));
+    const float qx = s_pts[pk * 3 + 0], qy = s_pts[pk * 3 + 1], qz = s_pts[pk * 3 + 2];
+    if (lane < 3) new_xyz[c * 3 + lane] = s_pts[pk * 3 + lane];
+    const unsigned long long below = (1ull << lane) - 1ull;
+    int cnt = 0, first = 0;
+    for (int base = 0; base < n && cnt < VG_K; base += 64) {
+        const int k = base + lane;
+        const bool valid = k < n;
+        const int kk = valid ? k : 0;
+        const float dx = qx - s_pts[kk * 3 + 0], dy = qy - s_pts[kk * 3 + 1], dz = qz - s_pts[kk * 3 + 2];
+        const float s = dx * dx + dy * dy + dz * dz;
+        const bool hit = valid && s < thr;
+        const unsigned long long mask = __ballot(hit);
+        if (mask) {
+            const int at = cnt + __popcll(mask & below);
+            if (hit && at < VG_K) s_row[w][at] = k;
+            if (cnt == 0) first = base + __ffsll((long long)mask) - 1;
+            cnt += __popcll(mask);
+        }
+    }
+    const int cn = cnt < VG_K ? cnt : VG_K;
+    __builtin_amdgcn_fence(__ATOMIC_RELEASE, "wavefront");
+    __builtin_amdgcn_wave_barrier();
+    __builtin_amdgcn_fence(__ATOMIC_ACQUIRE, "wavefront");
+    const int id = lane < cn ? s_row[w][lane] : first;
+    idx[c * VG_K + lane] = id;
+    if (lane == 0) pts_cnt[c] = cn;
+    const bool live = lane < kept_pieces(cn) * PS;
+    const unsigned prow = (unsigned)sc * (unsigned)n + (unsigned)id;
+    int rs, rl;
+    half_sort_runs(prow, live, lane, rs, rl);
+    if (live && rs == lane) atomicAdd(&count[prow], rl);
+}
+
+__global__ __launch_bounds__(1024) void vote_scans_kernel(int G, int n, int m, int npts, const int *__restrict__ pts_cnt, int *__restrict__ pos,
+                                                          int *__restrict__ hc, float *__restrict__ wh, int *__restrict__ nh_out,
+                                                          const int *__restrict__ idx, int *count)
+{
+    half_groups_body(G, pts_cnt, pos, hc, wh, nh_out, nullptr, count, idx, n, m);
+    __syncthreads();
+    half_sort_scan_body(npts, count);
+}
+
+__global__ __launch_bounds__(256) void vote_rows_kernel(const int *__restrict__ nh_dev, long max_rows, int n, int groups_per_scene,
+                                                        const float *__restrict__ xyz, const float *__restrict__ new_xyz,
+                                                        const int *__restrict__ idx, const int *__restrict__ pts_cnt,
+                                                        const int *__restrict__ hc, float4 *__restrict__ geo, long long *__restrict__ cntv,
+                                                        double *__restrict__ moments, int *__restrict__ cursor, int *__restrict__ order)
+{
+    assemble_rows_half_body<true>(nh_dev, max_rows, n, groups_per_scene, xyz, new_xyz, idx, pts_cnt, hc, geo, cntv, moments, cursor, order);
+}
+
+constexpr int LF_T = 256;
+constexpr int LF_S = LOSS_FUSED_WGS;
+constexpr int LF_G = 32;
+constexpr int LF_PW = LF_T / LF_G;
+
+static_assert(SCENE_FOLD_INTS == 4, "loss_workspace_floats (loss_terms.h) lays scene_fold's table at the workspace's start");
+
+__device__ __forceinline__ float group_softmax_ce(const float *lg, int c, int label, int l, float &prob)
+{
+    const float x = l < c ? lg[l] : -INFINITY;
+    float m = x;
+#pragma unroll
+    for (int off = LF_G / 2; off > 0; off >>= 1) m = fmaxf(m, __shfl_xor(m, off, LF_G));
+    const float e = l < c ? expf(x - m) : 0.0f;
+    float s = e;
+#pragma unroll
+    for (int off = LF_G / 2; off > 0; off >>= 1) s += __shfl_xor(s, off, LF_G);
+    if ((unsigned)label >= (unsigned)c) {
+        prob = __uint_as_float(0x7FC00000u);
+        return prob;
+    }
+    const float inv = 1.0f / s;
+    prob = e * inv - (l == label ? 1.0f : 0.0f);
+    return logf(s) + m - lg[label];
+}
+
+__global__ __launch_bounds__(LF_T) void votenet_loss_fused_kernel(LossArgs A, int *ws)
+{
+    __shared__ float s_box[LOSS_MAXBOX][8];
+    __shared__ float s_red[LF_T / 64][LOSS_NACC];
+    __shared__ int s_cnt[LF_T / 64][2];
+    __shared__ float s_dual[LOSS_MAXBOX][3];
+    __shared__ int s_dualp[LOSS_MAXBOX];
+    __shared__ int s_last;
+    const int tid = threadIdx.x, lane = tid & 63, wave = tid >> 6, nwave = LF_T / 64;
+    const int b = blockIdx.x / LF_S, sub = blockIdx.x % LF_S;
+    const int B = A.b, N = A.n, P = A.p, BB = A.bb, NH = A.nh, NS = A.ns, NC = A.nc;
+    const int W = 5 + 2 * NH + 4 * NS + NC;
+    int *sticket = ws + SCENE_FOLD_INTS + (size_t)B * LOSS_NACC;
+    float *partial = reinterpret_cast<float *>(sticket + loss_ticket_ints(B));
+    int n_pos = 0, n_neg = 0;
+    for (int sc = 0; sc < B; sc++) {
+        __syncthreads();
+        for (int j = tid; j < BB; j += LF_T)
+            for (int k = 0; k < 3; k++) s_box[j][k] = A.gxyz[(sc * BB + j) * 3 + k];
+        __syncthreads();
+        for (int pq = tid; pq < P; pq += LF_T) {
+            const int q = sc * P + pq;
+            int g;
+            const float best = nearest_box(s_box, BB, A.pxyz[q * 3 + 0], A.pxyz[q * 3 + 1], A.pxyz[q * 3 + 2], g);
+            n_pos += best < A.pos_thr;
+            n_neg += best > A.neg_thr;
+        }
+    }
+    for (int off = 32; off > 0; off >>= 1) {
+        n_pos += __shfl_down(n_pos, off);
+        n_neg += __shfl_down(n_neg, off);
+    }
+    if (lane == 0) {
+        s_cnt[wave][0] = n_pos;
+        s_cnt[wave][1] = n_neg;
+    }
+    __syncthreads();
+    n_pos = n_neg = 0;
+    for (int w = 0; w < nwave; w++) {
+        n_pos += s_cnt[w][0];
+        n_neg += s_cnt[w][1];
+    }
+    const float inv_np = 1.0f / (float)n_pos, inv_nn = 1.0f / (float)n_neg;
+    for (int j = tid; j < BB; j += LF_T) {
+        const int e = b * BB + j;
+        s_box[j][0] = A.gxyz[e * 3 + 0];
+        s_box[j][1] = A.gxyz[e * 3 + 1];
+        s_box[j][2] = A.gxyz[e * 3 + 2];
+        s_box[j][3] = A.glwh[e * 3 + 0] * 0.5f;
+        s_box[j][4] = A.glwh[e * 3 + 1] * 0.5f;
+        s_box[j][5] = A.glwh[e * 3 + 2] * 0.5f;
+        s_box[j][6] = cosf(-A.groty[e]);
+        s_box[j][7] = sinf(-A.groty[e]);
+    }
+    __syncthreads();
+    float acc[LOSS_NACC];
+#pragma unroll
+    for (int i = 0; i < LOSS_NACC; i++) acc[i] = 0.0f;
+    const float inv_bbb = 1.0f / (float)(B * BB);
+    for (int j = wave; j < BB; j += nwave) {
+        const float gx = s_box[j][0], gy = s_box[j][1], gz = s_box[j][2];
+        float best = INFINITY;
+        int bp = 0x7FFFFFFF;
+        for (int p = lane; p < P; p += 64) {
+            const float dx = A.pxyz[(b * P + p) * 3 + 0] - gx, dy = A.pxyz[(b * P + p) * 3 + 1] - gy,
+                        dz = A.pxyz[(b * P + p) * 3 + 2] - gz;
+            const float d = sqrtf(dx * dx + dy * dy + dz * dz);
+            if (d < best) {
+                best = d;
+                bp = p;
+            }
+        }
+        for (int off = 32; off > 0; off >>= 1) {
+            const float ob = __shfl_xor(best, off);
+            const int op = __shfl_xor(bp, off);
+            if (ob < best || (ob == best && op < bp)) {
+                best = ob;
+                bp = op;
+            }
+        }
+        if ((unsigned)bp >= (unsigned)P) bp = 0;
+        if (lane < 3) {
+            const int k = lane, q = b * P + bp;
+            const float cgk = (k == 0 ? gx : (k == 1 ? gy : gz)) - A.pxyz[q * 3 + k];
+            float gr;
+            const float l = huber(A.pout[(size_t)q * A.pout_pitch + 2 + k] - cgk, gr);
+            if (sub == 0) acc[4] += l;
+            s_dual[j][k] = gr * inv_bbb;
+            if (k == 0) s_dualp[j] = bp;
+        }
+    }
+    __syncthreads();
+    const int grp = tid / LF_G, l = tid % LF_G;
+    for (int pq = sub * LF_PW + grp; pq < P; pq += LF_S * LF_PW) {
+        const int q = b * P + pq;
+        const float px = A.pxyz[q * 3 + 0], py = A.pxyz[q * 3 + 1], pz = A.pxyz[q * 3 + 2];
+        int g;
+        const float best = nearest_box(s_box, BB, px, py, pz, g);
+        const float *o = A.pout + (size_t)q * A.pout_pitch;
+        float *go = A.d_pout + (size_t)q * W;
+        const bool pos = best < A.pos_thr, neg = best > A.neg_thr;
+        if ((pos || neg) && l == 0) {
+            float pr[2];
+            const float ce = softmax_ce(o, 2, pos ? 1 : 0, pr);
+            const float w = 0.5f * (pos ? inv_np : inv_nn);
+            if (pos) acc[1] += ce;
+            else acc[2] += ce;
+            go[0] = pr[0] * w;
+            go[1] = pr[1] * w;
+        }
+        float cen = 0.0f;
+        bool touched = false;
+        if (pos) {
+            const int gi = b * BB + g;
+            if (l < 3) {
+                const float cg = s_box[g][l] - (l == 0 ? px : (l == 1 ? py : pz));
+                float gr;
+                acc[3] += huber(o[2 + l] - cg, gr);
+                cen += gr * inv_np;
+                touched = true;
+            }
+            const int hl = A.hlab[gi];
+            const bool hok = (unsigned)hl < (unsigned)NH;
+            float pb;
+            const float hce = group_softmax_ce(o + 5, NH, hl, l, pb);
+            if (l < NH) go[5 + l] = pb * (0.1f * inv_np);
+            if (l == 0) {
+                acc[5] += hce;
+                float gr;
+                acc[6] += huber((hok ? o[5 + NH + hl] : 0.0f) - A.hres[gi], gr);
+                if (hok) go[5 + NH + hl] = gr * inv_np;
+            }
+            const int sl = A.slab[gi], so = 5 + 2 * NH;
+            const bool sok = (unsigned)sl < (unsigned)NS;
+            const float sce = group_softmax_ce(o + so, NS, sl, l, pb);
+            if (l < NS) go[so + l] = pb * (0.1f * inv_np);
+            if (l == 0) acc[7] += sce;
+            if (l < 3) {
+                float gr;
+                acc[8] += huber((sok ? o[so + NS + sl * 3 + l] : 0.0f) - A.sres[gi * 3 + l], gr);
+                if (sok) go[so + NS + sl * 3 + l] = gr * inv_np;
+            }
+            const int co = W - NC;
+            const float cce = group_softmax_ce(o + co, NC, A.sem[gi], l, pb);
+            if (l < NC) go[co + l] = pb * (0.1f * inv_np);
+            if (l == 0) acc[9] += cce;
+        }
+        if (l < 3) {
+            for (int j = 0; j < BB; j++)
+                if (s_dualp[j] == pq) {
+                    cen += s_dual[j][l];
+                    touched = true;
+                }
+            if (touched) {
+                go[2 + l] = cen;
+                A.d_pxyz[q * 3 + l] = cen;
+            }
+        }
+    }
+    const float inv_bn = 1.0f / (float)(B * N);
+    for (int i = sub * LF_T + tid; i < N; i += LF_S * LF_T) {
+        const int e = b * N + i;
+        const float sx = A.seeds[e * 3 + 0], sy = A.seeds[e * 3 + 1], sz = A.seeds[e * 3 + 2];
+        float best = 0.0f;
+        int g = 0;
+        bool surface = false;
+        for (int j = 0; j < BB; j++) {
+            const float dx = fabsf(sx - s_box[j][0]), dy = fabsf(sy - s_box[j][1]), dz = fabsf(sz - s_box[j][2]);
+            const float c = s_box[j][6], s = s_box[j][7];
+            const float rx = c * dx + s * dz, ry = dy, rz = -s * dx + c * dz;
+            surface = surface || (rx < s_box[j][3] && ry < s_box[j][4] && rz < s_box[j][5]);
+            const float d = sqrtf(rx * rx + ry * ry + rz * rz);
+            if (j == 0 || d < best) {
+                best = d;
+                g = j;
+            }
+        }
+        if (surface) {
+            for (int k = 0; k < 3; k++) {
+                const float df = A.votes[e * 3 + k] - s_box[g][k];
+                acc[0] += fabsf(df);
+                A.d_votes[e * 3 + k] = (df > 0.0f ? 1.0f : (df < 0.0f ? -1.0f : 0.0f)) * inv_bn;
+            }
+        }
+    }
+#pragma unroll
+    for (int i = 0; i < LOSS_NACC; i++) {
+        float v = acc[i];
+        for (int off = 32; off > 0; off >>= 1) v += __shfl_down(v, off);
+        if (lane == 0) s_red[wave][i] = v;
+    }
+    __syncthreads();
+    if (tid < LOSS_NACC) {
+        float v = 0.0f;
+        for (int w = 0; w < nwave; w++) v += s_red[w][tid];
+        __hip_atomic_store(&partial[((size_t)b * LF_S + sub) * LOSS_NACC + tid], v, __ATOMIC_RELAXED, __HIP_MEMORY_SCOPE_AGENT);
+    }
+    __threadfence();
+    __syncthreads();
+    if (tid == 0) s_last = (__hip_atomic_fetch_add(&sticket[b], 1, __ATOMIC_RELAXED, __HIP_MEMORY_SCOPE_AGENT) == LF_S - 1);
+    __syncthreads();
+    if (!s_last) return;
+    __threadfence();
+    if (tid < LOSS_NACC) {
+        float v = 0.0f;
+        for (int s = 0; s < LF_S; s++) {
+            float *at = &partial[((size_t)b * LF_S + s) * LOSS_NACC + tid];
+            v += __hip_atomic_load(at, __ATOMIC_RELAXED, __HIP_MEMORY_SCOPE_AGENT);
+            __hip_atomic_store(at, 0.0f, __ATOMIC_RELAXED, __HIP_MEMORY_SCOPE_AGENT);
+        }
+        s_red[0][tid] = v;
+    }
+    __syncthreads();
+    if (tid != 0) return;
+    __hip_atomic_store(&sticket[b], 0, __ATOMIC_RELAXED, __HIP_MEMORY_SCOPE_AGENT);
+    float v[LOSS_NACC], t[LOSS_NACC];
+    for (int i = 0; i < LOSS_NACC; i++) v[i] = s_red[0][i];
+    if (!scene_fold<LOSS_NACC>(ws, b, B, v, t)) return;
+    const float vote = t[0] * inv_bn;
+    const float obj = t[1] * inv_np + t[2] * inv_nn;
+    const float center = t[3] * inv_np + t[4] * inv_bbb;
+    const float hcls = t[5] * inv_np, hres = t[6] * inv_np, scls = t[7] * inv_np, sres = t[8] * inv_np, sem = t[9] * inv_np;
+    const float box = center + 0.1f * hcls + hres + 0.1f * scls + sres;
+    float *L = A.losses;
+    L[0] = vote + 0.5f * obj + box + 0.1f * sem;
+    L[1] = vote;
+    L[2] = obj;
+    L[3] = center;
+    L[4] = hcls;
+    L[5] = hres;
+    L[6] = scls;
+    L[7] = sres;
+    L[8] = sem;
+    L[9] = box;
+    L[10] = (float)n_pos;
+    L[11] = (float)n_neg;
+}
+
+}
+
+using namespace votenet;
+
+extern "C" const char *votenet_votegroup_last_error(void) { return g_vg_err.text; }
+
+extern "C" int votenet_vote_group_supported(int b, int n, int m)
+{
+    return b > 0 && n >= 1 && n <= VG_MAX_N && m >= 1 && ((long)b * m) % TP == 0 && 64L * b * m < (1L << 31) && (long)b * n < (1L << 31);
+}
+
+extern "C" int votenet_vote_group(int b, int n, int m, float radius, const float *xyz, const int *fps_idx, float *new_xyz, int *idx,
+                                  int *pts_cnt, int *pos, int *hc, float *wh, int *nh, float *geo, long long *cntv, double *moments,
+                                  int *work, int *order, void *stream)
+{
+    VG_REQUIRE(b > 0 && m >= 1, "vote_group: b > 0 scenes of m >= 1 centres expected, got b = %d, m = %d", b, m);
+    VG_REQUIRE(n >= 1 && n <= VG_MAX_N, "vote_group: 1 to %d points per scene, got n = %d", VG_MAX_N, n);
+    VG_REQUIRE(((long)b * m) % TP == 0, "vote_group: the number of centres must be a multiple of %d, got %ld", TP, (long)b * m);
+    VG_REQUIRE(64L * b * m < (1L << 31) && (long)b * n < (1L << 31), "vote_group: row and point counts must be below 2^31");
+    VG_REQUIRE(radius > 0, "vote_group: a positive radius expected, got %g", (double)radius);
+    VG_REQUIRE(xyz && fps_idx && new_xyz && idx && pts_cnt && pos && hc && wh && nh && geo && cntv && moments && work && order,
+               "vote_group: null buffer");
+    VG_REQUIRE((uintptr_t)geo % 16 == 0 && (uintptr_t)cntv % 16 == 0, "vote_group: geo / cntv must be 16-byte aligned");
+    VG_REQUIRE((uintptr_t)moments % 8 == 0, "vote_group: moments must be 8-byte aligned");
+    VG_REQUIRE(((uintptr_t)xyz | (uintptr_t)fps_idx | (uintptr_t)new_xyz | (uintptr_t)idx | (uintptr_t)pts_cnt | (uintptr_t)pos |
+                (uintptr_t)hc | (uintptr_t)wh | (uintptr_t)nh | (uintptr_t)work | (uintptr_t)order) % 4 == 0,
+               "vote_group: every int / float buffer must be 4-byte aligned");
+    const float thr = (radius <= 1e-20f) ? -1.0f : ball_threshold(radius);
+    hipStream_t st = as_stream(stream);
+    const int G = b * m;
+    const long max_rows = 64L * G;
+    hipLaunchKernelGGL(vote_ball_kernel, dim3((m + VG_WAVES - 1) / VG_WAVES, b), dim3(VG_WAVES * 64), 0, st, n, m, thr, xyz, fps_idx, new_xyz,
+                       idx, pts_cnt, work);
+    hipLaunchKernelGGL(vote_scans_kernel, dim3(1), dim3(1024), 0, st, G, n, m, b * n, pts_cnt, pos, hc, wh, nh, idx, work);
+    long gx = (max_rows / 2 + 256 * 8 - 1) / (256 * 8);
+    if (gx > 2048) gx = 2048;
+    hipLaunchKernelGGL(vote_rows_kernel, dim3((unsigned)gx), dim3(256), 0, st, nh, max_rows, n, m, xyz, new_xyz, idx, pts_cnt, hc,
+                       reinterpret_cast<float4 *>(geo), cntv, moments, work, order);
+    return g_vg_err.check_launch("vote_group");
+}
+
+extern "C" size_t votenet_loss_fused_workspace_floats(int b) { return loss_workspace_floats(b); }
+
+extern "C" int votenet_loss_fused(int b, int n_seeds, int n_prop, int n_box, int nh, int ns, int nc, const float *seeds_xyz,
+                                  const float *votes_xyz, const float *proposals_xyz, const float *proposals_output, long output_pitch,
+                                  const float *bboxes_xyz, const float *bboxes_lwh, const float *bboxes_roty, const int *semantic_labels,
+                                  const int *heading_labels, const float *heading_residuals, const int *size_labels,
+                                  const float *size_residuals, float pos_thr, float neg_thr, float *losses, float *d_votes_xyz,
+                                  float *d_proposals_xyz, float *d_proposals_output, float *workspace, void *stream)
+{
+    VG_REQUIRE(b > 0 && n_seeds > 0 && n_prop > 0 && n_box > 0, "loss_fused expects b, n_seeds, n_prop, n_box > 0");
+    VG_REQUIRE(n_box <= LOSS_MAXBOX, "loss_fused expects at most 256 boxes per scene");
+    VG_REQUIRE(nh > 0 && ns > 0 && nc > 0 && nh <= LOSS_MAXC && ns <= LOSS_MAXC && nc <= LOSS_MAXC, "loss_fused expects 0 < nh, ns, nc <= 32");
+    VG_REQUIRE(pos_thr < neg_thr, "loss_fused expects pos_thr < neg_thr (config.py)");
+    VG_REQUIRE((long)b * LF_S < (1L << 31) && (long)b * n_prop < (1L << 28) && (long)b * n_seeds < (1L << 29),
+               "loss_fused: b * n_prop must be below 2^28 and b * n_seeds below 2^29");
+    VG_REQUIRE(seeds_xyz && votes_xyz && proposals_xyz && proposals_output && bboxes_xyz && bboxes_lwh && bboxes_roty &&
+                   semantic_labels && heading_labels && heading_residuals && size_labels && size_residuals && losses &&
+                   d_votes_xyz && d_proposals_xyz && d_proposals_output && workspace,
+               "loss_fused: null buffer");
+    VG_REQUIRE(((uintptr_t)seeds_xyz | (uintptr_t)votes_xyz | (uintptr_t)proposals_xyz | (uintptr_t)proposals_output |
+                (uintptr_t)bboxes_xyz | (uintptr_t)bboxes_lwh | (uintptr_t)bboxes_roty | (uintptr_t)semantic_labels |
+                (uintptr_t)heading_labels | (uintptr_t)heading_residuals | (uintptr_t)size_labels | (uintptr_t)size_residuals |
+                (uintptr_t)losses | (uintptr_t)d_votes_xyz | (uintptr_t)d_proposals_xyz | (uintptr_t)d_proposals_output |
+                (uintptr_t)workspace) % 4 == 0,
+               "loss_fused: every buffer must be 4-byte aligned");
+    VG_REQUIRE(output_pitch >= 5 + 2 * nh + 4 * ns + nc, "loss_fused: the pitch of proposals_output is smaller than its width");
+    LossArgs a = {b, n_seeds, n_prop, n_box, nh, ns, nc, seeds_xyz, votes_xyz, proposals_xyz, proposals_output, bboxes_xyz, bboxes_lwh,
+                  bboxes_roty, semantic_labels, heading_labels, size_labels, heading_residuals, size_residuals, pos_thr, neg_thr, losses,
+                  d_votes_xyz, d_proposals_xyz, d_proposals_output, output_pitch};
+    hipLaunchKernelGGL(votenet_loss_fused_kernel, dim3((unsigned)(b * LF_S)), dim3(LF_T), 0, as_stream(stream), a,
+                       reinterpret_cast<int *>(workspace));
+    return g_vg_err.check_launch("loss_fused");
+}
diff --git a/votenet_amd/loss.py b/votenet_amd/loss.py
--- a/votenet_amd/loss.py
+++ b/votenet_amd/loss.py
@@ -4,6 +4,7 @@
 from .synth import NC, NH, NS
 
 POSITIVE_THRES, NEGATIVE_THRES = 0.3, 0.6
+LOSS_FUSED = True
 NAMES = ("total_cost", "vote_reg_loss", "obj_cls_loss", "center_loss", "heading_cls_loss", "heading_residual_loss",
          "size_cls_loss", "size_residual_loss", "sem_cls_loss", "box_loss", "n_pos", "n_neg")
 GT_KEYS = ("bboxes_xyz", "bboxes_lwh", "bboxes_roty", "semantic_labels", "heading_labels", "heading_residuals", "size_labels",
@@ -14,10 +15,14 @@
     return {k: torch.from_numpy(gt[k]).contiguous().to(device) for k in GT_KEYS}
 
 
+def workspace_floats(b):
+    return int(L.lib().votenet_loss_workspace_floats(b))
+
+
 def loss_buffers(out, losses=None):
     from . import mlp as M
     votes, pxyz, pout = out["votes_xyz"], out["proposals_xyz"], out["proposals_output"]
-    nws = int(L.lib().votenet_loss_workspace_floats(votes.shape[0]))
+    nws = workspace_floats(votes.shape[0])
     if losses is None:
         losses = torch.empty(12, dtype=torch.float32, device=votes.device)
     return losses, M._zeros_f32((votes.numel() + pxyz.numel() + pout.numel() + nws,), votes.device)
@@ -47,7 +52,7 @@
     if pout.shape[2] != 5 + 2 * nh + 4 * ns + nc:
         raise L.InvalidArgumentError("loss: proposals_output has %d channels, expected %d" % (pout.shape[2], 5 + 2 * nh + 4 * ns + nc))
     dev = seeds.device
-    total = votes.numel() + pxyz.numel() + pout.numel() + int(L.lib().votenet_loss_workspace_floats(b))
+    total = votes.numel() + pxyz.numel() + pout.numel() + workspace_floats(b)
     from . import mlp as M
     if buffers is not None:
         losses, flat = buffers
@@ -58,12 +63,17 @@
         flat = M._zeros_f32((total,), dev)
     cot, ws = cotangent_views(votes, pxyz, pout, flat)
     with L.device_guard(dev):
-        L.check(L.lib().votenet_loss_pitched(b, n, p, bb, nh, ns, nc, L.ptr(seeds), L.ptr(votes), L.ptr(pxyz), L.ptr(pout), pout.stride(1),
-                                     L.ptr(gt["bboxes_xyz"]), L.ptr(gt["bboxes_lwh"]), L.ptr(gt["bboxes_roty"]),
-                                     L.ptr(gt["semantic_labels"]), L.ptr(gt["heading_labels"]), L.ptr(gt["heading_residuals"]),
-                                     L.ptr(gt["size_labels"]), L.ptr(gt["size_residuals"]), POSITIVE_THRES, NEGATIVE_THRES,
-                                     L.ptr(losses), L.ptr(cot["votes_xyz"]), L.ptr(cot["proposals_xyz"]), L.ptr(cot["proposals_output"]),
-                                     L.ptr(ws), L.stream_ptr()))
+        args = (b, n, p, bb, nh, ns, nc, L.ptr(seeds), L.ptr(votes), L.ptr(pxyz), L.ptr(pout), pout.stride(1),
+                L.ptr(gt["bboxes_xyz"]), L.ptr(gt["bboxes_lwh"]), L.ptr(gt["bboxes_roty"]),
+                L.ptr(gt["semantic_labels"]), L.ptr(gt["heading_labels"]), L.ptr(gt["heading_residuals"]),
+                L.ptr(gt["size_labels"]), L.ptr(gt["size_residuals"]), POSITIVE_THRES, NEGATIVE_THRES,
+                L.ptr(losses), L.ptr(cot["votes_xyz"]), L.ptr(cot["proposals_xyz"]), L.ptr(cot["proposals_output"]),
+                L.ptr(ws), L.stream_ptr())
+        if LOSS_FUSED:
+            from . import vote_group as VG
+            VG.loss_fused(*args)
+        else:
+            L.check(L.lib().votenet_loss_pitched(*args))
     return losses, cot
 
 
diff --git a/votenet_amd/model.py b/votenet_amd/model.py
--- a/votenet_amd/model.py
+++ b/votenet_amd/model.py
@@ -768,10 +768,11 @@
             g.setdefault("fp2", P.FPModule.geometry(lv["l2_xyz"], lv["l3_xyz"]))
             g.setdefault("prop_fps", P.tf_sampling.farthest_point_sample(self.proposal.npoint, lv["l2_xyz"]))
         ins = self._stretch_inputs(lv, g)
+        from . import loss as VL
         key = tuple((k, tuple(v.shape), v.dtype) for k, v in ins.items()) + (P.HALF_GROUPS, P.ASSEMBLE_FIRST, P.ASSEMBLE_INLINE, P.POOL_GRAM_BACKWARD, P.ASSEMBLED_DECOMPOSED,
                                                                              self.overlap_wgrad, STRETCH_SEGMENTS, M.SPLIT_K, M.COEF_TAIL, P.WGRAD_BATCH, P.POOL_IN_EPILOGUE,
                                                                              self.store.split, bool(getattr(self, "inline_wgrad_tail", INLINE_WGRAD_TAIL)), M.FORWARD_H2, M.ADHOC_H2,
-                                                                             self.proposal_sampling or "seed_fps", self.vote_features or "sum", M.CONFIG_EPOCH)
+                                                                             self.proposal_sampling or "seed_fps", self.vote_features or "sum", P.VOTE_GROUP_FUSED, VL.LOSS_FUSED, M.CONFIG_EPOCH)
         graphs = self.__dict__.setdefault("_stretch_graphs", {})
         sg = graphs.get(key)
         self._gsync.begin()
diff --git a/votenet_amd/pointnet2.py b/votenet_amd/pointnet2.py
--- a/votenet_amd/pointnet2.py
+++ b/votenet_amd/pointnet2.py
@@ -15,6 +15,7 @@
 ASSEMBLE_INLINE = True
 HALF_GROUPS = True
 FUSE_BN_REDUCE = True
+VOTE_GROUP_FUSED = True
 
 
 class ParamStore:
@@ -871,6 +872,12 @@
         elif fps_idx is None:
             fps_idx, new_xyz, idx, pts_cnt = sample_and_group(self.npoint, self.radius, self.nsample, xyz, sample_xyz, self.knn)
         else:
+            if not ahead and VOTE_GROUP_FUSED and ASSEMBLE_INLINE and not self.knn and not self.narrow(xyz.shape[0] * self.npoint * self.nsample) \
+                    and self.half_groups(xyz.shape[0], xyz.shape[1]):
+                from . import vote_group as VG
+                if VG.supported(xyz.shape[0], xyz.shape[1], self.npoint, self.nsample):
+                    new_xyz, idx, pts_cnt, geo, cntv, mom, half = VG.vote_group(xyz, fps_idx, self.radius)
+                    return SAGeometry(fps_idx, new_xyz, M.attach_inverse(idx, xyz.shape[1]), pts_cnt, AssembledRows(geo, cntv, mom, half))
             new_xyz = tf_sampling.gather_point(xyz, fps_idx)
             idx, pts_cnt = _group_indices(self.radius, self.nsample, xyz, new_xyz, self.knn)
         first = None
diff --git a/votenet_amd/vote_group.py b/votenet_amd/vote_group.py
--- /dev/null
+++ b/votenet_amd/vote_group.py
@@ -0,0 +1,48 @@
+import torch
+
+from . import _lib as L
+from . import mlp as M
+
+
+def supported(b, n, m, nsample):
+    return bool(nsample == 64 and L.side_lib("votegroup").votenet_vote_group_supported(int(b), int(n), int(m)))
+
+
+def vote_group(xyz, fps_idx, radius):
+    xyz = L.dev_f32(xyz.detach(), "vote_group expects (batch_size,num_points,3) xyz shape", 3, 3)
+    fps_idx = L.dev_i32(fps_idx, "vote_group fps_idx", 2)
+    b, n, _ = xyz.shape
+    m = fps_idx.shape[1]
+    if fps_idx.shape[0] != b:
+        raise L.InvalidArgumentError("vote_group: fps_idx of %d scenes for %d scenes" % (fps_idx.shape[0], b))
+    dev = xyz.device
+    G, npts = b * m, b * n
+    NP = M.BALL_PIECES
+    new_xyz = torch.empty((b, m, 3), dtype=torch.float32, device=dev)
+    idx = torch.empty((b, m, 64), dtype=torch.int32, device=dev)
+    pts_cnt = torch.empty((b, m), dtype=torch.int32, device=dev)
+    ints = torch.empty((NP - 1) * G + NP * G + 1, dtype=torch.int32, device=dev)
+    pos, hc, nh = ints[:(NP - 1) * G], ints[(NP - 1) * G:-1], ints[-1:]
+    wh = torch.empty(NP * G, dtype=torch.float32, device=dev)
+    geo = torch.empty((G * 64, 4), dtype=torch.float32, device=dev)
+    order = torch.empty(G * 64, dtype=torch.int32, device=dev)
+    nz = npts * 4 + 16 + (npts + 1) // 2
+    if M._StatsArena.active and M._StatsArena.whole_step:
+        zero = M._zeros_i64((nz,), dev)
+    else:
+        zero = torch.zeros(nz, dtype=torch.int64, device=dev)
+    cntv = zero[:npts * 4].view(npts, 4)
+    mom = zero[npts * 4:npts * 4 + 9].view(torch.float64)
+    work = zero[npts * 4 + 16:].view(torch.int32)[:npts]
+    with L.device_guard(dev):
+        L.check(L.side_lib("votegroup").votenet_vote_group(b, n, m, float(radius), L.ptr(xyz), L.ptr(fps_idx), L.ptr(new_xyz), L.ptr(idx),
+                                                           L.ptr(pts_cnt), L.ptr(pos), L.ptr(hc), L.ptr(wh), L.ptr(nh), L.ptr(geo),
+                                                           L.ptr(cntv), L.ptr(mom), L.ptr(work), L.ptr(order), L.stream_ptr()),
+                side="votegroup")
+        half = M.HalfLayout(G, pos, hc, wh, nh, True, None)
+    half._geo, half._order = geo, order
+    return new_xyz, idx, pts_cnt, geo, cntv, mom, half
+
+
+def loss_fused(*args):
+    L.check(L.side_lib("votegroup").votenet_loss_fused(*args), side="votegroup")
```

Result: no change. 2286 (-0.5%).
